# mkeeter/fidget

Measured on AMD Instinct MI355X. Metric: Mvoxel/s (interval+point eval) on prospero.vm 1024^3, higher is better.
Workload: dtype f32; 1 GPU; prospero.vm 3D heightmap+normals 1024^3, HipShape render hints (the library's tiles: 128/32/8, or 32/8 when the root level has few tiles), world_to_model=I

## Files before the change

fidget_amd/_abi.py:

```python
import ctypes as C
import os

import numpy as np

from ._build import LIB_PATH

UNARY = ["neg", "abs", "recip", "sqrt", "square", "floor", "ceil", "round", "sin", "cos", "tan",
         "asin", "acos", "atan", "exp", "ln", "not", "rand"]
BINARY = ["add", "sub", "mul", "div", "atan2", "min", "max", "compare", "mod", "and", "or", "mix"]

FH_OPS = (["Output", "Input", "CopyReg", "CopyImm"] + [u.capitalize() for u in UNARY]
          + [b.capitalize() + "RR" for b in ["add", "sub", "mul", "div", "atan2", "compare", "mix", "mod", "min", "max", "and", "or"]]
          + [b.capitalize() + "RI" for b in ["add", "sub", "mul", "div", "atan2", "compare", "mix", "mod", "min", "max", "and", "or"]]
          + [b.capitalize() + "IR" for b in ["sub", "div", "atan2", "compare", "mix", "mod"]])

STATUS = {1: "BadVarSlice", 2: "MismatchedSlices", 3: "BadChoiceSlice", 4: "MissingVar", 5: "BadTape",
          6: "Unsupported", 7: "HipError", 8: "Cancelled", 9: "ParseError", 10: "Overflow"}

GEOMETRY_PIXEL = np.dtype([("normal", np.float32, 3), ("depth", np.uint32)])
HIP_TILES_2D, HIP_TILES_3D = [128, 16], [128, 32, 8]
VM_TILES_2D, VM_TILES_3D = [128, 32, 8], [128, 64, 32, 16, 8]


class FidgetHipError(RuntimeError):
# ... 30 lines not shown
    "fhip_ctx_set_option": (i32, [vp, C.c_char_p, i32]),
    "fhip_ctx_get_option": (i32, [vp, C.c_char_p, C.POINTER(i32)]),
    "fhip_tape_from_bytecode": (i32, [vp, vp, C.c_size_t, C.POINTER(vp)]),
    "fhip_tape_free": (None, [vp]),
    "fhip_tape_len": (u32, [vp]),
    "fhip_tape_choice_count": (u32, [vp]),
    "fhip_tape_reg_count": (u32, [vp]),
    "fhip_tape_var_count": (u32, [vp]),
    "fhip_tape_output_count": (u32, [vp]),
    "fhip_tape_ops": (u32, [vp, vp, u32]),
    "fhip_tape_reg_tape": (i32, [vp, u32, vp, u32, vp, u32, vp]),
    "fhip_tape_group_count": (u32, [vp]),
    "fhip_tape_group_op": (i32, [vp]),
    "fhip_tape_group": (i32, [vp, vp, u32, vp]),
    "fhip_tape_term_plan": (u32, [vp, vp]),
    "fhip_tape_term_group": (i32, [vp, vp, u32, vp]),
    "fhip_tape_term_tree": (u32, [vp, vp, u32]),
    "fhip_tape_term_choice_src": (u32, [vp, vp, u32]),
    "fhip_simplify": (i32, [vp, vp, vp, u32, C.POINTER(vp)]),
    "fhip_interval_eval": (i32, [vp, vp, vp, u32, u32, vp, vp, vp]),
    "fhip_point_eval": (i32, [vp, vp, vp, u32, u32, vp, vp, vp]),
    "fhip_float_eval": (i32, [vp, vp, vp, vp, u32, vp]),
    "fhip_grad_eval": (i32, [vp, vp, vp, vp, u32, vp]),
    "fhip_solve": (i32, [vp, vp, u32, vp, vp, vp, u32, vp, u32, u32, vp, vp, vp, vp]),
    "fhip_render2d": (i32, [vp, vp, C.POINTER(_Cfg2D), vp, i32]),
    "fhip_render3d": (i32, [vp, vp, C.POINTER(_Cfg3D), vp, i32]),
    "fhip_render3d_shard": (i32, [vp, vp, C.POINTER(_Cfg3D), vp, i32, u32, u32]),
    "fhip_render3d_block": (i32, [vp, vp, C.POINTER(_Cfg3D), vp, i32, u32, vp]),
    "fhip_merge_depth": (i32, [vp, vp, vp, u64, u32]),
    "fhip_denoise_normals": (i32, [vp, vp, u32, u32, vp, i32]),
    "fhip_compute_ssao": (i32, [vp, vp, u32, u32, u32, vp, u32, vp, u32, vp, i32]),
    "fhip_blur_ssao": (i32, [vp, vp, u32, u32, vp, i32]),
    "fhip_apply_shading": (i32, [vp, vp, u32, u32, u32, vp, vp, i32]),
    "fhip_to_rgba": (i32, [vp, vp, u32, u32, i32, vp, i32]),
    "fhip_mesh_sample": (i32, [vp, vp, u32, vp, vp, vp, vp, u32, C.POINTER(vp)]),
    "fhip_mesh_build": (i32, [vp, vp, u32, vp, vp, vp, vp, u32, C.POINTER(vp)]),
    "fhip_mesh_vertices": (None, [vp, vp]),
    "fhip_mesh_triangles": (None, [vp, vp]),
    "fhip_mesh_vertices_ptr": (vp, [vp]),
    "fhip_mesh_triangles_ptr": (vp, [vp]),
    "fhip_mesh_free": (None, [vp]),
    "fhip_mesh_counts": (None, [vp, vp]),
    "fhip_mesh_leaves": (None, [vp, vp]),
    "fhip_mesh_sample_part": (i32, [vp, vp, u32, vp, vp, vp, vp, u32, u32, u32, C.POINTER(vp)]),
    "fhip_mesh_part_bytes": (C.c_uint64, [vp]),
    "fhip_mesh_part_export": (None, [vp, vp]),
    "fhip_mesh_merge": (i32, [vp, vp, vp, u32, vp, C.POINTER(vp)]),
    "fhip_mesh_vertices_dev": (vp, [vp]),
    "fhip_mesh_triangles_dev": (vp, [vp]),
    "fhip_mesh_stl_bytes": (u64, [vp]),
    "fhip_mesh_stl": (i32, [vp, vp, vp, i32]),
    "fhip_mesh_vertex_grads": (i32, [vp, vp, vp, vp, vp, vp, u32, vp, i32]),
    "fhip_shape_occupancy": (i32, [vp, vp, u32, vp, vp, vp, vp, u32, vp]),
    "fhip_voxels_words": (u64, [u32]),
    "fhip_shape_voxels": (i32, [vp, vp, u32, vp, vp, vp, vp, u32, vp, i32, vp]),
    "fhip_voxels_slices": (i32, [vp, vp, u32, u32, u32, vp, i32]),
    "fhip_voxels_layer_counts": (i32, [vp, vp, u32, vp, i32]),
    "fhip_contour2d": (i32, [vp, vp, vp, vp]),
    "fhip_contours_counts": (None, [vp, vp]),
    "fhip_contours_vertices": (i32, [vp, vp]),
    "fhip_contours_segments": (i32, [vp, vp]),
    "fhip_contours_next": (i32, [vp, vp]),
    "fhip_contours_vertices_dev": (vp, [vp]),
    "fhip_contours_segments_dev": (vp, [vp]),
    "fhip_contours_free": (None, [vp]),
    "fhip_contour_loops": (i32, [vp, u64, vp, vp, vp, vp]),
    "fhip_voxels_components": (i32, [vp, vp, u32, i32, u32, i32, vp]),
    "fhip_components_counts": (None, [vp, vp]),
    "fhip_components_table": (i32, [vp, vp, vp, vp, vp, vp]),
    "fhip_components_label_slices": (i32, [vp, vp, vp, i32, u32, u32, vp, i32]),
    "fhip_components_extract": (i32, [vp, vp, vp, i32, vp, u64, vp, i32]),
    "fhip_components_free": (None, [vp]),
    "fhip_voxels_distance": (i32, [vp, vp, u32, i32, i32, vp]),
    "fhip_distance_info": (None, [vp, vp]),
    "fhip_distance_slices": (i32, [vp, vp, u32, u32, vp, i32]),
    "fhip_distance_dev": (vp, [vp]),
    "fhip_distance_threshold": (i32, [vp, vp, u32, i32, vp, i32]),
    "fhip_distance_free": (None, [vp]),
    "fhip_distance_thickness": (i32, [vp, vp, vp]),
    "fhip_thickness_info": (None, [vp, vp]),
    "fhip_thickness_thin": (i32, [vp, vp, u32, vp, i32]),
    "fhip_thickness_histogram": (i32, [vp, vp, vp, u32, vp, i32]),
    "fhip_voxels_surface": (i32, [vp, vp, u32, i32, vp]),
    "fhip_voxels_mesh": (i32, [vp, vp, u32, i32, vp]),
    "fhip_voxels_flow": (i32, [vp, vp, vp, u32, i32, u32, u32, vp, i32]),
    "fhip_voxels_overhangs": (i32, [vp, vp, u32, i32, u32, u32, i32, vp, i32]),
    "fhip_voxels_heights": (i32, [vp, vp, u32, i32, u32, vp, i32]),
    "fhip_triangles_voxels": (i32, [vp, vp, u64, vp, u64, i32, vp, u32, vp, i32, vp]),
    "fhip_mesh_voxels": (i32, [vp, vp, vp, u32, vp, i32, vp]),
    "fhip_triangles_topology": (i32, [vp, vp, u64, vp, u64, i32, i32, u32, vp]),
    "fhip_mesh_topology": (i32, [vp, vp, i32, u32, vp]),
    "fhip_topology_counts": (None, [vp, vp]),
    "fhip_topology_vertex_rows": (u64, [vp]),
    "fhip_topology_vertices": (i32, [vp, vp]),
    "fhip_topology_triangles": (i32, [vp, vp]),
    "fhip_topology_triangle_shells": (i32, [vp, vp]),
    "fhip_topology_vertices_dev": (vp, [vp]),
    "fhip_topology_triangles_dev": (vp, [vp]),
    "fhip_topology_triangle_shells_dev": (vp, [vp]),
    "fhip_topology_shells": (i32, [vp, vp, vp, vp, vp, vp, vp, vp]),
    "fhip_topology_edges": (i32, [vp, vp, u32, vp, i32]),
    "fhip_topology_free": (None, [vp]),
    "fhip_voxels_outlines": (i32, [vp, vp, u32, i32, u32, u32, u32, vp]),
    "fhip_outlines_counts": (None, [vp, vp]),
    "fhip_outlines_layers": (i32, [vp, vp, vp, vp, vp]),
    "fhip_outlines_vertices": (i32, [vp, u64, u64, vp, vp, vp]),
    "fhip_outlines_loops": (i32, [vp, u64, u64, vp, vp, vp, vp, vp, vp]),
    "fhip_outlines_xy_dev": (vp, [vp]),
    "fhip_outlines_next_dev": (vp, [vp]),
    "fhip_outlines_loop_dev": (vp, [vp]),
    "fhip_outlines_free": (None, [vp]),
    "fhip_outlines_nesting": (i32, [vp, vp, vp, i32, vp]),
    "fhip_nesting_counts": (None, [vp, vp]),
    "fhip_nesting_layers": (i32, [vp, vp, vp, vp]),
    "fhip_nesting_loops": (i32, [vp, u64, u64, vp, vp, vp, vp, vp]),
    "fhip_nesting_parent_dev": (vp, [vp]),
    "fhip_nesting_depth_dev": (vp, [vp]),
    "fhip_nesting_children": (i32, [vp, u64, vp, vp]),
    "fhip_nesting_free": (None, [vp]),
    "fhip_topology_slices": (i32, [vp, vp, vp, u32, u32, vp]),
    "fhip_slices_counts": (None, [vp, vp]),
    "fhip_slices_planes": (i32, [vp, vp, vp, vp, vp]),
    "fhip_slices_loops": (i32, [vp, vp, vp, vp, vp, vp, vp, vp, vp]),
    "fhip_slices_vertices": (i32, [vp, vp, vp, vp, vp, vp, vp]),
    "fhip_slices_xy_dev": (vp, [vp]),
    "fhip_slices_next_dev": (vp, [vp]),
    "fhip_slices_loop_dev": (vp, [vp]),
    "fhip_slices_plane_dev": (vp, [vp]),
    "fhip_slices_free": (None, [vp]),
    "fhip_profile_enable": (None, [vp, i32]),
    "fhip_profile_read": (i32, [vp, vp, vp]),
    "fhip_profile_read_kernels": (i32, [vp, vp, vp]),
    "fhip_render_counters": (i32, [vp, vp]),
    "fhip_graph_new": (vp, []),
    "fhip_graph_free": (None, [vp]),
    "fhip_graph_len": (u32, [vp]),
    "fhip_graph_var": (u32, [vp, i32, u64]),
    "fhip_graph_constant": (u32, [vp, f32]),
    "fhip_graph_unary": (u32, [vp, i32, u32]),
    "fhip_graph_binary": (u32, [vp, i32, u32, u32]),
    "fhip_graph_from_text": (u32, [vp, C.c_char_p]),
    "fhip_tape_from_graph": (i32, [vp, vp, vp, u32, C.POINTER(vp)]),
    "fhip_tape_axis_slot": (i32, [vp, i32]),
    "fhip_tape_var_slot": (i32, [vp, u64]),
    "fhip_screen_to_world": (None, [vp, i32, vp]),
    "fhip_debug_stats": (i32, [vp, vp]),
    "fhip_debug_leaf_stats": (i32, [vp, vp]),
    "fhip_debug_tape_links": (u32, [vp, vp, u32]),
    "fhip_debug_tape_chain": (u32, [vp, vp, u32]),
    "fhip_debug_leaves": (u32, [vp, vp, u32]),
    "fhip_debug_probe": (i32, [vp, vp]),
    "fhip_debug_lane_frames": (u64, [vp]),
    "fhip_debug_rare_frames": (u64, [vp]),
    "fhip_debug_lane_tune": (i32, [vp, vp, vp]),
    "fhip_debug_trans_probe": (i32, [vp, u32, u32, u32, u64, vp]),
    "fhip_debug_arena": (u32, [vp, u32, u32, vp]),
    "fhip_debug_bound_tape": (i32, [vp, vp, vp, vp, vp, u32, C.POINTER(vp)]),
    "fhip_debug_bench": (i32, [vp, vp, u32, u32, i32, vp]),
    "fhip_debug_ubench": (i32, [vp, u32, u32, u32, vp]),
    "fhip_debug_math_sweep": (i32, [vp, i32, u32, u32, u64, vp, vp]),
    "fhip_debug_groups": (u32, [vp, i32, u32, vp, u32, vp]),
    "fhip_debug_walk_dual": (None, [vp, u64, vp, vp, u64, i32, vp, vp, vp]),
    "fhip_debug_stl_pack": (i32, [vp, vp, u64, vp, u64, vp]),
}
del vp, u32, i32, f32, u64
EXPORTS = list(SIGNATURES)

_lib = None


def lib():
    global _lib
    if _lib is None:
        if not os.path.exists(LIB_PATH):
            raise ImportError(f"{LIB_PATH} is missing: run `python -c 'import __graft_entry__ as g; g.build()'`")
        L = C.CDLL(LIB_PATH)
        for name, (res, args) in SIGNATURES.items():
            fn = getattr(L, name)
            fn.restype = res
            fn.argtypes = args
        _lib = L
    return _lib


def _p(a):
    return a.ctypes.data_as(C.c_void_p) if a is not None else None


def libm_probe():
    buf = C.create_string_buffer(200)
    n = lib().fhip_libm_probe(buf, 200)
    return int(n), buf.value.decode()


class _Handle:
    def __init__(self, h, free):
        self.h = h
        self._free = free

    def __del__(self):
        if self.h and self._free is not None:
            self._free(self.h)
            self.h = None


class _DeviceArray:
    def __init__(self, owner, ptr, shape, typestr):
        self._owner = owner
        self.ptr, self.shape = int(ptr), tuple(shape)
        self.__cuda_array_interface__ = {"shape": self.shape, "typestr": typestr, "data": (self.ptr, False), "version": 2, "strides": None}
```

fidget_amd/context.py:

```python
import ctypes as C
import os

import numpy as np

from ._abi import FidgetHipError, _p, lib


class HipContext:

    def __init__(self, device=0, stream=None):
        h = C.c_void_p()
        st = lib().fhip_ctx_create(device, C.c_void_p(stream or 0), C.byref(h))
        if st != 0:
            raise FidgetHipError(st, "no usable HIP device: fidget_amd has no CPU fallback")
        self._h = h

    def __del__(self):
        try:
            lib().fhip_ctx_destroy(self._h)
        except Exception:
            pass

    def check(self, st):
        if st != 0:
            raise FidgetHipError(st, (lib().fhip_last_error(self._h) or b"").decode())

    def sync(self):
        self.check(lib().fhip_ctx_sync(self._h))

    def trim(self):
        self.check(lib().fhip_ctx_trim(self._h))

    def reserve_arena(self, megabytes):
        self.check(lib().fhip_ctx_reserve_arena(self._h, int(megabytes)))

    def cancel(self):
        lib().fhip_cancel(self._h)

    def cancel_watch(self, flag):
        self._watched = flag
        lib().fhip_cancel_watch(self._h, None if flag is None else flag.ctypes.data_as(C.c_void_p))

    def cancel_reset(self):
        lib().fhip_cancel_reset(self._h)

    def lane_tune(self):
        ms, ln = (C.c_float * 3)(), C.c_int(0)
        ph = lib().fhip_debug_lane_tune(self._h, ms, C.byref(ln))
        return {"phase": int(ph), "stage_pipeline_ms": [float(ms[0]), float(ms[2])], "frame_lanes_ms": float(ms[1]), "kept": "frame lanes" if ln.value else "stage pipeline"}

    def lane_frames(self):
        return int(lib().fhip_debug_lane_frames(self._h))

    def rare_frames(self):
        return int(lib().fhip_debug_rare_frames(self._h))

    def set_option(self, name, value=1):
        self.check(lib().fhip_ctx_set_option(self._h, name.encode(), int(value)))

    def option(self, name):
        v = C.c_int(0)
        self.check(lib().fhip_ctx_get_option(self._h, name.encode(), C.byref(v)))
        return v.value

    def options(self, **kw):
        import contextlib

        @contextlib.contextmanager
        def scope():
            old = {k: self.option(k) for k in kw}
            try:
                for k, v in kw.items():
                    self.set_option(k, v)
                yield self
            finally:
                for k, v in old.items():
                    self.set_option(k, v)
        return scope()

    def profile(self, on):
        lib().fhip_profile_enable(self._h, int(on))

    def profile_read(self):
        ms = np.zeros(4, np.float64)
        n = np.zeros(4, np.uint32)
        self.check(lib().fhip_profile_read(self._h, _p(ms), _p(n)))
        names = ["tiles", "points", "normals", "other"]
        return {k: (float(ms[i]), int(n[i])) for i, k in enumerate(names)}

    def profile_read_kernels(self):
        ms = np.zeros(8, np.float64)
        n = np.zeros(8, np.uint32)
        self.check(lib().fhip_profile_read_kernels(self._h, _p(ms), _p(n)))
        names = ["fh_columns", "fh_float_eval_16x4", "fh_float_eval_32x2", "fh_tiles", "fh_prune1", "fh_tiles_v32", "fh_tiles_v64", "unused"]
        return {k: (float(ms[i]), int(n[i])) for i, k in enumerate(names)}

    def counters(self):
        c = np.zeros(8, np.uint64)
        self.check(lib().fhip_render_counters(self._h, _p(c)))
        return {"arena_ops": int(c[0]), "arena_overflow": int(c[1]), "leaves_last_slab": int(c[2]),
                "queue_overflow": int(c[3]), "groups_last_slab": [int(v) for v in c[4:6]], "hip_tile_stage_frames": int(c[6]), "substituted_tile_lists": int(c[7])}

    def last_leaves(self, cap=1 << 20):
        dt = np.dtype([("off", np.uint32), ("len", np.uint32), ("regs", np.uint16), ("choices", np.uint16),
                       ("x", np.uint32), ("y", np.uint32), ("z", np.uint32)])
        buf = np.zeros(cap, dt)
        n = lib().fhip_debug_leaves(self._h, _p(buf), cap)
        return buf[:n]

    def groups(self, kind, index, cap=1 << 20):
        dt = np.dtype([("off", np.uint32), ("len", np.uint32), ("regs", np.uint16), ("choices", np.uint16),
                       ("x", np.uint32), ("y", np.uint32), ("z", np.uint32), ("first", np.uint32), ("n", np.uint32), ("stride", np.uint32)])
        assert dt.itemsize == 36
        buf = np.zeros(cap, dt)
        cnt = np.zeros(2, np.uint32)
        n = lib().fhip_debug_groups(self._h, kind, index, _p(buf), cap, _p(cnt))
        return buf[:n], (int(cnt[0]), int(cnt[1]))

    def arena_ops(self, off, n):
        buf = np.zeros(n, np.uint64)
        got = lib().fhip_debug_arena(self._h, int(off), int(n), _p(buf))
        return buf[:got]

    def leaf_stats(self):
        c = np.zeros(8, np.uint64)
        self.check(lib().fhip_debug_leaf_stats(self._h, _p(c)))
        return {"leaves": int(c[0]), "tape_ops": int(c[1]), "tape_words_read": int(c[2]), "lane_ops": int(c[3]),
                "prune2_phase_clocks_max": [int(v) for v in c[4:8]]}

    def wave_stats(self):
        c = np.zeros(64, np.uint64)
        self.check(lib().fhip_debug_stats(self._h, _p(c)))
        names = ["tiles_l0", "tiles_l1", "tiles_l2", "tiles_l3", "tiles_l4", "columns_c0", "columns_c12", "tiles_2d"]
        self.tile_v = {f"l{l}": {"slots": int(c[8 + l]), "fwd_clocks": int(c[16 + l]), "prune_clocks": int(c[24 + l]), "max_slot_clocks": int(c[l])}
                       for l in range(8) if c[8 + l]}
        self.tile_phases = {f"l{l}": {"fwd_us": int(c[32 + l]) / 100.0, "prune_us": int(c[40 + l]) / 100.0,
                                      "ops": int(c[48 + l]), "ops_written": int(c[56 + l]), "fwd_shader_clocks": int(c[16 + l])} for l in range(8) if c[48 + l]}
        return {k: {"busy_us_sum": int(c[4 * i]) / 100.0, "busy_us_max": int(c[4 * i + 1]) / 100.0,
                    "waves": int(c[4 * i + 2]), "units": int(c[4 * i + 3])} for i, k in enumerate(names) if c[4 * i + 2]}


_default_ctx = None


def default_context():
    global _default_ctx
    if _default_ctx is None:
        _default_ctx = HipContext(int(os.environ.get("LOCAL_RANK", "0")) if os.environ.get("FHIP_USE_LOCAL_RANK") else 0)
    return _default_ctx
```

fidget_amd/csrc/capi_context.hpp:

```cpp
int fhip_libm_probe(char* msg, size_t cap) {
    using namespace fhlm;
    struct R1 { const char* name; float (*mine)(float); float (*host)(float); };
    const R1 r1[] = {{"sinf", [](float x) { return sincosf_<MemTables, false>(x); }, [](float x) { return ::sinf(x); }},
                     {"cosf", [](float x) { return sincosf_<MemTables, true>(x); }, [](float x) { return ::cosf(x); }},
                     {"tanf", [](float x) { return tanf_<MemTables>(x); }, [](float x) { return ::tanf(x); }},
                     {"asinf", [](float x) { return asinf_(x); }, [](float x) { return ::asinf(x); }},
                     {"acosf", [](float x) { return acosf_(x); }, [](float x) { return ::acosf(x); }},
                     {"atanf", [](float x) { return atanf_(x); }, [](float x) { return ::atanf(x); }},
                     {"expf", [](float x) { return expf_<MemTables>(x); }, [](float x) { return ::expf(x); }},
                     {"logf", [](float x) { return logf_<MemTables>(x); }, [](float x) { return ::logf(x); }}};
    static const float args[32] = {0.1f, -0.3f, 0.5f, 0.7853982f, 0.7853981f, 1.0f, -1.0f, 1.5707964f, 2.0f, 3.0f, 3.1415927f, -4.5f, 6.2831855f, 10.0f,
                                   -25.132742f, 100.0f, 119.99999f, 120.0f, 1000.5f, -31415.926f, 1.0e6f, 3.0e8f, 1.0e-3f, 2.4414062e-4f, -1.0e-5f,
                                   1.0e-20f, 0.9999999f, 0.99f, -0.6f, 0.25f, 87.0f, -80.0f};
    int bad = 0;
    if (msg && cap) msg[0] = 0;
    auto differ = [](float a, float b) { return !(a != a && b != b) && f2u(a) != f2u(b); };
    for (const R1& r : r1)
        for (float x : args) {
            volatile float xv = x;
            const float a = r.mine(xv), b = r.host(xv);
            if (differ(a, b) && bad++ == 0 && msg && cap)
                snprintf(msg, cap, "%s(%a): device family 0x%08x, host libm 0x%08x", r.name, (double)x, f2u(a), f2u(b));
        }
    for (int i = 0; i < 32; i++) {
        volatile float y = args[i], x = args[(i * 7 + 3) & 31];
        const float a = atan2f_(y, x), b = ::atan2f(y, x);
        if (differ(a, b) && bad++ == 0 && msg && cap)
            snprintf(msg, cap, "atan2f(%a, %a): device family 0x%08x, host libm 0x%08x", (double)y, (double)x, f2u(a), f2u(b));
    }
    return bad;
}
static void libm_probe_once() {
    static std::once_flag once;
    std::call_once(once, [] {
        char msg[160];
        const int bad = fhip_libm_probe(msg, sizeof msg);
        const char* q = getenv("FHIP_QUIET");
        if (bad && !(q && q[0] == '1'))
            fprintf(stderr, "fidget-hip: this host's libm is not the one the device restates (glibc 2.35 x86-64, FMA variants; trans_libm.hpp): %d of 288 "
                            "probe arguments differ, first %s.  Transcendental opcodes on the device will differ from this host's CPU evaluators "
                            "in the last bits for some arguments.\n", bad, msg);
    });
}

fhip_status fhip_ctx_create(int device, void* stream, fhip_ctx** out) {
    if (!out) return FHIP_ERR_BAD_TAPE;
    *out = nullptr;
    libm_probe_once();
    int count = 0;
    if (hipGetDeviceCount(&count) != hipSuccess || count <= 0 || device >= count) return FHIP_ERR_HIP;
    fhip_ctx* c = new fhip_ctx();
    c->device = device;
    c->stream = (hipStream_t)stream;
    if (hipSetDevice(device) != hipSuccess) { delete c; return FHIP_ERR_HIP; }
    hipDeviceProp_t prop;
    if (hipGetDeviceProperties(&prop, device) == hipSuccess) c->n_cu = prop.multiProcessorCount;
    options_from_env(c->opt);
    apply_options(c);
    const void* fns[] = {(const void*)k_eval_f32<false>, (const void*)k_eval_interval<false>, (const void*)k_eval_grad<false>,
                         (const void*)k_tiles<false, false, true, 16>, (const void*)k_tiles<false, true, true, 16>,
                         (const void*)k_tiles<true, false, true, 16>, (const void*)k_tiles<true, true, true, 16>,
                         (const void*)k_tiles<false, false, true, 64>, (const void*)k_tiles<false, true, true, 64>,
                         (const void*)k_tiles<true, false, true, 64>, (const void*)k_tiles<true, true, true, 64>,
                         (const void*)k_pixels2d<0, false>, (const void*)k_pixels2d<0, true>,
                         (const void*)k_leaves3d<2, 0, 1, false>, (const void*)k_leaves3d<2, 0, 1, true>,
                         (const void*)k_normals3d<false, true>, (const void*)k_normals3d<true, true>};
    for (const void* f : fns) (void)hipFuncSetAttribute(f, hipFuncAttributeMaxDynamicSharedMemorySize, FH_LDS_MAX);
    {
        std::vector<char> alt;
        if (const char* p = getenv("FHIP_INTERP_CO")) {
            if (FILE* f = fopen(p, "rb")) {
                fseek(f, 0, SEEK_END);
                long n = ftell(f);
                fseek(f, 0, SEEK_SET);
                alt.resize(n > 0 ? (size_t)n : 0);
                if (n <= 0 || fread(alt.data(), 1, (size_t)n, f) != (size_t)n) alt.clear();
                fclose(f);
            }
            if (alt.empty()) { fprintf(stderr, "fidget-hip: FHIP_INTERP_CO=%s cannot be read\n", p); delete c; return FHIP_ERR_HIP; }
            fprintf(stderr, "fidget-hip: assembly kernels from %s\n", p);
        }
        if (hipModuleLoadData(&c->asm_mod, alt.empty() ? (const void*)fh_interp_co : (const void*)alt.data()) != hipSuccess) { delete c; return FHIP_ERR_HIP; }
    }
    for (int i = 0; i < FH_ASM_COUNT; i++)
        if (hipModuleGetFunction(&c->asm_fn[i], c->asm_mod, FH_ASM_NAMES[i]) != hipSuccess) { delete c; return FHIP_ERR_HIP; }
    (void)hipFuncSetAttribute((const void*)c->asm_fn[FH_ASM_TILES], hipFuncAttributeMaxDynamicSharedMemorySize, FH_LDS_MAX);
    (void)hipFuncSetAttribute((const void*)c->asm_fn[FH_ASM_TILES_T], hipFuncAttributeMaxDynamicSharedMemorySize, FH_LDS_MAX);
    (void)hipGetLastError();
    {
        int lo = 0, hi = 0;
        (void)hipDeviceGetStreamPriorityRange(&lo, &hi);
        if (hipStreamCreateWithPriority(&c->stream2, hipStreamNonBlocking, hi) != hipSuccess) { delete c; return FHIP_ERR_HIP; }
    }
    (void)hipEventCreateWithFlags(&c->ev_fork, hipEventDisableTiming);
    (void)hipEventCreateWithFlags(&c->ev_pre, hipEventDisableTiming);
    (void)hipEventCreateWithFlags(&c->ev_l0, hipEventDisableTiming);
    (void)hipEventCreateWithFlags(&c->ev_l1, hipEventDisableTiming);
    (void)hipEventCreateWithFlags(&c->ev_rest_fork, hipEventDisableTiming);
    (void)hipEventCreateWithFlags(&c->ev_rest_join, hipEventDisableTiming);
    (void)hipEventCreateWithFlags(&c->ev_done, hipEventDisableTiming);
    for (auto& o : c->others) (void)hipEventCreateWithFlags(&o.ev_done, hipEventDisableTiming);
    if (!c->stream3 && hipStreamCreateWithFlags(&c->stream3, hipStreamNonBlocking) != hipSuccess) { delete c; return FHIP_ERR_HIP; }
    if (hipStreamCreateWithFlags(&c->stream_pre, hipStreamNonBlocking) != hipSuccess) { delete c; return FHIP_ERR_HIP; }
    if (c->sticky.ensure(256) != hipSuccess || hipMemset(c->sticky.p, 0, 256) != hipSuccess) { delete c; return FHIP_ERR_HIP; }
    {
        void* hf = nullptr;
        if (hipHostMalloc(&hf, 64, hipHostMallocDefault) != hipSuccess) { delete c; return FHIP_ERR_HIP; }
        memset(hf, 0, 64);
        ((uint32_t*)hf)[2] = 1;
        c->host_flags = (volatile uint32_t*)hf;
    }
    c->ev_tiles.resize(FH_MAX_SLABS); c->ev_leaves.resize(FH_MAX_SLABS); c->ev_aux.resize(FH_MAX_SLABS);
    for (int i = 0; i < FH_MAX_SLABS; i++) {
        (void)hipEventCreateWithFlags(&c->ev_tiles[i], hipEventDisableTiming);
        (void)hipEventCreateWithFlags(&c->ev_leaves[i], hipEventDisableTiming);
        (void)hipEventCreateWithFlags(&c->ev_aux[i], hipEventDisableTiming);
    }
    (void)hipFuncSetAttribute((const void*)k_prune2, hipFuncAttributeMaxDynamicSharedMemorySize, FH_LDS_MAX);
    {
        const void* fb[] = {(const void*)k_teval3d<false, true>, (const void*)k_teval3d<true, true>};
        for (const void* f : fb) (void)hipFuncSetAttribute(f, hipFuncAttributeMaxDynamicSharedMemorySize, FH_LDS_MAX);
    }
    *out = c;
    return FHIP_OK;
}
static void lanes_release(fhip_ctx* ctx, bool keep_measurements = false);
void fhip_ctx_destroy(fhip_ctx* c) {
    if (!c) return;
    (void)hipSetDevice(c->device);
    (void)hipStreamSynchronize(c->stream);
    lanes_release(c);
    if (c->ev_last) (void)hipEventDestroy(c->ev_last);
    if (c->stream_pre) (void)hipStreamSynchronize(c->stream_pre);
    if (c->stream2) (void)hipStreamSynchronize(c->stream2);
    (void)hipStreamSynchronize(c->stream);
    DevBuf* bufs[] = {&c->tmp_out, &c->io_a, &c->io_b, &c->io_c, &c->io_d, &c->io_e, &c->sticky};
    for (DevBuf* b : bufs) b->release();
    c->release_all();
    for (auto& o : c->others) o.release_all();
    if (c->stream_pre) (void)hipStreamDestroy(c->stream_pre);
    if (c->ev_rest_fork) (void)hipEventDestroy(c->ev_rest_fork);
    if (c->ev_rest_join) (void)hipEventDestroy(c->ev_rest_join);
    if (c->ev_pre) (void)hipEventDestroy(c->ev_pre);
    if (c->ev_l0) (void)hipEventDestroy(c->ev_l0);
    if (c->ev_l1) (void)hipEventDestroy(c->ev_l1);
    for (auto& sg : c->staging) { if (sg.p) (void)hipHostFree(sg.p); if (sg.ev) (void)hipEventDestroy(sg.ev); }
    c->mesh_leaves.release();
    if (c->host_flags) (void)hipHostFree((void*)c->host_flags);
    if (c->mesh_pinned) (void)hipHostFree(c->mesh_pinned);
    mesh_cache_release(c->mesh_octree_cache);
    free(c->mesh_first);
    if (c->asm_mod) (void)hipModuleUnload(c->asm_mod);
    if (c->stream2) { (void)hipStreamSynchronize(c->stream2); (void)hipStreamDestroy(c->stream2); }
    if (c->stream3) { (void)hipStreamSynchronize(c->stream3); (void)hipStreamDestroy(c->stream3); }
    for (hipEvent_t e : c->ev_aux) (void)hipEventDestroy(e);
    if (c->ev_fork) (void)hipEventDestroy(c->ev_fork);
    for (hipEvent_t e : c->ev_tiles) (void)hipEventDestroy(e);
    for (hipEvent_t e : c->ev_leaves) (void)hipEventDestroy(e);
    for (auto& e : c->prof_events) { (void)hipEventDestroy(e.second.first); (void)hipEventDestroy(e.second.second); }
    for (auto& e : c->asm_events) { (void)hipEventDestroy(e.second.first); (void)hipEventDestroy(e.second.second); }
    delete c;
}
const char* fhip_last_error(const fhip_ctx* c) { return c ? c->err.c_str() : "no context"; }
fhip_status fhip_ctx_sync(fhip_ctx* c) {
    (void)hipSetDevice(c->device);
    HIP_TRY(c, hipStreamSynchronize(c->stream));
    fhip_status st = FHIP_OK;
    for (auto& o : c->others)
        if (o.async_pending) {
            std::swap(static_cast<FrameBufs&>(*c), o);
            c->async_pending = false;
            const fhip_status s1 = finish_render(c);
            if (st == FHIP_OK) st = s1;
            std::swap(static_cast<FrameBufs&>(*c), o);
        }
    if (c->async_pending) {
        c->async_pending = false;
        const fhip_status s2 = finish_render(c);
        if (st == FHIP_OK) st = s2;
    }
    for (fhip_ctx* L : c->lanes) {
        const fhip_status s3 = fhip_ctx_sync(L);
        if (s3 && st == FHIP_OK) { st = s3; c->err = L->err; }
    }
    uint32_t sticky = 0;
    HIP_TRY(c, hipMemcpy(&sticky, c->sticky.p, 4, hipMemcpyDeviceToHost));
    if (sticky) {
        HIP_TRY(c, hipMemset(c->sticky.p, 0, 4));
        if (st == FHIP_OK) st = fail(c, FHIP_ERR_OVERFLOW, "device work queue overflow in an earlier asynchronous frame");
    }
    return st;
}
void fhip_cancel(fhip_ctx* c) { c->cancelled.store(1); }
void fhip_cancel_reset(fhip_ctx* c) { c->cancelled.store(0); }
void fhip_cancel_watch(fhip_ctx* c, const void* flag) { c->watch.store((const volatile unsigned char*)flag); }
fhip_status fhip_ctx_trim(fhip_ctx* c) {
    if (!c) return FHIP_ERR_UNSUPPORTED;
    (void)hipSetDevice(c->device);
    HIP_TRY(c, hipDeviceSynchronize());
    lanes_release(c);
    c->mesh_leaves.release();
    if (c->mesh_pinned) { (void)hipHostFree(c->mesh_pinned); c->mesh_pinned = nullptr; c->mesh_pinned_cap = 0; }
    return FHIP_OK;
}
static hipError_t sync_own_streams(fhip_ctx* ctx);
fhip_status fhip_ctx_reserve_arena(fhip_ctx* c, size_t megabytes) {
    if (!c) return FHIP_ERR_UNSUPPORTED;
    (void)hipSetDevice(c->device);
    const size_t want = std::min(c->arena_cap_bytes, megabytes << 20);
    if (want <= c->arena_bytes) return FHIP_OK;
    HIP_TRY(c, sync_own_streams(c));
    c->arena_bytes = want;
    return FHIP_OK;
}
fhip_status fhip_ctx_set_option(fhip_ctx* c, const char* name, int value) {
    if (!c || !name) return FHIP_ERR_UNSUPPORTED;
    if (!strcmp(name, "leaf_streams") || !strcmp(name, "pre_priority")) return fail(c, FHIP_ERR_UNSUPPORTED, std::string(name) + " is fixed when the context is created");
    for (const FhOptionEntry& e : FH_OPTION_TABLE)
        if (!strcmp(e.name, name)) {
            if (c->opt.*(e.field) == value) return FHIP_OK;
            const fhip_status st = fhip_ctx_sync(c);
            c->opt.*(e.field) = value;
            apply_options(c);
            lanes_release(c);
            return st;
        }
    return fail(c, FHIP_ERR_UNSUPPORTED, std::string("unknown option ") + name);
}
fhip_status fhip_ctx_get_option(const fhip_ctx* c, const char* name, int* value) {
    if (!c || !name || !value) return FHIP_ERR_UNSUPPORTED;
    for (const FhOptionEntry& e : FH_OPTION_TABLE)
        if (!strcmp(e.name, name)) { *value = c->opt.*(e.field); return FHIP_OK; }
    return FHIP_ERR_UNSUPPORTED;
}
```

fidget_amd/csrc/capi_core.hpp:

```cpp
struct DevBuf {
    void* p = nullptr;
    size_t cap = 0;
    hipError_t ensure(size_t bytes) {
        if (bytes <= cap) return hipSuccess;
        if (p) (void)hipFree(p);
        p = nullptr; cap = 0;
        hipError_t e = hipMalloc(&p, bytes);
        if (e == hipSuccess) cap = bytes;
        return e;
    }
    void release() { if (p) (void)hipFree(p); p = nullptr; cap = 0; }
};

static std::atomic<uint64_t> g_tape_serial{1};
struct BoundCache {
    struct Entry {
        uint64_t hash = 0, used = 0;
        std::vector<uint64_t> key;
        std::shared_ptr<const fhip_tape> tape;
    };
    std::mutex lock;
    std::vector<Entry> entries;
    uint64_t clock = 0;
};
struct fhip_tape {
    const uint64_t serial = g_tape_serial.fetch_add(1);
    fh::HostTape t;
    mutable uint64_t* d_ops = nullptr;
    std::vector<fh::HostTape> groups;
    int group_op = -1;
    fh::TermPlan plan;
    std::vector<fh::HostTape> tgroups;
    mutable FhTopOp* d_top = nullptr;
    mutable uint32_t* d_chsrc = nullptr;
    mutable uint64_t* d_links = nullptr;
    mutable uint64_t* d_ctab = nullptr;
    mutable std::atomic<uint32_t> input_slots{0x80000000u};
    mutable uint32_t n_chain = 0;
    mutable bool links_tried = false;
    mutable std::mutex upload_lock;
    mutable int device = -1;
    uint64_t parent_serial = 0;
    std::weak_ptr<const fhip_tape> self;
    mutable BoundCache bound;
};
struct fhip_graph {
    fh::Graph g;
};

#ifndef __HIP_DEVICE_COMPILE__
__asm__(".section .rodata\n.global fh_interp_co\n.p2align 6\nfh_interp_co:\n.incbin \"" FH_INTERP_CO "\"\n.previous\n");
#endif
extern "C" const char fh_interp_co[];
enum { FH_ASM_COLUMNS = 0, FH_ASM_FLOAT_16x4, FH_ASM_FLOAT_32x2, FH_ASM_TILES, FH_ASM_PRUNE1, FH_ASM_TILES_V32, FH_ASM_TILES_V64, FH_ASM_PROBE, FH_ASM_UBENCH, FH_ASM_COLUMNS_T, FH_ASM_NORMALS, FH_ASM_NORMALS_T, FH_ASM_TILES_T, FH_ASM_TILES_V32_T, FH_ASM_TILES_V64_T, FH_ASM_FLOAT_16x4_T, FH_ASM_FLOAT_32x2_T, FH_ASM_TRANS_PROBE, FH_ASM_COUNT };
static const char* const FH_ASM_NAMES[FH_ASM_COUNT] = {"fh_columns", "fh_float_eval_16x4", "fh_float_eval_32x2", "fh_tiles", "fh_prune1",
                                                       "fh_tiles_v32", "fh_tiles_v64", "fh_probe", "fh_ubench", "fh_columns_t", "fh_normals", "fh_normals_t", "fh_tiles_t", "fh_tiles_v32_t", "fh_tiles_v64_t", "fh_float_eval_16x4_t", "fh_float_eval_32x2_t", "fh_trans_probe"};

#define FH_OPTION_LIST(X)                                                                                                       \
     \
    X(no_asm, 0) X(no_split, 0) X(no_asm_tiles, 0) X(no_tiles_v, 0) X(no_asm_tiles_t, 0) X(no_columns_t, 0) X(no_asm_normals, 0)   \
    X(no_tape_groups, 0) X(prune2, 1)                                                                                           \
                      \
    X(no_column_inv, 0) X(no_zrep, 0) X(root32_max, 4096) X(column_walk, 1) X(column_group, 2)                                                    \
                                                                                                 \
    X(no_pipeline, 0) X(frame_lanes, 4) X(lanes_fail, 0) X(slab_layers, 4) X(arena_mb, 4096)  \
          \
    X(mesh_device_assembly, 1) X(mesh_device_walk, 1) X(mesh_simplify_min_ops, 256) X(mesh_keep_device, 0)                      \
                                                                                                              \
    X(probe, 0) X(stats, 0)
struct FhOptions {
#define X(name, dflt) int name = dflt;
    FH_OPTION_LIST(X)
#undef X
};
struct FhOptionEntry { const char* name; int FhOptions::*field; };
static const FhOptionEntry FH_OPTION_TABLE[] = {
#define X(name, dflt) {#name, &FhOptions::name},
    FH_OPTION_LIST(X)
#undef X
};
static void options_from_env(FhOptions& o) {
    for (const FhOptionEntry& e : FH_OPTION_TABLE) {
        std::string var = "FHIP_";
        for (const char* c = e.name; *c; c++) var += (char)toupper((unsigned char)*c);
        if (const char* v = getenv(var.c_str())) o.*(e.field) = *v ? atoi(v) : 1;
    }
}

struct FrameBufs {
    DevBuf state, arena, leaves, leaf_table, zbuf, normals, fp_lists, mind, squeue, slots[2], leaves_b, leaf_table_b, fp_lists_b, chw[2], tvals, topch, chwr, gscratch, rare_scratch;
    DevBuf queue[FH_MAX_LEVELS];
    uint32_t frame_stamp = 0;
    uint64_t resident_serial = 0;
    uint32_t resident_groups = 0;
    uint32_t forked = 0;
    bool async_pending = false;
    hipEvent_t ev_done = nullptr;
    bool ev_done_valid = false;
    std::shared_ptr<const fhip_tape> bound_hold;
    CleanSig clean;
    void release_all() {
        clean = CleanSig();
        DevBuf* bufs[] = {&state, &arena, &leaves, &leaf_table, &zbuf, &normals, &fp_lists, &mind, &squeue, &slots[0], &slots[1],
                          &leaves_b, &leaf_table_b, &fp_lists_b, &chw[0], &chw[1], &tvals, &topch, &chwr, &gscratch, &rare_scratch};
        for (DevBuf* b : bufs) b->release();
        for (auto& q : queue) q.release();
        if (ev_done) (void)hipEventDestroy(ev_done);
        ev_done = nullptr;
        bound_hold.reset();
    }
};
struct fhip_ctx : FrameBufs {
    FhOptions opt;
#define FH_EXTRA_SETS 4
    FrameBufs others[FH_EXTRA_SETS];
    uint32_t extra_sets = 3;
    bool frame_pipeline = true;
    hipStream_t stream_pre = nullptr;
    uint32_t pre_turn = 0;
    hipEvent_t ev_rest_fork = nullptr, ev_rest_join = nullptr;
    hipEvent_t ev_pre = nullptr, ev_l0 = nullptr, ev_l1 = nullptr;
    hipModule_t asm_mod = nullptr;
    hipFunction_t asm_fn[FH_ASM_COUNT] = {};
    bool use_asm = true;
    bool probe = false;
    bool use_split = true;
    bool use_pipeline = true;
    hipStream_t stream2 = nullptr, stream3 = nullptr;
    std::vector<hipEvent_t> ev_tiles, ev_leaves, ev_aux;
    hipEvent_t ev_fork = nullptr;
    FhRenderState last_state_b;
    uint32_t slab_contexts = 4;
    int device = 0;
    hipStream_t stream = nullptr;
    int n_cu = 256;
    std::string err;
    bool launch_failed = false;
    std::atomic<int> cancelled{0};
    const std::atomic<int>* cancel_src = nullptr;
    std::atomic<const volatile unsigned char*> watch{nullptr};
    bool is_cancelled() const {
        if ((cancel_src ? cancel_src : &cancelled)->load() != 0) return true;
        const volatile unsigned char* w = watch.load(std::memory_order_relaxed);
        return w && *w != 0;
    }
    DevBuf tmp_out, io_a, io_b, io_c, io_d, io_e;
    DevBuf sticky;
    struct Staging { void* p = nullptr; size_t cap = 0; hipEvent_t ev = nullptr; bool used = false; } staging[8];
    DevBuf mesh_leaves;
    void* mesh_pinned = nullptr;
    size_t mesh_pinned_cap = 0;
    void* mesh_octree_cache = nullptr;
    uint32_t* mesh_first = nullptr;
    size_t mesh_first_cap = 0;
    uint32_t staging_next = 0;
    size_t arena_bytes = (size_t)256 << 20, arena_cap_bytes = (size_t)4 << 30;
    uint64_t hip_tile_frames = 0;
    uint64_t substituted_tiles = 0;
    int last_hip_error = 0;
    volatile uint32_t* host_flags = nullptr;
    bool profiling = false;
    std::vector<std::pair<int, std::pair<hipEvent_t, hipEvent_t>>> prof_events;
    std::vector<std::pair<int, std::pair<hipEvent_t, hipEvent_t>>> asm_events;
    FhRenderState last_state;
    bool have_last_state = false;
    std::vector<fhip_ctx*> lanes;
    uint32_t lane_next = 0;
    uint64_t rare_frames = 0;
    uint64_t lane_frames = 0;
    uint64_t lane_frames_wanted = 0;
    hipEvent_t ev_last = nullptr;
    bool ev_last_valid = false;
    struct LaneTune {
        uint64_t key = 0, used = 0;
        int phase = 0;
        uint32_t n = 0;
        bool lanes = false;
        float ms[3] = {0.0f, 0.0f, 0.0f};
        hipEvent_t ev[6] = {nullptr, nullptr, nullptr, nullptr, nullptr, nullptr};
    };
    std::vector<LaneTune> lane_tune;
    uint64_t tune_last_key = 0, tune_clock = 0;
    int tune_cur = -1;
    bool is_lane = false, lane_stream_owned = false;
    DevBuf lane_img;
    hipEvent_t lane_done = nullptr, lane_copied = nullptr;
    bool lane_copied_valid = false;
};

#define FH_ARENA_START_MB 128
static void apply_options(fhip_ctx* c) {
    c->use_asm = c->opt.no_asm == 0;
    c->use_split = c->opt.no_split == 0;
    c->probe = c->opt.probe != 0;
    c->use_pipeline = c->opt.no_pipeline == 0;
    c->frame_pipeline = true;
    c->slab_contexts = 4;
    c->arena_cap_bytes = (size_t)std::max(1, c->opt.arena_mb) << 20;
    c->arena_bytes = std::min(c->arena_cap_bytes, std::max(c->arena_bytes, (size_t)FH_ARENA_START_MB << 20));
    c->extra_sets = 3;
}

static fhip_status finish_render(fhip_ctx* ctx);
static void mesh_cache_release(void* octree);
static fhip_status fail(fhip_ctx* ctx, fhip_status s, const std::string& msg) {
    if (ctx) ctx->err = msg;
    return s;
}
#define HIP_TRY(ctx, call)                                                                                       \
    do {                                                                                                         \
        hipError_t e_ = (call);                                                                                  \
        if (e_ != hipSuccess) {                                                                                  \
            if (ctx) (ctx)->last_hip_error = (int)e_;                                                            \
            return fail(ctx, FHIP_ERR_HIP, std::string(#call) + ": " + hipGetErrorString(e_));                   \
        }                                                                                                        \
    } while (0)

template <class F>
static void launch(fhip_ctx* ctx, hipStream_t st, int klass, F&& f) {
    if (ctx->profiling) {
        hipEvent_t a, b;
        (void)hipEventCreate(&a);
        (void)hipEventCreate(&b);
        (void)hipEventRecord(a, st);
        f();
        (void)hipEventRecord(b, st);
        ctx->prof_events.push_back({klass, {a, b}});
    } else {
        f();
    }
}

static bool simplify_host(const fh::HostTape& p, const uint8_t* choices, fh::HostTape& out) {
    std::vector<int> map(FH_MAX_REGS, -1);
    fh::RegPool pool;
    std::vector<uint64_t> rev;
    uint32_t ci = p.n_choices, kept = 0;
    auto use = [&](uint32_t r) { if (map[r] < 0) map[r] = pool.take(); return (uint32_t)map[r]; };
    for (size_t k = p.ops.size(); k-- > 0;) {
        const uint64_t w = p.ops[k];
        const uint32_t w0 = (uint32_t)w, w1 = (uint32_t)(w >> 32);
        const uint32_t op = FH_W_OP(w0), ro = FH_W_OUT(w0), ra = FH_W_A(w0), rb = w1;
        const bool is_choice = fh_is_choice(op);
        uint32_t c = FH_CHOICE_BOTH;
        if (is_choice) {
            c = choices[--ci];
            if (c == FH_CHOICE_UNKNOWN) return false;
        }
        if (op == FH_OUTPUT) { rev.push_back(fh_pack(op, 0, use(ra), 0, w1)); continue; }
        const int no = map[ro];
        if (no < 0) continue;
        map[ro] = -1;
        int alias = -1;
        bool copy_imm = false;
        if (op == FH_COPY_REG) alias = (int)ra;
        else if (is_choice && c == FH_CHOICE_LEFT) alias = (int)ra;
        else if (is_choice && c == FH_CHOICE_RIGHT) { if (fh_is_rr(op)) alias = (int)rb; else copy_imm = true; }
        if (alias >= 0) {
            if (map[alias] < 0) { map[alias] = no; continue; }
            pool.give(no);
            rev.push_back(fh_pack(FH_COPY_REG, no, map[alias], 0, 0));
            continue;
        }
        pool.give(no);
        if (copy_imm) { rev.push_back(fh_pack(FH_COPY_IMM, no, 0, 0, w1)); continue; }
        uint32_t na = 0, nb = 0;
        if (op != FH_INPUT && op != FH_COPY_IMM) na = use(ra);
        if (fh_is_rr(op)) nb = use(rb);
        if (is_choice) kept++;
        rev.push_back(fh_pack(op, no, na, nb, w1));
    }
    out.ops.assign(rev.rbegin(), rev.rend());
    out.n_regs = pool.high;
    out.n_choices = kept;
    out.n_outputs = p.n_outputs;
    out.n_vars = p.n_vars;
    out.vars = p.vars;
    return true;
}

template <class T> struct FhKArgs;
template <class... K> struct FhKArgs<void (*)(K...)> {
    template <class... A> static size_t pack(char* buf, A&&... a) {
        size_t off = 0;
        auto put = [&](auto v) {
            constexpr size_t al = alignof(decltype(v));
            off = (off + al - 1) & ~(al - 1);
            memcpy(buf + off, &v, sizeof(v));
            off += sizeof(v);
        };
        (put(static_cast<K>(std::forward<A>(a))), ...);
        return off;
    }
    static constexpr size_t bytes = (sizeof(K) + ... + 0) + 16 * sizeof...(K);
};
template <auto Kernel, class... A>
static inline void fh_launch(fhip_ctx* ctx, dim3 g, dim3 b, size_t lds, hipStream_t st, A&&... a) {
    constexpr int MAXDEV = 64;
    static std::atomic<hipFunction_t> fns[MAXDEV];
    static std::atomic<bool> no_handle[MAXDEV];
    const int device = ctx->device;
    hipFunction_t fn = nullptr;
    if (device >= 0 && device < MAXDEV) {
        fn = fns[device].load(std::memory_order_acquire);
        if (!fn && !no_handle[device].load(std::memory_order_relaxed)) {
            if (hipGetFuncBySymbol(&fn, (const void*)Kernel) != hipSuccess || !fn) { fn = nullptr; no_handle[device].store(true, std::memory_order_relaxed); (void)hipGetLastError(); }
            else fns[device].store(fn, std::memory_order_release);
        }
    }
    hipError_t e;
    if (!fn) {
        hipLaunchKernelGGL(Kernel, g, b, lds, st, std::forward<A>(a)...);
        e = hipGetLastError();
    } else {
        alignas(16) char buf[FhKArgs<decltype(Kernel)>::bytes];
        size_t bytes = FhKArgs<decltype(Kernel)>::pack(buf, std::forward<A>(a)...);
        void* extra[] = {HIP_LAUNCH_PARAM_BUFFER_POINTER, buf, HIP_LAUNCH_PARAM_BUFFER_SIZE, &bytes, HIP_LAUNCH_PARAM_END};
        e = hipModuleLaunchKernel(fn, g.x, g.y, g.z, b.x, b.y, b.z, (unsigned)lds, st, nullptr, extra);
    }
    if (e != hipSuccess) {
        ctx->launch_failed = true;
        ctx->last_hip_error = (int)e;
        if (ctx->err.empty()) ctx->err = std::string("kernel launch: ") + hipGetErrorString(e);
        (void)hipGetLastError();
    }
// ... 4 lines not shown
```

fidget_amd/csrc/capi_debug.hpp:

```cpp
void fhip_profile_enable(fhip_ctx* ctx, int on) { ctx->profiling = on != 0; }
fhip_status fhip_profile_read(fhip_ctx* ctx, double ms[4], uint32_t launches[4]) {
    HIP_TRY(ctx, hipStreamSynchronize(ctx->stream));
    for (int i = 0; i < 4; i++) { ms[i] = 0; launches[i] = 0; }
    for (auto& e : ctx->prof_events) {
        float t = 0;
        if (hipEventElapsedTime(&t, e.second.first, e.second.second) == hipSuccess) { ms[e.first] += t; launches[e.first]++; }
    }
    return FHIP_OK;
}
fhip_status fhip_profile_read_kernels(fhip_ctx* ctx, double ms[8], uint32_t launches[8]) {
    HIP_TRY(ctx, hipStreamSynchronize(ctx->stream));
    for (int i = 0; i < 8; i++) { ms[i] = 0; launches[i] = 0; }
    for (auto& e : ctx->asm_events) {
        float t = 0;
        if (e.first < 8 && hipEventElapsedTime(&t, e.second.first, e.second.second) == hipSuccess) { ms[e.first] += t; launches[e.first]++; }
    }
    return FHIP_OK;
}
fhip_status fhip_render_counters(fhip_ctx* ctx, uint64_t out[8]) {
    fhip_status st = finish_render(ctx);
    if (st != FHIP_OK && st != FHIP_ERR_OVERFLOW) return st;
    const FhRenderState& S = ctx->last_state;
    out[0] = S.arena_head; out[1] = S.arena_overflow; out[2] = S.n_leaves; out[3] = S.queue_overflow;
    for (int i = 0; i < 2; i++) out[4 + i] = S.count[i + 1];
    out[6] = ctx->hip_tile_frames;
    out[7] = ctx->substituted_tiles;
    return FHIP_OK;
}

fhip_status fhip_debug_stats(fhip_ctx* ctx, uint64_t out[64]) {
    fhip_status st = finish_render(ctx);
    if (st != FHIP_OK && st != FHIP_ERR_OVERFLOW) return st;
    for (int i = 0; i < 64; i++) out[i] = ctx->last_state.stat[i];
    return FHIP_OK;
}
uint32_t fhip_debug_tape_links(const fhip_tape* tape, uint64_t* out, uint32_t cap) {
    std::vector<uint64_t> lk;
    std::vector<uint64_t> cops;
    if (!fh::compute_links(tape->t, lk, cops)) return 0;
    for (size_t i = 0; i < lk.size() && i < cap; i++) out[i] = lk[i];
    return (uint32_t)lk.size();
}
uint32_t fhip_debug_tape_chain(const fhip_tape* tape, uint32_t* out, uint32_t cap) {
    std::vector<uint64_t> lk;
    std::vector<uint64_t> cops;
    if (!fh::compute_links(tape->t, lk, cops)) return 0;
    const std::vector<uint32_t> chain = chain_table(tape, cops);
    for (size_t i = 0; i < chain.size() && i < cap; i++) out[i] = chain[i];
    return (uint32_t)chain.size();
}
fhip_status fhip_debug_leaf_stats(fhip_ctx* ctx, uint64_t out[8]) {
    fhip_status st = finish_render(ctx);
    if (st != FHIP_OK && st != FHIP_ERR_OVERFLOW) return st;
    for (int i = 0; i < 8; i++) out[i] = ctx->last_state.leaf_stat[i];
    return FHIP_OK;
}

uint32_t fhip_debug_leaves(fhip_ctx* ctx, void* out, uint32_t cap) {
    if (finish_render(ctx) != FHIP_OK) return 0;
    const uint32_t n = std::min(std::min(ctx->last_state.n_leaves, ctx->last_state.leaf_cap), cap);
    if (hipMemcpy(out, ctx->last_state.leaves, (size_t)n * sizeof(FhLeaf), hipMemcpyDeviceToHost) != hipSuccess) return 0;
    return n;
}

uint32_t fhip_debug_groups(fhip_ctx* ctx, int kind, uint32_t index, void* out, uint32_t cap, uint32_t counts[2]) {
    counts[0] = counts[1] = 0;
    if (finish_render(ctx) != FHIP_OK) return 0;
    const FhRenderState& S = ctx->last_state;
    const FhGroup* base; uint32_t ns, nb, qcap;
    if (kind == 0) {
        if (index >= FH_MAX_LEVELS || !S.queue[index]) return 0;
        base = S.queue[index]; ns = S.count[index]; nb = S.count_big[index]; qcap = S.qcap[index];
    } else {
        if (index >= FH_MAX_SLABS || !S.squeue) return 0;
        base = S.squeue + (size_t)index * S.squeue_cap; ns = S.scount[index]; nb = S.scount_big[index]; qcap = S.squeue_cap;
    }
    ns = std::min(ns, qcap); nb = std::min(nb, qcap - ns);
    const uint32_t n0 = std::min(ns, cap), n1 = std::min(nb, cap - n0);
    if (n0 && hipMemcpy(out, base, (size_t)n0 * sizeof(FhGroup), hipMemcpyDeviceToHost) != hipSuccess) return 0;
    if (n1 && hipMemcpy((FhGroup*)out + n0, base + (qcap - nb), (size_t)n1 * sizeof(FhGroup), hipMemcpyDeviceToHost) != hipSuccess) return 0;
    counts[0] = n0; counts[1] = n1;
    return n0 + n1;
}

fhip_status fhip_debug_probe(fhip_ctx* ctx, float* out) {
    HIP_TRY(ctx, ctx->io_a.ensure(16 * 256));
    struct { void* p; } ka = {ctx->io_a.p};
    if (launch_asm(ctx, ctx->stream, FH_ASM_PROBE, 1, &ka, sizeof(ka)) != hipSuccess) return FHIP_ERR_HIP;
    HIP_TRY(ctx, hipStreamSynchronize(ctx->stream));
    HIP_TRY(ctx, hipMemcpy(out, ctx->io_a.p, 16 * 256, hipMemcpyDeviceToHost));
    return FHIP_OK;
}

fhip_status fhip_debug_ubench(fhip_ctx* ctx, uint32_t test, uint32_t iters, uint32_t n_waves, float* out) {
    HIP_TRY(ctx, ctx->io_a.ensure((size_t)n_waves * 4));
    HIP_TRY(ctx, hipMemsetAsync(ctx->io_a.p, 0, (size_t)n_waves * 4, ctx->stream));
    struct { void* p; uint32_t test, iters; } ka = {ctx->io_a.p, test, iters};
    if (launch_asm(ctx, ctx->stream, FH_ASM_UBENCH, n_waves, &ka, sizeof(ka), 64) != hipSuccess) return FHIP_ERR_HIP;
    HIP_TRY(ctx, hipStreamSynchronize(ctx->stream));
    HIP_TRY(ctx, hipMemcpy(out, ctx->io_a.p, (size_t)n_waves * 4, hipMemcpyDeviceToHost));
    return FHIP_OK;
}

fhip_status fhip_debug_math_sweep(fhip_ctx* ctx, int op, uint32_t first, uint32_t stride, uint64_t n, const float* ref, uint64_t out[4]) {
    (void)hipSetDevice(ctx->device);
    HIP_TRY(ctx, ctx->io_a.ensure(n * 4));
    HIP_TRY(ctx, ctx->io_b.ensure(64));
    HIP_TRY(ctx, hipMemcpyAsync(ctx->io_a.p, ref, n * 4, hipMemcpyHostToDevice, ctx->stream));
    HIP_TRY(ctx, hipMemsetAsync(ctx->io_b.p, 0, 64, ctx->stream));
    hipLaunchKernelGGL(k_math_sweep, dim3(ctx->n_cu * 16), dim3(256), 0, ctx->stream, op, first, stride, (size_t)n, (const float*)ctx->io_a.p,
                       (unsigned long long*)ctx->io_b.p);
    HIP_TRY(ctx, hipGetLastError());
    unsigned long long r[4];
    HIP_TRY(ctx, hipMemcpyAsync(r, ctx->io_b.p, 32, hipMemcpyDeviceToHost, ctx->stream));
    HIP_TRY(ctx, hipStreamSynchronize(ctx->stream));
    out[0] = r[0] >> 32; out[1] = r[1]; out[2] = r[2]; out[3] = r[0] & 0xFFFFFFFFull;
    return FHIP_OK;
}

fhip_status fhip_debug_trans_probe(fhip_ctx* ctx, uint32_t copy, uint32_t fn, uint32_t first, uint64_t n, uint64_t out[2]) {
    (void)hipSetDevice(ctx->device);
    if (!n || n % 256 || n > (1ull << 28)) return fail(ctx, FHIP_ERR_UNSUPPORTED, "trans probe: n must be a multiple of 256, at most 2^28");
    if (!ctx->asm_fn[FH_ASM_TRANS_PROBE]) return fail(ctx, FHIP_ERR_UNSUPPORTED, "trans probe: the assembly kernels are not loaded");
    HIP_TRY(ctx, ctx->io_a.ensure(n * 4));
    HIP_TRY(ctx, ctx->io_b.ensure(64));
    HIP_TRY(ctx, hipMemsetAsync(ctx->io_a.p, 0x5A, n * 4, ctx->stream));
    HIP_TRY(ctx, hipMemsetAsync(ctx->io_b.p, 0, 64, ctx->stream));
    struct { void* out; uint32_t first, copy, fn, pad; } ka = {ctx->io_a.p, first, copy, fn, 0};
    if (launch_asm(ctx, ctx->stream, FH_ASM_TRANS_PROBE, (uint32_t)(n / 256), &ka, sizeof(ka)) != hipSuccess) return FHIP_ERR_HIP;
    hipLaunchKernelGGL(k_trans_compare, dim3(ctx->n_cu * 16), dim3(256), 0, ctx->stream, (int)fn, first, (size_t)n, (const uint32_t*)ctx->io_a.p,
                       (unsigned long long*)ctx->io_b.p);
    HIP_TRY(ctx, hipGetLastError());
    unsigned long long r[2];
    HIP_TRY(ctx, hipMemcpyAsync(r, ctx->io_b.p, 16, hipMemcpyDeviceToHost, ctx->stream));
    HIP_TRY(ctx, hipStreamSynchronize(ctx->stream));
    out[0] = r[1]; out[1] = r[0] & 0xFFFFFFFFull;
    return FHIP_OK;
}

uint64_t fhip_debug_rare_frames(const fhip_ctx* ctx) {
    if (!ctx) return 0;
    uint64_t n = ctx->rare_frames;
    for (const fhip_ctx* l : ctx->lanes) n += l ? l->rare_frames : 0;
    return n;
}
uint64_t fhip_debug_lane_frames(const fhip_ctx* ctx) { return ctx ? ctx->lane_frames : 0; }
int fhip_debug_lane_tune(const fhip_ctx* ctx, float ms[3], int* lanes) {
    if (!ctx) return -1;
    for (const auto& t : ctx->lane_tune)
        if (t.key == ctx->tune_last_key) {
            if (ms) { ms[0] = t.ms[0]; ms[1] = t.ms[1]; ms[2] = t.ms[2]; }
            if (lanes) *lanes = t.lanes ? 1 : 0;
            return t.phase;
        }
    return -1;
}

uint32_t fhip_debug_arena(fhip_ctx* ctx, uint32_t off, uint32_t n, uint64_t* out) {
    if ((size_t)(off + (size_t)n) * 8 > ctx->arena_bytes) return 0;
    if (hipMemcpy(out, (const uint64_t*)ctx->arena.p + off, (size_t)n * 8, hipMemcpyDeviceToHost) != hipSuccess) return 0;
    return n;
}

fhip_status fhip_debug_bench(fhip_ctx* ctx, const fhip_tape* tape, uint32_t n_waves, uint32_t reps, int variant, double* ms) {
    fhip_status st = tape_to_device(ctx, tape);
    if (st) return st;
    HIP_TRY(ctx, ctx->state.ensure(2 * sizeof(FhRenderState)));
    FhRenderState S;
    memset(&S, 0, sizeof(S));
    for (int i = 0; i < FH_MAX_INPUTS; i++) S.P.in_kind[i] = i % 3;
    HIP_TRY(ctx, hipMemcpy(ctx->state.p, &S, sizeof(S), hipMemcpyHostToDevice));
    HIP_TRY(ctx, ctx->io_a.ensure((size_t)n_waves * WAVE * 4));
    hipEvent_t a, b;
    HIP_TRY(ctx, hipEventCreate(&a));
    HIP_TRY(ctx, hipEventCreate(&b));
    const uint32_t len = (uint32_t)tape->t.ops.size();
    FhRenderState* dS = (FhRenderState*)ctx->state.p;
    for (int it = 0; it < 2; it++) {
        HIP_TRY(ctx, hipEventRecord(a, ctx->stream));
        if (variant == 0) hipLaunchKernelGGL((k_bench_points<16, 4>), dim3(n_waves), dim3(WAVE), 0, ctx->stream, dS, tape->d_ops, len, reps, (float*)ctx->io_a.p);
        else if (variant == 1) hipLaunchKernelGGL((k_bench_points<32, 2>), dim3(n_waves), dim3(WAVE), 0, ctx->stream, dS, tape->d_ops, len, reps, (float*)ctx->io_a.p);
        else if (variant == 3) hipLaunchKernelGGL((k_bench_points<32, 1>), dim3(n_waves), dim3(WAVE), 0, ctx->stream, dS, tape->d_ops, len, reps, (float*)ctx->io_a.p);
        else hipLaunchKernelGGL((k_bench_points<0, 1>), dim3(n_waves), dim3(WAVE), (size_t)std::max<uint32_t>(tape->t.n_regs, 1) * WAVE * 4, ctx->stream, dS, tape->d_ops, len, reps, (float*)ctx->io_a.p);
        HIP_TRY(ctx, hipEventRecord(b, ctx->stream));
        HIP_TRY(ctx, hipEventSynchronize(b));
    }
    float t = 0;
    HIP_TRY(ctx, hipEventElapsedTime(&t, a, b));
    *ms = t;
    (void)hipEventDestroy(a); (void)hipEventDestroy(b);
    return FHIP_OK;
}

static const int UNARY_MAP[] = {FH_NEG, FH_ABS, FH_RECIP, FH_SQRT, FH_SQUARE, FH_FLOOR, FH_CEIL, FH_ROUND, FH_SIN,
                                FH_COS, FH_TAN, FH_ASIN, FH_ACOS, FH_ATAN, FH_EXP, FH_LN, FH_NOT, FH_RAND};
static const int BINARY_MAP[] = {FH_ADD_RR, FH_SUB_RR, FH_MUL_RR, FH_DIV_RR, FH_ATAN2_RR, FH_MIN_RR, FH_MAX_RR,
                                 FH_COMPARE_RR, FH_MOD_RR, FH_AND_RR, FH_OR_RR, FH_MIX_RR};
fhip_graph* fhip_graph_new(void) { return new fhip_graph(); }
void fhip_graph_free(fhip_graph* g) { delete g; }
uint32_t fhip_graph_len(const fhip_graph* g) { return (uint32_t)g->g.nodes.size(); }
uint32_t fhip_graph_var(fhip_graph* g, int kind, uint64_t index) { return g->g.var((uint8_t)kind, kind < 3 ? 0 : index); }
uint32_t fhip_graph_constant(fhip_graph* g, float v) { return g->g.constant(v); }
uint32_t fhip_graph_unary(fhip_graph* g, int opcode, uint32_t a) {
    if (opcode < 0 || opcode >= 18) return fh::NO_NODE;
    return g->g.unary(UNARY_MAP[opcode], a);
}
uint32_t fhip_graph_binary(fhip_graph* g, int opcode, uint32_t a, uint32_t b) {
    if (opcode < 0 || opcode >= 12) return fh::NO_NODE;
    return g->g.binary(BINARY_MAP[opcode], a, b);
}
uint32_t fhip_graph_from_text(fhip_graph* g, const char* text) {
    std::string err;
    return g->g.parse(text, err);
}
```

fidget_amd/csrc/capi_render.hpp:

```cpp
static fhip_status bind_inputs(fhip_ctx* ctx, const fhip_tape* tape, const int32_t* axis_slots, const uint64_t* keys,
                               const float* vals, uint32_t n, FhRender& P) {
    const fh::HostTape& t = tape->t;
    std::vector<char> bound(FH_MAX_INPUTS, 0);
    for (uint32_t s = 0; s < FH_MAX_INPUTS; s++) { P.in_kind[s] = 3; P.in_value[s] = 0.0f; }
    for (int a = 0; a < 3; a++) {
        const int s = axis_slots ? axis_slots[a] : t.vars.axis[a];
        if (s >= 0 && s < FH_MAX_INPUTS) { P.in_kind[s] = (uint32_t)a; bound[s] = 1; }
    }
    for (uint32_t i = 0; i < n; i++) {
        const int s = axis_slots ? (int)keys[i] : t.vars.slot_of(3, keys[i]);
        if (s >= 0 && s < FH_MAX_INPUTS) { P.in_value[s] = vals[i]; bound[s] = 1; }
    }
    for (uint32_t s = 0; s < t.n_vars; s++)
        if (!bound[s]) return fail(ctx, FHIP_ERR_MISSING_VAR, "a variable of the shape has no value");
    return FHIP_OK;
}

struct HostSpans {
    double t[8] = {0, 0, 0, 0, 0, 0, 0, 0};
    uint64_t n = 0;
    std::chrono::steady_clock::time_point last;
    void start() { last = std::chrono::steady_clock::now(); }
    void mark(int k) { const auto now = std::chrono::steady_clock::now(); t[k] += std::chrono::duration<double, std::micro>(now - last).count(); last = now; }
    void frame() {
// ... 19 lines not shown
    hipError_t e = hipSuccess;
    for (hipStream_t s : {ctx->stream, ctx->stream2, ctx->stream3, ctx->stream_pre}) {
        const hipError_t r = hipStreamSynchronize(s);
        if (r != hipSuccess && e == hipSuccess) e = r;
    }
    for (fhip_ctx* L : ctx->lanes)
        if (L) { const hipError_t r = sync_own_streams(L); if (r != hipSuccess && e == hipSuccess) e = r; }
    return e;
}
static fhip_status grow_arena_if_asked(fhip_ctx* ctx, size_t want) {
    if (want == ctx->arena_bytes) return FHIP_OK;
    HIP_TRY(ctx, sync_own_streams(ctx));
    if (ctx->host_flags) ctx->host_flags[0] = 0;
    ctx->arena_bytes = want;
    return FHIP_OK;
}

static fhip_status ensure_root_tables(fhip_ctx* ctx, const fhip_tape* tape) {
    const fh::HostTape& t = tape->t;
    std::lock_guard<std::mutex> guard(tape->upload_lock);
    if (tape->device >= 0 && tape->device != ctx->device) return fail(ctx, FHIP_ERR_UNSUPPORTED, "this tape's device copies belong to another device: build the tape per device");
    tape->device = ctx->device;
    if (!tape->d_top) {
        static_assert(sizeof(FhTopOp) == sizeof(fh::TopOp), "top op layout");
        HIP_TRY(ctx, hipMalloc((void**)&tape->d_top, tape->plan.top.size() * sizeof(FhTopOp)));
        HIP_TRY(ctx, hipMemcpy(tape->d_top, tape->plan.top.data(), tape->plan.top.size() * sizeof(FhTopOp), hipMemcpyHostToDevice));
        HIP_TRY(ctx, hipMalloc((void**)&tape->d_chsrc, std::max<size_t>(tape->plan.choice_src.size(), 1) * 4));
        HIP_TRY(ctx, hipMemcpy(tape->d_chsrc, tape->plan.choice_src.data(), tape->plan.choice_src.size() * 4, hipMemcpyHostToDevice));
    }
    if (ctx->opt.prune2 && !tape->links_tried) {
        tape->links_tried = true;
        std::vector<uint64_t> lk;
        std::vector<uint64_t> cops;
        if (fh::compute_links(t, lk, cops)) {
            uint64_t *dl = nullptr, *dc = nullptr;
            std::vector<uint32_t> chain = chain_table(tape, cops);
            const size_t n_cops = std::max<size_t>(cops.size(), 1);
            cops.resize(n_cops + (chain.size() + 1) / 2, 0);
            if (!chain.empty()) memcpy(cops.data() + n_cops, chain.data(), chain.size() * 4);
            hipError_t e = hipMalloc((void**)&dl, lk.size() * 8);
            if (e == hipSuccess) e = hipMemcpy(dl, lk.data(), lk.size() * 8, hipMemcpyHostToDevice);
            if (e == hipSuccess) e = hipMalloc((void**)&dc, std::max<size_t>(cops.size(), 1) * 8);
            if (e == hipSuccess) e = hipMemcpy(dc, cops.data(), cops.size() * 8, hipMemcpyHostToDevice);
            if (e != hipSuccess) {
                if (dl) (void)hipFree(dl);
                if (dc) (void)hipFree(dc);
                HIP_TRY(ctx, e);
            }
            tape->d_links = dl; tape->d_ctab = dc; tape->n_chain = (uint32_t)chain.size();
        }
    }
    return FHIP_OK;
}

static void bind_state(fhip_ctx* ctx, const fhip_tape* tape, bool is3d, RenderSetup& R) {
    FhRenderState& S = R.S;
    const FhRender& P = S.P;
    S.frame_stamp = ++ctx->frame_stamp;
    if (R.hip_tiles_unasked) ctx->hip_tile_frames++;
    S.gscratch = R.big_hbm ? (char*)ctx->gscratch.p : nullptr;
    if (is3d) {
        uint32_t* mp = (uint32_t*)ctx->mind.p;
        for (uint32_t l = 0; l < P.n_levels; l++) {
            S.mind[l] = mp;
            mp += (size_t)((P.width + P.tiles[l] - 1) / P.tiles[l]) * ((P.height + P.tiles[l] - 1) / P.tiles[l]);
        }
        for (int c = 0; c < 3; c++) S.fp_list[c] = (uint32_t*)ctx->fp_lists.p + (size_t)c * R.n_footprints;
        S.hit_list = (uint32_t*)ctx->fp_lists.p + (size_t)3 * R.n_footprints;
    }
    S.arena = (uint64_t*)ctx->arena.p;
    S.arena_overflow = 0;
    for (int l = 0; l < FH_MAX_LEVELS; l++) {
        S.queue[l] = (FhGroup*)ctx->queue[l].p;
        S.count[l] = S.cursor[l] = S.count_big[l] = S.cursor_big[l] = 0;
    }
    S.count_big[0] = (uint32_t)R.roots.size();
    if (R.groups) {
        S.ttop = tape->d_top; S.chsrc = tape->d_chsrc;
        R.d_ctab = tape->d_ctab; R.d_links = tape->d_links;
        S.tvals = (float*)ctx->tvals.p; S.topch = (uint8_t*)ctx->topch.p; S.chwr = (uint32_t*)ctx->chwr.p;
    }
    if (R.prune1) for (int k = 0; k < 2; k++) S.chw[k] = (uint32_t*)ctx->chw[k].p;
    if (R.split) for (int k = 0; k < 2; k++) S.slots[k] = (FhSlot*)ctx->slots[k].p;
    S.squeue = (FhGroup*)ctx->squeue.p;
    for (int k = 0; k < FH_MAX_SLABS; k++) S.scount[k] = S.scount_big[k] = 0;
    S.queue_overflow = 0;
    S.leaves = (FhLeaf*)ctx->leaves.p;
    S.n_leaves = S.leaf_cursor = S.leaf_cursor_big = S.normal_cursor = S.normal_cursor_big = 0;
    S.leaf_table = (FhLeafRef*)ctx->leaf_table.p;
    for (int c = 0; c < 3; c++) S.fp_count[c] = S.fp_cursor[c] = 0;
    S.zbuf = (uint64_t*)ctx->zbuf.p;
    S.normals = (float*)ctx->normals.p;
    S.image2d = nullptr;
    memset(S.stat, 0, sizeof(S.stat));
    memset(S.leaf_stat, 0, sizeof(S.leaf_stat));
    S.want_stats = (ctx->profiling || ctx->probe || (ctx->opt.stats & 1)) ? 1 : 0;
}

static fhip_status prepare(fhip_ctx* ctx, const fhip_tape* tape, const TapeFacts& facts, bool is3d, const std::vector<uint32_t>& ts,
                           const PartSpec& part, RenderSetup& R) {
    static_assert(PLAN_BAD_TAPE == FHIP_ERR_BAD_TAPE && PLAN_UNSUPPORTED == FHIP_ERR_UNSUPPORTED, "the plan's refusals are fhip_status values");
    const FhRender& P = R.S.P;
    PlanInputs in = plan_inputs(ctx);
    in.arena_bytes = arena_bytes_for(ctx->arena_bytes, ctx->arena_cap_bytes, (size_t)FH_ARENA_START_MB << 20, ctx->host_flags && ctx->host_flags[0] != 0, facts.n_ops,
                                     is3d && !R.root_invariant ? (uint64_t)P.width * P.height * P.depth : 0);
    const PlanStatus ps = plan_frame(facts, in, is3d, ts, part, R);
    if (ps.status) return fail(ctx, (fhip_status)ps.status, ps.msg);
    { const fhip_status gs = grow_arena_if_asked(ctx, in.arena_bytes); if (gs) return gs; }
    const FrameBytes& B = R.bytes;
    HIP_TRY(ctx, ctx->gscratch.ensure(B.gscratch));
    HIP_TRY(ctx, ctx->state.ensure(4 * sizeof(FhRenderState)));
    { void* const before = ctx->arena.p; HIP_TRY(ctx, ctx->arena.ensure(ctx->arena_bytes)); if (ctx->arena.p != before) ctx->resident_serial = 0; }
    for (size_t l = 0; l < ts.size(); l++) HIP_TRY(ctx, ctx->queue[l].ensure(B.queue[l]));
    const std::pair<DevBuf*, size_t> list[] = {{&ctx->squeue, B.squeue}, {&ctx->leaves, B.leaves}, {&ctx->leaves_b, B.leaves_b}, {&ctx->leaf_table, B.leaf_table},
                                               {&ctx->leaf_table_b, B.leaf_table_b}, {&ctx->zbuf, B.zbuf}, {&ctx->normals, B.normals}, {&ctx->fp_lists, B.fp_lists},
                                               {&ctx->fp_lists_b, B.fp_lists_b}, {&ctx->mind, B.mind}, {&ctx->tvals, B.tvals}, {&ctx->topch, B.topch}, {&ctx->chwr, B.chwr},
                                               {&ctx->chw[0], B.chw[0]}, {&ctx->chw[1], B.chw[1]}, {&ctx->slots[0], B.slots}, {&ctx->slots[1], B.slots}};
    for (const auto& b : list) HIP_TRY(ctx, b.first->ensure(b.second));
    if (R.groups) {
        const fhip_status us = ensure_root_tables(ctx, tape);
        if (us) return us;
        plan_linked_prune(facts, in, tape->d_links && tape->d_ctab, tape->n_chain, R);
    }
    bind_state(ctx, tape, is3d, R);
    return FHIP_OK;
}

static int blocks_for(const fhip_ctx* ctx, size_t lds, int max_per_cu);
static int blocks_big(const fhip_ctx* ctx, const RenderSetup& R, size_t lds, int max_per_cu) {
    return R.big_hbm ? (int)R.hbm_waves : blocks_for(ctx, lds, max_per_cu);
}
static int blocks_for(const fhip_ctx* ctx, size_t lds, int max_per_cu) {
    int per_cu = lds ? (int)std::min<size_t>((size_t)max_per_cu, FH_LDS_MAX / std::max<size_t>(lds, 1)) : max_per_cu;
    per_cu = std::max(per_cu, 1);
    return ctx->n_cu * per_cu;
}

static fhip_status finish_render(fhip_ctx* ctx) {
    HIP_TRY(ctx, hipMemcpyAsync(&ctx->last_state, ctx->state.p, sizeof(FhRenderState), hipMemcpyDeviceToHost, ctx->stream));
    HIP_TRY(ctx, hipStreamSynchronize(ctx->stream));
    for (uint32_t k = 1; k < ctx->forked; k++) {
        HIP_TRY(ctx, hipMemcpy(&ctx->last_state_b, (char*)ctx->state.p + k * sizeof(FhRenderState), sizeof(FhRenderState), hipMemcpyDeviceToHost));
        ctx->last_state.queue_overflow += ctx->last_state_b.queue_overflow;
        ctx->last_state.arena_overflow += ctx->last_state_b.arena_overflow;
        for (int i = 0; i < 64; i++) ctx->last_state.stat[i] += ctx->last_state_b.stat[i];
        for (int i = 0; i < 8; i++) ctx->last_state.leaf_stat[i] += ctx->last_state_b.leaf_stat[i];
    }
    ctx->have_last_state = true;
    if (ctx->last_state.queue_overflow) return fail(ctx, FHIP_ERR_OVERFLOW, "device work queue overflow");
    return FHIP_OK;
}

struct FrameClear { void* p = nullptr; size_t bytes = 0; uint32_t fill = 0; };
static fhip_status upload_frame(fhip_ctx* ctx, hipStream_t st, const fhip_tape* tape, RenderSetup& R, const FrameClear (&clear)[3]) {
    const size_t roots_bytes = R.roots.size() * sizeof(FhGroup);
    fhip_ctx::Staging& sg = ctx->staging[ctx->staging_next++ % 8];
    if (sg.ev && sg.used) HIP_TRY(ctx, hipEventSynchronize(sg.ev));
    if (!sg.ev) HIP_TRY(ctx, hipEventCreateWithFlags(&sg.ev, hipEventDisableTiming));
    if (sg.cap < sizeof(FhRenderState) + roots_bytes) {
        if (sg.p) (void)hipHostFree(sg.p);
        sg.p = nullptr; sg.cap = 0;
        HIP_TRY(ctx, hipHostMalloc(&sg.p, sizeof(FhRenderState) + roots_bytes + 4096, hipHostMallocDefault));
        sg.cap = sizeof(FhRenderState) + roots_bytes + 4096;
    }
    memcpy(sg.p, &R.S, sizeof(FhRenderState));
    if (roots_bytes) memcpy((char*)sg.p + sizeof(FhRenderState), R.roots.data(), roots_bytes);
    { const fhip_status hs = hold_bound(ctx, tape); if (hs) return hs; }
    if (ctx->resident_serial != tape->serial || ctx->resident_groups != R.S.n_tgroups) {
        ctx->resident_serial = 0;
        HIP_TRY(ctx, hipMemcpyAsync(ctx->arena.p, tape->t.ops.data(), tape->t.ops.size() * 8, hipMemcpyHostToDevice, st));
        for (uint32_t g = 0; g < R.S.n_tgroups; g++)
            HIP_TRY(ctx, hipMemcpyAsync((uint64_t*)ctx->arena.p + R.S.tgroup[g].off, tape->tgroups[g].ops.data(),
                                        tape->tgroups[g].ops.size() * 8, hipMemcpyHostToDevice, st));
        ctx->resident_serial = tape->serial;
        ctx->resident_groups = R.S.n_tgroups;
    }
    static_assert(sizeof(FhRenderState) % 4 == 0 && sizeof(FhGroup) % 4 == 0, "copied as 32-bit words");
    FhFrameBegin fb;
    memset(&fb, 0, sizeof(fb));
    fb.state_dst = (uint32_t*)ctx->state.p; fb.state_src = (const uint32_t*)sg.p; fb.state_words = (uint32_t)(sizeof(FhRenderState) / 4);
    if (!R.roots.empty()) {
        fb.roots_dst = (uint32_t*)((FhGroup*)ctx->queue[0].p + (R.S.qcap[0] - R.roots.size()));
        fb.roots_src = (const uint32_t*)((const char*)sg.p + sizeof(FhRenderState));
        fb.roots_words = (uint32_t)(roots_bytes / 4);
    }
    size_t most = 0;
    for (int k = 0; k < 3; k++) {
        fb.clear[k] = (uint32_t*)clear[k].p; fb.clear_words[k] = clear[k].bytes / 4; fb.fill[k] = clear[k].fill;
        if (clear[k].p) most = std::max(most, clear[k].bytes);
    }
    const unsigned blocks = (unsigned)std::max<size_t>(8, std::min<size_t>((size_t)ctx->n_cu * 32, (most + 64 * 64 - 1) / (64 * 64)));
    FH_KLAUNCH(k_frame_begin, dim3(blocks), dim3(WAVE), 0, st, fb);
    HIP_TRY(ctx, hipGetLastError());
    HIP_TRY(ctx, hipEventRecord(sg.ev, st));
    sg.used = true;
    for (auto& e : ctx->prof_events) { (void)hipEventDestroy(e.second.first); (void)hipEventDestroy(e.second.second); }
    ctx->prof_events.clear();
    for (auto& e : ctx->asm_events) { (void)hipEventDestroy(e.second.first); (void)hipEventDestroy(e.second.second); }
    ctx->asm_events.clear();
    return FHIP_OK;
}

#define FH_LAUNCH_TILES(IS3D, FULL, BIG, grid, lds)                                                                  \
    do {                                                                                                            \
        if (R.tl == 64) FH_KLAUNCH((k_tiles<IS3D, FULL, BIG, 64>), dim3(grid), dim3(WAVE), lds, st, dS, level); \
        else FH_KLAUNCH((k_tiles<IS3D, FULL, BIG, 16>), dim3(grid), dim3(WAVE), lds, st, dS, level);            \
    } while (0)
struct KaTiles { FhRenderState* S; uint32_t level, big, max_regs, max_choices, n_waves, flags, skip_regs, skip_choices; };
struct KaPrune1 { FhRenderState* S; uint32_t level, big, max_choices, mode; };
struct KaColumns { FhRenderState* S; uint32_t n_waves, slots, depmask, flags, pad[2]; const void* table; uint32_t nfpl, layers; };
struct KaNormals { FhRenderState* S; uint32_t n_waves, slots, z_lo, z_hi, bucket_cap, mode; };

struct FrameStreams { hipStream_t s[N_ROLES]; Role cur; hipStream_t on() const { return s[cur]; } };
static FrameStreams frame_streams(const fhip_ctx* ctx, Role at = CALLER) { return FrameStreams{{ctx->stream, ctx->stream_pre, ctx->stream2, ctx->stream3}, at}; }
static hipError_t hop(FrameStreams& fs, Role to, hipEvent_t ev) {
    if (to == fs.cur) return hipSuccess;
    const hipError_t e = hipEventRecord(ev, fs.on());
    fs.cur = to;
    return e != hipSuccess ? e : hipStreamWaitEvent(fs.on(), ev, 0);
}
static ScheduleInputs schedule_inputs(const fhip_ctx* ctx, int out_is_device) {
    ScheduleInputs in;
    in.no_tiles_v = ctx->opt.no_tiles_v; in.no_zrep = ctx->opt.no_zrep; in.column_walk = ctx->opt.column_walk; in.column_group = ctx->opt.column_group;
    in.frame_pipeline = ctx->frame_pipeline; in.use_pipeline = ctx->use_pipeline; in.profiling = ctx->profiling; in.slab_contexts = ctx->slab_contexts;
    in.has_side = ctx->stream2 != nullptr; in.has_tail = ctx->stream3 != nullptr; in.has_flags = ctx->host_flags != nullptr; in.out_is_device = out_is_device != 0;
    return in;
}
static char* rare_file(const fhip_ctx* ctx, const FhRenderState* dS, uint32_t rare_stride) {
    if (!rare_stride) return nullptr;
    return (char*)ctx->rare_scratch.p + (size_t)(dS - (const FhRenderState*)ctx->state.p) * FH_RARE_BLOCKS * rare_stride;
}
static void tiles_by_groups(fhip_ctx* ctx, const RenderSetup& R, FhRenderState* dS, hipStream_t st) {
    const int gg = blocks_for(ctx, R.lds_tiles_group, 8);
    KaTiles ka = {dS, 0, 1, R.group_regs, R.group_choices, (uint32_t)gg, (ctx->probe ? 1u : 0u) | 2u | 4u | 8u, 0, 0};
    (void)launch_asm(ctx, st, FH_ASM_TILES, (uint32_t)gg, &ka, sizeof(ka), R.lds_tiles_group);
    const uint32_t blocks = R.S.qcap[0], root_words = (R.S.troot_choices + 15) / 16, group_words = (R.group_choices + 15) / 16;
    if (R.S.top_chain && R.S.n_top > 64u * FH_CHAIN_SEG) FH_KLAUNCH(k_tchain3d_chunks, dim3(WAVE, blocks), dim3(WAVE), 0, st, dS);
    else if (R.S.top_chain) FH_KLAUNCH(k_tchain3d, dim3(WAVE, blocks), dim3(WAVE), 0, st, dS);
    else FH_KLAUNCH(k_ttop3d, dim3(blocks), dim3(WAVE), 0, st, dS);
    if (R.classify_only || !root_words) FH_KLAUNCH(k_tmark3d, dim3(blocks), dim3(WAVE), 0, st, dS);
    if (R.classify_only) return;
    if (root_words) FH_KLAUNCH(k_tscatter3d, dim3(root_words + 1, blocks), dim3(WAVE), 0, st, dS, group_words, root_words);
    KaPrune1 kp = {dS, 0, 1, R.S.troot_choices, 2};
    if (!R.prune2) { (void)launch_asm(ctx, st, FH_ASM_PRUNE1, blocks * 64, &kp, sizeof(kp)); return; }
    hipEvent_t ea = nullptr, eb = nullptr;
    if (ctx->profiling) { (void)hipEventCreate(&ea); (void)hipEventCreate(&eb); (void)hipEventRecord(ea, st); }
    FH_KLAUNCH(k_prune2, dim3(blocks * FH_P2_PER_SLOT), dim3(FH_P2_WPB * FH_P2_WPC * 64), R.lds_prune2, st, dS, 0u, 1u, root_words,
                       (const uint2*)R.d_links, (const uint2*)R.d_ctab, 2u, R.S.troot_len, R.S.troot_choices, R.p2_cap_kept,
                       (const uint32_t*)(R.d_ctab + std::max<uint32_t>(R.S.troot_choices, 1)), R.n_chain);
    size_t kp_bytes = sizeof(kp);
    void* extra[] = {HIP_LAUNCH_PARAM_BUFFER_POINTER, &kp, HIP_LAUNCH_PARAM_BUFFER_SIZE, &kp_bytes, HIP_LAUNCH_PARAM_END};
    (void)hipModuleLaunchKernel(ctx->asm_fn[FH_ASM_PRUNE1], blocks * 64, 1, 1, WAVE, 1, 1, 0, st, nullptr, extra);
    if (ctx->profiling) { (void)hipEventRecord(eb, st); ctx->asm_events.push_back({FH_ASM_PRUNE1, {ea, eb}}); }
}
static void tiles_asm(fhip_ctx* ctx, const RenderSetup& R, const LevelPlan& L, FhRenderState* dS, int level, FrameStreams& fs) {
    const int gs = blocks_for(ctx, R.lds_tiles_small, 8), gb = blocks_big(ctx, R, R.lds_tiles_big, 8);
    const int K_TILES = R.asm_tiles_t ? FH_ASM_TILES_T : FH_ASM_TILES;
    auto big_stream = [&] { return L.fork_big ? fs.s[SIDE] : fs.on(); };
    KaTiles ka = {dS, (uint32_t)level, 0, SMALL_REGS, SMALL_CHOICES, (uint32_t)gs, (ctx->probe ? 1u : 0u) | (L.exp ? 2u : 0u), 0, 0};
    if (L.fork_big) { (void)hipEventRecord(ctx->ev_rest_fork, fs.on()); (void)hipStreamWaitEvent(fs.s[SIDE], ctx->ev_rest_fork, 0); }
    if (L.v32) {
        ka.n_waves = (uint32_t)(ctx->n_cu * 32);
        (void)launch_asm(ctx, fs.on(), R.asm_tiles_t ? FH_ASM_TILES_V32_T : FH_ASM_TILES_V32, ka.n_waves, &ka, sizeof(ka));
    } else if (L.small_lds)
        (void)launch_asm(ctx, fs.on(), K_TILES, (uint32_t)gs, &ka, sizeof(ka), R.lds_tiles_small);
    ka.big = 1;
    if (L.exp) ka.flags |= ((R.S.P.max_choices + 15) / 16) << 16;
    if (L.rare) return;
    if (L.v64) {
        ka.max_regs = V64_REGS; ka.max_choices = V64_CHOICES;
        ka.n_waves = L.per_slab ? 128u : (uint32_t)(ctx->n_cu * 8);
        if (L.both_lists) ka.flags |= 16u;
        (void)launch_asm(ctx, big_stream(), R.asm_tiles_t ? FH_ASM_TILES_V64_T : FH_ASM_TILES_V64, ka.n_waves, &ka, sizeof(ka));
        (void)hop(fs, L.rest_on, ctx->ev_l1);
        ka.flags &= ~16u;
        ka.skip_regs = V64_REGS; ka.skip_choices = V64_CHOICES;
    }
    if (L.mid) {
        const int gm = blocks_for(ctx, R.lds_tiles_mid, 8);
        ka.max_regs = MID_REGS; ka.max_choices = MID_CHOICES; ka.n_waves = (uint32_t)gm;
        (void)launch_asm(ctx, big_stream(), K_TILES, (uint32_t)gm, &ka, sizeof(ka), R.lds_tiles_mid);
        ka.skip_regs = MID_REGS; ka.skip_choices = MID_CHOICES;
    }
    ka.max_regs = R.S.P.max_regs; ka.max_choices = R.S.P.max_choices; ka.n_waves = (uint32_t)gb;
    if (L.rest) (void)launch_asm(ctx, big_stream(), K_TILES, (uint32_t)gb, &ka, sizeof(ka), R.lds_tiles_big);
    if (L.fork_big) { (void)hipEventRecord(ctx->ev_rest_join, fs.s[SIDE]); (void)hipStreamWaitEvent(fs.on(), ctx->ev_rest_join, 0); }
    if (L.exp) {
        KaPrune1 kp = {dS, (uint32_t)level, 0, SMALL_CHOICES, 0};
        const uint32_t bound = R.S.qcap[level] * 64;
        if (level > 0) (void)launch_asm(ctx, fs.on(), FH_ASM_PRUNE1, bound, &kp, sizeof(kp));
        kp.big = 1; kp.max_choices = R.S.P.max_choices;
        (void)launch_asm(ctx, fs.on(), FH_ASM_PRUNE1, bound, &kp, sizeof(kp));
    }
}
static void tiles_hip(fhip_ctx* ctx, const RenderSetup& R, FhRenderState* dS, int level, hipStream_t st) {
    const int gs = blocks_for(ctx, R.lds_tiles_small, 8), gb = blocks_big(ctx, R, R.lds_tiles_big, 8);
    if (level > 0 && R.full) FH_KLAUNCH((k_teval3d<true, false>), dim3(gs), dim3(WAVE), R.lds_tiles_small, st, dS, level);
    else if (level > 0) FH_KLAUNCH((k_teval3d<false, false>), dim3(gs), dim3(WAVE), R.lds_tiles_small, st, dS, level);
    if (R.full) FH_KLAUNCH((k_teval3d<true, true>), dim3(gb), dim3(WAVE), R.lds_tiles_big, st, dS, level);
    else FH_KLAUNCH((k_teval3d<false, true>), dim3(gb), dim3(WAVE), R.lds_tiles_big, st, dS, level);
}
static void launch_tiles_mono(fhip_ctx* ctx, const RenderSetup& R, FhRenderState* dS, int level, bool is3d, hipStream_t st) {
    const int gs = blocks_for(ctx, R.lds_tiles_small, 8), gb = blocks_big(ctx, R, R.lds_tiles_big, 8);
    launch(ctx, st, FHIP_K_TILES, [&] {
        if (is3d) { if (R.full) FH_LAUNCH_TILES(true, true, true, gb, R.lds_tiles_big); else FH_LAUNCH_TILES(true, false, true, gb, R.lds_tiles_big); }
        else { if (R.full) FH_LAUNCH_TILES(false, true, true, gb, R.lds_tiles_big); else FH_LAUNCH_TILES(false, false, true, gb, R.lds_tiles_big); }
    });
    if (level > 0)
        launch(ctx, st, FHIP_K_TILES, [&] {
            if (is3d) { if (R.full) FH_LAUNCH_TILES(true, true, false, gs, R.lds_tiles_small); else FH_LAUNCH_TILES(true, false, false, gs, R.lds_tiles_small); }
            else { if (R.full) FH_LAUNCH_TILES(false, true, false, gs, R.lds_tiles_small); else FH_LAUNCH_TILES(false, false, false, gs, R.lds_tiles_small); }
        });
}
static void launch_tiles(fhip_ctx* ctx, const RenderSetup& R, const LevelPlan& L, FhRenderState* dS, int level, bool is3d, FrameStreams& fs, const FhHead* head = nullptr) {
    if (L.path == LevelPlan::MONO) return launch_tiles_mono(ctx, R, dS, level, is3d, fs.on());
    const int gp = ctx->n_cu * 8;
    launch(ctx, fs.on(), FHIP_K_TILES, [&] {
        if (is3d) FH_KLAUNCH(k_tsetup3d, dim3(gp), dim3(WAVE), 0, fs.on(), dS, level, head ? *head : FhHead{});
        else FH_KLAUNCH(k_tsetup2d, dim3(gp), dim3(WAVE), 0, fs.on(), dS, level);
    });
    launch(ctx, fs.on(), FHIP_K_TILES, [&] {
        if (L.path == LevelPlan::GROUPS) tiles_by_groups(ctx, R, dS, fs.on());
        else if (L.path == LevelPlan::ASM) tiles_asm(ctx, R, L, dS, level, fs);
        else tiles_hip(ctx, R, dS, level, fs.on());
    });
    const bool last = level + 1 == (int)R.S.P.n_levels;
    const int gpush = last ? ctx->n_cu * L.push_mul : gp;
    launch(ctx, fs.on(), FHIP_K_TILES, [&] {
        const uint32_t rb = L.rare ? FH_RARE_BLOCKS : 0u;
        if (is3d) FH_KLAUNCH(k_tpush3d, dim3(gpush + rb, last ? 1 : 17), dim3(WAVE), 0, fs.on(), dS, level, rb, rare_file(ctx, dS, L.rare_stride), L.rare_stride);
        else {
            if (!R.classify_only) FH_KLAUNCH(k_tpush2d, dim3(gpush), dim3(WAVE), 0, fs.on(), dS, level);
            const uint32_t slots_max = R.S.qcap[level] * ((level == 0 && R.groups) ? R.S.n_tgroups : 1u);
            FH_KLAUNCH(k_tfill2d, dim3(64, slots_max), dim3(256), 0, fs.on(), dS, level);
        }
    });
}

static fhip_status render2d_frame(fhip_ctx* ctx, const fhip_tape* tape, const fhip_render2d_config* cfg, float* out,
                                  int out_is_device) {
    if (ctx->is_cancelled()) return fail(ctx, FHIP_ERR_CANCELLED, "cancelled");
    RenderSetup R;
    memset(&R.S, 0, sizeof(R.S));
    FhRender& P = R.S.P;
    P.width = cfg->width; P.height = cfg->height; P.depth = 0; P.z = cfg->z; P.pixel_perfect = cfg->pixel_perfect ? 1 : 0;
    fhip_status st = bind_inputs(ctx, tape, cfg->axis_slots, cfg->var_keys, cfg->var_values, cfg->n_vars, P);
    if (st) return st;
    const uint32_t size[2] = {cfg->width, cfg->height};
    float s2w[9], m3[9];
    const float ident[9] = {1, 0, 0, 0, 1, 0, 0, 0, 1};
    fhip_screen_to_world(size, 2, s2w);
    mat_product(cfg->world_to_model ? cfg->world_to_model : ident, s2w, 3, m3);
    const float m4[16] = {m3[0], m3[1], 0, m3[2], m3[3], m3[4], 0, m3[5], 0, 0, 1, 0, m3[6], m3[7], 0, m3[8]};
    memcpy(P.mat, m4, sizeof(m4));
    std::vector<uint32_t> ts = cfg->tile_sizes ? trim_tiles(cfg->tile_sizes, cfg->n_tile_sizes, std::max(cfg->width, cfg->height))
                                               : trim_tiles(HIP_TILES_2D, 2, std::max(cfg->width, cfg->height));
    std::vector<uint32_t> tags;
    {
        std::vector<uint32_t> out;
        for (size_t i = 0; i < ts.size(); i++) {
            if (i) {
                uint32_t a = ts[i - 1];
                const uint32_t b = ts[i];
                if (a <= b || a % b) return fail(ctx, FHIP_ERR_UNSUPPORTED, "bad tile size list");
                while (a / b > 8) {
                    uint32_t c = 0;
                    for (uint32_t k = 8; k >= 2 && !c; k--) if (a % k == 0 && (a / k) % b == 0 && a / k > b) c = a / k;
                    if (!c) break;
                    out.push_back(c); tags.push_back((uint32_t)i);
                    a = c;
                }
            }
            out.push_back(ts[i]); tags.push_back((uint32_t)i);
        }
        if (out.size() > FH_MAX_LEVELS) return fail(ctx, FHIP_ERR_UNSUPPORTED, "1..8 tile levels supported");
        ts = out;
    }
    const size_t npix = (size_t)cfg->width * cfg->height;
    float* d_out = out;
    if (!out_is_device) { HIP_TRY(ctx, ctx->tmp_out.ensure(npix * 4)); d_out = (float*)ctx->tmp_out.p; }
    const TapeFacts facts = tape_facts(tape);
    auto pass = [&](RenderSetup& Q, const std::vector<uint32_t>& tiles, const std::vector<uint32_t>& tg) -> fhip_status {
        for (size_t i = 0; i < FH_MAX_LEVELS; i++) Q.S.P.tag[i] = i < tg.size() ? tg[i] : (uint32_t)i;
        fhip_status ps = prepare(ctx, tape, facts, false, tiles, PartSpec{}, Q);
        if (ps) return ps;
        Q.S.image2d = d_out;
        FhRenderState* dS = (FhRenderState*)ctx->state.p;
        const FrameClear no_clear[3] = {};
        FrameStreams fs = frame_streams(ctx);
        hipStream_t const st = fs.on();
        ps = upload_frame(ctx, st, tape, Q, no_clear);
        if (ps) return ps;
        for (uint32_t l = 0; l < Q.S.P.n_levels; l++) {
            if (ctx->is_cancelled()) return fail(ctx, FHIP_ERR_CANCELLED, "cancelled");
            launch_tiles(ctx, Q, plan_level(Q, schedule_inputs(ctx, out_is_device), (int)l, false, 0u, CALLER, CALLER), dS, (int)l, false, fs);
        }
        if (Q.classify_only) return FHIP_OK;
        launch(ctx, st, FHIP_K_POINTS, [&] {
            if (Q.full) FH_KLAUNCH((k_pixels2d<32, true>), dim3(ctx->n_cu * 8), dim3(WAVE), 0, st, dS);
            else FH_KLAUNCH((k_pixels2d<32, false>), dim3(ctx->n_cu * 16), dim3(WAVE), 0, st, dS);
        });
        if (Q.S.P.max_regs > 32)
            launch(ctx, st, FHIP_K_POINTS, [&] {
                const int g = blocks_big(ctx, Q, Q.lds_points_big, 16);
                if (Q.full) FH_KLAUNCH((k_pixels2d<0, true>), dim3(g), dim3(WAVE), Q.lds_points_big, st, dS);
                else FH_KLAUNCH((k_pixels2d<0, false>), dim3(g), dim3(WAVE), Q.lds_points_big, st, dS);
            });
        if (ctx->host_flags) FH_KLAUNCH(k_latch_arena, dim3(1), dim3(1), 0, st, dS, 1u, ctx->host_flags);
        return FHIP_OK;
    };
    const bool small_ok = ts.size() == 2 && tags.size() == 2 && ts[1] >= 8 && ts[0] / ts[1] <= 8 && ctx->opt.root32_max > 0 && linked_root_tape(facts, plan_inputs(ctx)) &&
                          (uint64_t)((P.width + ts[1] - 1) / ts[1]) * ((P.height + ts[1] - 1) / ts[1]) <= 2048u &&
                          (uint64_t)((P.width + ts[0] - 1) / ts[0]) * ((P.height + ts[0] - 1) / ts[0]) <= 64u;
    if (small_ok) {
        RenderSetup A = R;
        A.one_level_64 = true;
        st = pass(A, std::vector<uint32_t>{ts[1]}, std::vector<uint32_t>{1u});
        if (st) return st;
        if (!P.pixel_perfect) {
            RenderSetup B = R;
            B.one_level_64 = true; B.classify_only = true;
            st = pass(B, std::vector<uint32_t>{ts[0]}, std::vector<uint32_t>{0u});
            if (st) return st;
        }
    } else {
        st = pass(R, ts, tags);
        if (st) return st;
    }
    HIP_TRY(ctx, hipGetLastError());
    HIP_TRY(ctx, hipEventRecord(ctx->ev_done, ctx->stream));
    ctx->ev_done_valid = true;
    if (!out_is_device) {
        HIP_TRY(ctx, hipMemcpyAsync(out, d_out, npix * 4, hipMemcpyDeviceToHost, ctx->stream));
        return finish_render(ctx);
    }
    return FHIP_OK;
}

static void slab_begin(fhip_ctx* ctx, const RenderSetup& R, const FrameSchedule& F, FhRenderState* dS, int k, hipStream_t st) {
    const FhRender& P = R.S.P;
    const uint32_t pre = R.S.pre_levels, n_groups = R.groups_per_slab, n32 = ((P.width + 31) / 32) * ((P.height + 31) / 32);
    launch(ctx, st, FHIP_K_OTHER, [&] {
        const bool pyr3 = P.n_levels == 3 && P.tiles[2] == 8 && P.tiles[1] == 32 && P.tiles[0] == 128 && n32 <= 1024;
        const bool rebuild = k != F.slab_first;
        const bool pyr2 = P.n_levels == 2 && P.tiles[1] == 8 && P.tiles[0] == 32 && pre == 1;
        if (rebuild && pyr2) { FH_KLAUNCH(k_slab_begin2, dim3(n32 + F.reset_blocks), dim3(256), 0, st, dS, n32, F.table_words, (uint32_t)k, n_groups); return; }
        if (rebuild && pyr3 && pre == 2) { FH_KLAUNCH(k_slab_begin3, dim3(n32 + F.reset_blocks), dim3(256), 0, st, dS, n32, F.table_words, (uint32_t)k, n_groups); return; }
        FH_KLAUNCH(k_reset_slab, dim3(F.reset_blocks * 4), dim3(WAVE), 0, st, dS, F.table_words, (uint32_t)k, n_groups, (pyr3 && rebuild) ? 1u : 0u);
        if (rebuild && pyr3) FH_KLAUNCH(k_minpyramid3, dim3(n32), dim3(256), 0, st, dS);
        else if (rebuild) FH_KLAUNCH(k_minpyramid, dim3(P.roots_x * P.roots_y), dim3(256), 0, st, dS);
    });
}
static fhip_status tile_step(fhip_ctx* ctx, const RenderSetup& R, const FrameSchedule& F, FrameStreams& fs, FhRenderState* dS, int k, int idx, const FhHead* head) {
    fs.cur = F.tiles;
    if (F.pipe && idx >= (int)F.NC) HIP_TRY(ctx, hipStreamWaitEvent(fs.on(), ctx->ev_leaves[idx - (int)F.NC], 0));
    const FhHead* const mine = head && idx == 0 ? head : nullptr;
    if (!mine) slab_begin(ctx, R, F, dS, k, fs.on());
    for (uint32_t l = R.S.pre_levels; l < R.S.P.n_levels; l++) launch_tiles(ctx, R, F.level[l], dS, (int)l, true, fs, l == R.S.pre_levels ? mine : nullptr);
    if (F.pipe) HIP_TRY(ctx, hipEventRecord(ctx->ev_tiles[idx], fs.on()));
    fs.cur = CALLER;
    return FHIP_OK;
}
static void classify_work(fhip_ctx* ctx, const RenderSetup& R, const FrameSchedule& F, FhRenderState* dS, hipStream_t st) {
    const uint32_t class_blocks = (R.n_footprints + FH_CLASSIFY_FP - 1) / FH_CLASSIFY_FP;
    if (F.by_list && F.rare && R.S.P.max_regs > R.S.leaf_asm_regs)
        launch(ctx, st, FHIP_K_OTHER, [&] { FH_KLAUNCH(k_classify3d, dim3(FH_RARE_BLOCKS), dim3(WAVE), 0, st, dS, 1, 0u, rare_file(ctx, dS, F.rare_stride), F.rare_stride); });
    else if (!F.by_list) launch(ctx, st, FHIP_K_OTHER, [&] {
        FH_KLAUNCH(k_classify3d, dim3(class_blocks + (F.rare ? FH_RARE_BLOCKS : 0u)), dim3(R.S.P.slab / 8 > 16 ? 256 : WAVE), 0, st, dS, R.asm_points ? 1 : 0, class_blocks,
                   rare_file(ctx, dS, F.rare_stride), F.rare_stride);
    });
    if (R.S.P.max_regs > R.S.leaf_asm_regs && !F.rare)
        launch(ctx, st, FHIP_K_POINTS, [&] {
            const int g = blocks_big(ctx, R, R.lds_points_big, 16);
            if (R.full) FH_KLAUNCH((k_leaves3d<2, 0, 1, true>), dim3(g), dim3(WAVE), R.lds_points_big, st, dS);
            else FH_KLAUNCH((k_leaves3d<2, 0, 1, false>), dim3(g), dim3(WAVE), R.lds_points_big, st, dS);
        });
}
static void leaf_work(fhip_ctx* ctx, const RenderSetup& R, const FrameSchedule& F, FhRenderState* dS, uint32_t sk, hipStream_t st) {
    launch(ctx, st, FHIP_K_POINTS, [&] {
        if (F.leaf_walk == FrameSchedule::HIP_LEAVES) {
            const int per_cu = R.full ? 8 : 16;
            if (R.full) { FH_KLAUNCH((k_leaves3d<0, 16, 4, true>), dim3(ctx->n_cu * per_cu), dim3(WAVE), 0, st, dS); FH_KLAUNCH((k_leaves3d<1, 32, 2, true>), dim3(ctx->n_cu * per_cu), dim3(WAVE), 0, st, dS); }
            else { FH_KLAUNCH((k_leaves3d<0, 16, 4, false>), dim3(ctx->n_cu * per_cu), dim3(WAVE), 0, st, dS); FH_KLAUNCH((k_leaves3d<1, 32, 2, false>), dim3(ctx->n_cu * per_cu), dim3(WAVE), 0, st, dS); }
            return;
        }
        const int which = R.asm_points_t ? FH_ASM_COLUMNS_T : FH_ASM_COLUMNS;
        const uint32_t layers = R.S.P.slab / 8;
        const void* const slab_table = sk == 0 ? (const void*)R.S.leaf_table : (const void*)((const FhLeafRef*)ctx->leaf_table_b.p + (size_t)(sk - 1) * R.S.leaf_cap);
        const void* const slab_leaves = sk == 0 ? (const void*)R.S.leaves : (const void*)((const FhLeaf*)ctx->leaves_b.p + (size_t)(sk - 1) * R.S.leaf_cap);
        KaColumns ka = {dS, 0u, R.col_slots, R.col_depmask, R.col_flags, {0, 0}, slab_table, R.n_footprints, layers};
        if (F.leaf_walk == FrameSchedule::BY_LIST) {
            ka.flags |= (3u << 20) | (6u << 24); ka.pad[0] = F.list_waves; ka.table = slab_leaves; ka.nfpl = R.S.leaf_cap;
            (void)launch_asm(ctx, st, which, F.list_waves, &ka, sizeof(ka));
        } else if (F.leaf_walk == FrameSchedule::BY_COLUMNS) {
            ka.flags |= (1u << 20) | (F.g << 24);
            (void)launch_asm(ctx, st, which, (R.n_footprints + 63) / 64 * 64, &ka, sizeof(ka), 0, (layers + (1u << F.g) - 1) >> F.g);
        } else {
            const uint32_t n_blocks = (R.n_footprints + 3) / 4;
            ka.pad[0] = n_blocks > 1 ? (uint32_t)(((uint64_t)1 << 32) / n_blocks) : 0u;
            (void)launch_asm(ctx, st, which, n_blocks, &ka, sizeof(ka), 0, layers);
        }
    });
}
static void normals_work(fhip_ctx* ctx, const RenderSetup& R, const FrameSchedule& F, FhRenderState* dS, int k, hipStream_t st) {
    const uint32_t z_lo = (uint32_t)k * R.S.P.slab, z_hi = z_lo + R.S.P.slab;
    launch(ctx, st, FHIP_K_NORMALS, [&] {
        const int gs = blocks_for(ctx, R.lds_normals_small, 8), gb = blocks_big(ctx, R, R.lds_normals_big, 8);
        const int which = R.asm_points_t ? FH_ASM_NORMALS_T : FH_ASM_NORMALS;
        if (F.by_list) {
            if (F.rare && R.S.P.max_regs > R.S.norm_asm_regs)
                FH_KLAUNCH(k_hits3d, dim3(FH_RARE_BLOCKS), dim3(WAVE), 0, st, dS, z_lo, z_hi, R.hit_bucket_cap, 0u, rare_file(ctx, dS, F.rare_stride), F.rare_stride);
            KaNormals kn = {dS, F.list_waves, R.col_slots, z_lo, z_hi, R.hit_bucket_cap, 1u};
            (void)launch_asm(ctx, st, which, kn.n_waves, &kn, sizeof(kn));
        }
        else if (R.asm_normals) {
            const uint32_t hb = std::min<uint32_t>(R.n_footprints, (uint32_t)ctx->n_cu * 64);
            FH_KLAUNCH(k_hits3d, dim3(hb + (F.rare ? FH_RARE_BLOCKS : 0u)), dim3(WAVE), 0, st, dS, z_lo, z_hi, R.hit_bucket_cap, hb, rare_file(ctx, dS, F.rare_stride), F.rare_stride);
            KaNormals kn = {dS, std::max<uint32_t>((uint32_t)(ctx->n_cu * 8) / FH_HIT_BUCKETS, 1u) * FH_HIT_BUCKETS, R.col_slots, z_lo, z_hi, R.hit_bucket_cap, 0};
            (void)launch_asm(ctx, st, which, kn.n_waves, &kn, sizeof(kn));
        }
        else if (R.full) FH_KLAUNCH((k_normals3d<true, false>), dim3(gs), dim3(WAVE), R.lds_normals_small, st, dS, z_lo, z_hi);
        else FH_KLAUNCH((k_normals3d<false, false>), dim3(gs), dim3(WAVE), R.lds_normals_small, st, dS, z_lo, z_hi);
        if (R.S.P.max_regs > R.S.norm_asm_regs && !(F.rare && R.asm_normals)) {
            if (R.full) FH_KLAUNCH((k_normals3d<true, true>), dim3(gb), dim3(WAVE), R.lds_normals_big, st, dS, z_lo, z_hi);
            else FH_KLAUNCH((k_normals3d<false, true>), dim3(gb), dim3(WAVE), R.lds_normals_big, st, dS, z_lo, z_hi);
        }
    });
}
static FhHead tile_head(const fhip_ctx* ctx, const RenderSetup& R, const FrameSchedule& F) {
    FhHead h{};
    FhFork& fork = h.fork;
    fork.n = F.NC; fork.mark = F.coarse ? 1u : 0u;
    fork.leaves = (FhLeaf*)ctx->leaves_b.p; fork.leaf_table = (FhLeafRef*)ctx->leaf_table_b.p; fork.fp_lists = (uint32_t*)ctx->fp_lists_b.p;
    fork.leaf_cap = (size_t)R.S.leaf_cap; fork.n_footprints = (size_t)R.n_footprints; fork.hit_words = R.hit_words;
    h.on = F.coarse && R.zrep && R.S.pre_levels == 1 && F.by_list && F.n_rendered > 0 && F.level[1].path != LevelPlan::MONO ? 1u : 0u;
    h.slab = (uint32_t)F.slab_first; h.n_root_groups = R.groups_per_slab; h.depmask = R.col_depmask;
    return h;
}
static fhip_status coarse_levels(fhip_ctx* ctx, const RenderSetup& R, const FrameSchedule& F, FrameStreams& fs, FhRenderState* dS, const FhHead& head) {
    const uint32_t pre = R.S.pre_levels;
    const FhFork& fork = head.fork;
    const bool forked_here = F.coarse && R.zrep;
    if (F.coarse) {
        launch_tiles(ctx, R, F.level[0], dS, 0, true, fs);
        if (pre > 1) {
            HIP_TRY(ctx, hop(fs, F.l1_flags, ctx->ev_l0));
            if (R.zrep) launch(ctx, fs.on(), FHIP_K_OTHER, [&] { FH_KLAUNCH(k_tape_flags, dim3(ctx->n_cu * 4), dim3(WAVE), 0, fs.on(), dS, 1, R.col_depmask, 0, FhFork{}); });
            HIP_TRY(ctx, hop(fs, F.l1, ctx->ev_l0));
            launch_tiles(ctx, R, F.level[1], dS, 1, true, fs);
        }
        HIP_TRY(ctx, hop(fs, F.fork_on, pre > 1 ? ctx->ev_l1 : ctx->ev_l0));
        if (R.zrep && !head.on) launch(ctx, fs.on(), FHIP_K_OTHER, [&] { FH_KLAUNCH(k_tape_flags, dim3(ctx->n_cu * 8 + 1), dim3(WAVE), 0, fs.on(), dS, (int)pre, R.col_depmask, 1, fork); });
        if (!F.pipe && !forked_here) launch(ctx, fs.on(), FHIP_K_OTHER, [&] { FH_KLAUNCH(k_mark_frame, dim3(1), dim3(1), 0, fs.on(), dS); });
    }
    if (F.pipe) {
        if (!forked_here) FH_KLAUNCH(k_fork_state, dim3(1), dim3(1), 0, fs.on(), dS, fork);
        HIP_TRY(ctx, hipEventRecord(ctx->ev_fork, fs.on()));
        if (F.fork_to_side) HIP_TRY(ctx, hipStreamWaitEvent(fs.s[SIDE], ctx->ev_fork, 0));
    }
    if (F.ev_pre) HIP_TRY(ctx, hop(fs, CALLER, ctx->ev_pre));
    fs.cur = CALLER;
    if (F.fork_to_tail) HIP_TRY(ctx, hipStreamWaitEvent(fs.s[TAIL], ctx->ev_fork, 0));
    return FHIP_OK;
}
static fhip_status render_slabs(fhip_ctx* ctx, const RenderSetup& R, const FrameSchedule& F, FrameStreams& fs, FhRenderState* dS0, const FhHead& head) {
    const FhHead* const hd = head.on ? &head : nullptr;
    auto slab_state = [&](int idx) { return dS0 + (F.pipe ? (uint32_t)idx % F.NC : 0u); };
    for (int idx = 0; F.tiles_first && idx < F.n_rendered; idx++) { const fhip_status st = tile_step(ctx, R, F, fs, slab_state(idx), F.slab_first - idx, idx, hd); if (st) return st; }
    for (int idx = 0; idx < F.n_rendered; idx++) {
        if (ctx->is_cancelled()) {
            if (hd && idx == 0 && !F.tiles_first) ctx->forked = 0;
            return fail(ctx, FHIP_ERR_CANCELLED, "cancelled");
        }
        const int k = F.slab_first - idx;
        FhRenderState* const dS = slab_state(idx);
        if (!F.tiles_first) { const fhip_status st = tile_step(ctx, R, F, fs, dS, k, idx, hd); if (st) return st; }
        if (F.pipe) HIP_TRY(ctx, hipStreamWaitEvent(fs.s[F.leaf], ctx->ev_tiles[idx], 0));
        if (F.aux_edge) HIP_TRY(ctx, hipStreamWaitEvent(fs.s[F.lists], ctx->ev_tiles[idx], 0));
        classify_work(ctx, R, F, dS, fs.s[F.lists]);
        leaf_work(ctx, R, F, dS, (uint32_t)(dS - dS0), fs.s[F.leaf]);
        if (F.aux_edge) { HIP_TRY(ctx, hipEventRecord(ctx->ev_aux[idx], fs.s[F.leaf])); HIP_TRY(ctx, hipStreamWaitEvent(fs.s[F.normals], ctx->ev_aux[idx], 0)); }
        if (F.normals_on) normals_work(ctx, R, F, dS, k, fs.s[F.normals]);
        if (F.pipe) HIP_TRY(ctx, hipEventRecord(ctx->ev_leaves[idx], fs.s[F.normals]));
    }
    if (F.aux_edge && F.n_rendered > 0) HIP_TRY(ctx, hipStreamWaitEvent(fs.s[CALLER], ctx->ev_leaves[F.n_rendered - 1], 0));
    return FHIP_OK;
}

static fhip_status render3d_frame(fhip_ctx* ctx, const fhip_tape* tape, const fhip_render3d_config* cfg, void* out,
                                  int out_is_device, const PartSpec& part) {
    if (ctx->is_cancelled()) return fail(ctx, FHIP_ERR_CANCELLED, "cancelled");
    if (ctx->opt.stats & 2) g_spans.start();
    (void)hipSetDevice(ctx->device);
    RenderSetup R;
    memset(&R.S, 0, sizeof(R.S));
    FhRender& P = R.S.P;
    P.width = cfg->width; P.height = cfg->height; P.depth = cfg->depth; P.z = 0; P.pixel_perfect = 0;
    fhip_status st = bind_inputs(ctx, tape, cfg->axis_slots, cfg->var_keys, cfg->var_values, cfg->n_vars, P);
    if (st) return st;
    const uint32_t size[3] = {cfg->width, cfg->height, cfg->depth};
    float s2w[16];
    const float ident[16] = {1, 0, 0, 0, 0, 1, 0, 0, 0, 0, 1, 0, 0, 0, 0, 1};
    fhip_screen_to_world(size, 3, s2w);
    mat_product(cfg->world_to_model ? cfg->world_to_model : ident, s2w, 4, P.mat);
    const TapeFacts facts = tape_facts(tape);
    const PlanInputs pin = plan_inputs(ctx);
    column_facts(P, facts, pin, R);
    const TileChoice tiles = choose_tiles_3d(cfg->tile_sizes, cfg->n_tile_sizes, size, part.n_shards * part.nx * part.ny, part.nz, R.column_inv, pin.root32_max, pin.no_zrep,
                                             linked_root_tape(facts, pin));
    if (!tiles.valid) return fail(ctx, FHIP_ERR_UNSUPPORTED, "bad tile size list");
    if (tiles.substituted) ctx->substituted_tiles++;
    ScheduleInputs in = schedule_inputs(ctx, out_is_device);
    in.huge = (size_t)std::max<uint32_t>(tape->t.n_regs, 1) * WAVE * 16 > FH_LDS_MAX || tiles_lds(std::max<uint32_t>(tape->t.n_regs, 1), tape->t.n_choices, 64) > FH_LDS_MAX;
    in.whole = part.n_shards == 1 && part.nx * part.ny * part.nz == 1;
    if (frame_pipelined(in)) {
        for (uint32_t i = 0; i < ctx->extra_sets; i++) std::swap(static_cast<FrameBufs&>(*ctx), ctx->others[i]);
        in.frames_queued = ctx->extra_sets > 0 && ctx->others[0].ev_done_valid && hipEventQuery(ctx->others[0].ev_done) == hipErrorNotReady;
        (void)hipGetLastError();
    }
    const CleanSig left_clean = ctx->clean;
    ctx->clean = CleanSig();
    FH_SPAN(0);
    st = prepare(ctx, tape, facts, true, tiles.ts, part, R);
    if (st) return st;
    FH_SPAN(1);
    in.pre_turn = ctx->pre_turn;
    if (ctx->host_flags) { in.rare_seen = ctx->host_flags[2]; in.last_leaves = ctx->host_flags[3]; }
    const FrameSchedule F = schedule_frame(R, in);
    if (F.takes_turn) ctx->pre_turn++;
    if (F.rare) { HIP_TRY(ctx, ctx->rare_scratch.ensure((size_t)F.rare_stride * FH_RARE_BLOCKS * 4)); ctx->rare_frames++; }
    R.S.leaf_list = F.by_list ? 1u : 0u; ctx->forked = F.pipe ? F.NC : 0;
    FrameStreams fs = frame_streams(ctx, F.root);
    if (F.fpipe && ctx->ev_done_valid) HIP_TRY(ctx, hipStreamWaitEvent(fs.on(), ctx->ev_done, 0));
    const size_t npix = (size_t)cfg->width * cfg->height;
    FhGeometryPixel* d_out = (FhGeometryPixel*)out;
    if (!out_is_device) { HIP_TRY(ctx, ctx->tmp_out.ensure(npix * sizeof(FhGeometryPixel))); d_out = (FhGeometryPixel*)ctx->tmp_out.p; }
    FhRenderState* const dS0 = (FhRenderState*)ctx->state.p;
    const CleanFrame kind = {out_is_device != 0, ctx->profiling};
    CleanSig want_clean;
    want_clean.valid = true; want_clean.pixels = npix; want_clean.mind_words = R.mind_words;
    const bool is_clean = set_is_clean(left_clean, want_clean);
    const FrameClear clear3[3] = {{ctx->zbuf.p, npix * 8, 0u}, {ctx->normals.p, npix * 12, 0u}, {ctx->mind.p, R.mind_words * 4, 0u}}, no_clear[3] = {};
    st = upload_frame(ctx, fs.on(), tape, R, is_clean ? no_clear : clear3);
    if (st) return st;
    FH_SPAN(2);
    const FhHead head = tile_head(ctx, R, F);
    st = coarse_levels(ctx, R, F, fs, dS0, head);
    if (st) return st;
    FH_SPAN(3);
    st = render_slabs(ctx, R, F, fs, dS0, head);
    if (st) return st;
    FH_SPAN(4);
    launch(ctx, ctx->stream, FHIP_K_OTHER, [&] { FH_KLAUNCH(k_finish3d, dim3(ctx->n_cu * 16), dim3(WAVE), 0, ctx->stream, dS0, d_out, std::max<uint32_t>(ctx->forked, 1u), (uint32_t*)ctx->sticky.p, ctx->host_flags,
                                                            leaves_set_clean(kind) ? 1u : 0u, (uint32_t)R.mind_words); });
    HIP_TRY(ctx, hipGetLastError());
    if (ctx->launch_failed) { ctx->launch_failed = false; return FHIP_ERR_HIP; }
    ctx->async_pending = out_is_device != 0;
    HIP_TRY(ctx, hipEventRecord(ctx->ev_done, ctx->stream));
    ctx->ev_done_valid = true;
    ctx->clean = set_left_by(kind, want_clean, true);
    if (ctx->opt.stats & 2) { g_spans.mark(5); g_spans.frame(); }
    if (!out_is_device) {
        HIP_TRY(ctx, hipMemcpyAsync(out, d_out, npix * sizeof(FhGeometryPixel), hipMemcpyDeviceToHost, ctx->stream));
        return finish_render(ctx);
    }
    return FHIP_OK;
}
static bool lanes_possible(fhip_ctx* ctx, int out_is_device) {
    if (ctx->opt.frame_lanes < 2 || ctx->is_lane || !out_is_device || ctx->profiling || ctx->probe || (ctx->opt.stats & 1)) return false;
    if (!ctx->ev_last_valid) return false;
    const hipError_t q = hipEventQuery(ctx->ev_last);
    (void)hipGetLastError();
    return q == hipErrorNotReady;
}
static void lane_tune_release(fhip_ctx* ctx);
static void lanes_release(fhip_ctx* ctx, bool keep_measurements) {
    if (!keep_measurements) lane_tune_release(ctx);
    for (fhip_ctx* L : ctx->lanes) {
        hipStream_t const s = L->lane_stream_owned ? L->stream : nullptr;
        if (L->lane_done) (void)hipEventDestroy(L->lane_done);
        if (L->lane_copied) (void)hipEventDestroy(L->lane_copied);
        L->lane_img.release();
        fhip_ctx_destroy(L);
        if (s) (void)hipStreamDestroy(s);
    }
    ctx->lanes.clear();
}
static fhip_status run_on_lane_(fhip_ctx* ctx, uint32_t max_lanes, size_t bytes, void* out, const std::function<fhip_status(fhip_ctx*, void*)>& render) {
    const uint32_t K = std::min((uint32_t)std::min(ctx->opt.frame_lanes, 8), max_lanes);
    if (ctx->opt.lanes_fail) return fail(ctx, FHIP_ERR_HIP, "frame lanes: failure provoked (option lanes_fail)");
    while (ctx->lanes.size() < K) {
        hipStream_t const mine[3] = {ctx->stream_pre, ctx->stream3, ctx->stream2};
        const size_t k = ctx->lanes.size();
        hipStream_t s = k < 3 ? mine[k] : nullptr;
        const bool owned = !s;
        if (owned) HIP_TRY(ctx, hipStreamCreateWithFlags(&s, hipStreamNonBlocking));
        fhip_ctx* L = nullptr;
        const fhip_status st = fhip_ctx_create(ctx->device, (void*)s, &L);
        if (st) { if (owned) (void)hipStreamDestroy(s); return fail(ctx, st, "frame lanes: no child context"); }
        L->lane_stream_owned = owned;
        L->opt = ctx->opt;
        L->opt.no_pipeline = 1;
        L->opt.frame_lanes = 0;
        apply_options(L);
        L->is_lane = true;
        (void)hipEventCreateWithFlags(&L->lane_done, hipEventDisableTiming);
        (void)hipEventCreateWithFlags(&L->lane_copied, hipEventDisableTiming);
        ctx->lanes.push_back(L);
    }
    fhip_ctx* const L = ctx->lanes[ctx->lane_next++ % K];
    L->cancel_src = &ctx->cancelled;
    L->watch.store(ctx->watch.load(std::memory_order_relaxed), std::memory_order_relaxed);
    HIP_TRY(ctx, L->lane_img.ensure(bytes));
    if (L->lane_copied_valid) HIP_TRY(ctx, hipStreamWaitEvent(L->stream, L->lane_copied, 0));
    const fhip_status st = render(L, L->lane_img.p);
    if (st) { ctx->err = L->err; return st; }
    HIP_TRY(ctx, hipEventRecord(L->lane_done, L->stream));
    HIP_TRY(ctx, hipStreamWaitEvent(ctx->stream, L->lane_done, 0));
    HIP_TRY(ctx, hipMemcpyAsync(out, L->lane_img.p, bytes, hipMemcpyDeviceToDevice, ctx->stream));
    HIP_TRY(ctx, hipEventRecord(L->lane_copied, ctx->stream));
    L->lane_copied_valid = true;
    ctx->lane_frames++;
    if (ctx->tune_cur < 0) ctx->lane_frames_wanted++;
    return FHIP_OK;
}
static const fhip_status FHIP_LANE_FALLBACK = (fhip_status)1000;
static fhip_status run_on_lane(fhip_ctx* ctx, uint32_t max_lanes, size_t bytes, void* out, const std::function<fhip_status(fhip_ctx*, void*)>& render) {
    ctx->last_hip_error = 0;
    for (fhip_ctx* L : ctx->lanes) if (L) L->last_hip_error = 0;
    const fhip_status st = run_on_lane_(ctx, max_lanes, bytes, out, render);
    if (st != FHIP_ERR_HIP) return st;
    bool resources = ctx->opt.lanes_fail != 0 || ctx->last_hip_error == (int)hipErrorOutOfMemory || ctx->err.rfind("frame lanes:", 0) == 0;
    for (fhip_ctx* L : ctx->lanes) if (L && L->last_hip_error == (int)hipErrorOutOfMemory) resources = true;
    if (!resources) return st;
    if (ctx->mesh_leaves.cap) {
        (void)hipDeviceSynchronize();
        ctx->mesh_leaves.release();
    }
    fprintf(stderr, "fidget-hip: frame lanes given up for this context (%s); frames keep to the stage pipeline\n", ctx->err.c_str());
    (void)hipGetLastError();
    (void)hipStreamSynchronize(ctx->stream);
    ctx->opt.frame_lanes = 0;
    lanes_release(ctx);
    ctx->err.clear();
    return FHIP_LANE_FALLBACK;
}
static constexpr uint32_t TUNE_SKIP = 4, TUNE_WIN = 8;
static uint32_t tune_lanes(const fhip_ctx* ctx) { return (uint32_t)std::min(std::max(ctx->opt.frame_lanes, 2), 8); }
static void lane_tune_release(fhip_ctx* ctx) {
    for (auto& t : ctx->lane_tune)
        for (hipEvent_t& e : t.ev) if (e) { (void)hipEventDestroy(e); e = nullptr; }
    ctx->lane_tune.clear();
    ctx->tune_last_key = 0;
    ctx->tune_cur = -1;
}
static bool lane_mode(fhip_ctx* ctx, const fhip_tape* tape, const fhip_render3d_config* cfg, int out_is_device, const PartSpec& part) {
    ctx->tune_cur = -1;
    const bool whole = part.n_shards == 1 && part.nx * part.ny * part.nz == 1;
    const bool possible = lanes_possible(ctx, out_is_device) && ctx->use_pipeline && ctx->frame_pipeline;
    const bool prior = ctx->use_asm && !ctx->opt.no_columns_t && !tape_asm_ok(tape->t);
    if (!possible) { ctx->tune_last_key = 0; return false; }
    uint64_t key = (tape->parent_serial ? tape->parent_serial : tape->serial) * 0x9E3779B97F4A7C15ull;
    key ^= ((uint64_t)cfg->width << 42) ^ ((uint64_t)cfg->height << 21) ^ (uint64_t)cfg->depth;
    key ^= (((uint64_t)part.shard * 64 + part.n_shards) * 0xD6E8FEB86659FD93ull) ^ ((((uint64_t)part.ix * 16 + part.iy) * 16 + part.iz) * 4096 + (part.nx * 16 + part.ny) * 16 + part.nz) * 0xA24BAED4963EE407ull;
    key |= 1;
    int at = -1;
    for (size_t i = 0; i < ctx->lane_tune.size(); i++) if (ctx->lane_tune[i].key == key) at = (int)i;
    if (at < 0) {
        if (ctx->lane_tune.size() < 32) { ctx->lane_tune.emplace_back(); at = (int)ctx->lane_tune.size() - 1; }
        else {
            at = 0;
            for (size_t i = 1; i < ctx->lane_tune.size(); i++) if (ctx->lane_tune[i].used < ctx->lane_tune[at].used) at = (int)i;
            for (hipEvent_t& e : ctx->lane_tune[at].ev) if (e) { (void)hipEventDestroy(e); e = nullptr; }
            ctx->lane_tune[at] = fhip_ctx::LaneTune();
        }
        ctx->lane_tune[at].key = key;
    }
    fhip_ctx::LaneTune& T = ctx->lane_tune[at];
    T.used = ++ctx->tune_clock;
    if (T.phase == 4) { ctx->tune_last_key = key; return T.lanes; }
    if (ctx->tune_last_key != key) {
        ctx->tune_last_key = key;
        if (T.phase < 3) { T.n = 0; return prior; }
    }
    if (T.phase == 3) {
        const hipError_t q = hipEventQuery(T.ev[5]);
        (void)hipGetLastError();
        if (q != hipSuccess) return false;
        bool ok = true;
        for (int w = 0; w < 3; w++) {
            float t = 0.0f;
            ok = ok && hipEventElapsedTime(&t, T.ev[2 * w], T.ev[2 * w + 1]) == hipSuccess && t > 0.0f;
            T.ms[w] = t / (w == 1 ? 2 * tune_lanes(ctx) : TUNE_WIN);
        }
        (void)hipGetLastError();
        T.lanes = ok ? T.ms[1] < 0.97f * std::min(T.ms[0], T.ms[2]) : prior;
        T.phase = 4;
        if (!T.lanes && ctx->lane_frames_wanted == 0) {
            bool others = false;
            for (const fhip_ctx::LaneTune& o : ctx->lane_tune) others = others || (&o != &T && (o.phase != 4 || o.lanes));
            if (!others) lanes_release(ctx, true);
        }
        return T.lanes;
    }
    ctx->tune_cur = at;
    return T.phase == 1;
}
static fhip_status frame_queued(fhip_ctx* ctx, int out_is_device) {
    if (!out_is_device || ctx->is_lane || ctx->opt.frame_lanes < 2) return FHIP_OK;
    if (!ctx->ev_last) HIP_TRY(ctx, hipEventCreateWithFlags(&ctx->ev_last, hipEventDisableTiming));
    HIP_TRY(ctx, hipEventRecord(ctx->ev_last, ctx->stream));
    ctx->ev_last_valid = true;
    if (ctx->tune_cur >= 0) {
        fhip_ctx::LaneTune& T = ctx->lane_tune[(size_t)ctx->tune_cur];
        ctx->tune_cur = -1;
        T.n++;
        const uint32_t K = tune_lanes(ctx);
        const uint32_t skip = T.phase == 1 ? K : TUNE_SKIP, win = T.phase == 1 ? 2 * K : TUNE_WIN, tail = T.phase == 1 ? K : 0u;
        if (T.n == skip || T.n == skip + win) {
            hipEvent_t& e = T.ev[2 * T.phase + (T.n == skip ? 0 : 1)];
            if (!e) HIP_TRY(ctx, hipEventCreate(&e));
            HIP_TRY(ctx, hipEventRecord(e, ctx->stream));
        }
        if (T.n == skip + win + tail) { T.phase++; T.n = 0; }
    }
    return FHIP_OK;
}
static fhip_status render3d_part(fhip_ctx* ctx, const fhip_tape* tape, const fhip_render3d_config* cfg, void* out,
                                 int out_is_device, const PartSpec& part) {
    (void)hipSetDevice(ctx->device);
    std::shared_ptr<const fhip_tape> bound;
    fhip_render3d_config bcfg;
    if (tape->t.n_vars > FH_MAX_INPUTS) {
        const fhip_status bs = bound_tape(ctx, tape, cfg->axis_slots, cfg->var_keys, cfg->var_values, cfg->n_vars, bound);
        if (bs) return bs;
        tape = bound.get();
        bcfg = *cfg; bcfg.axis_slots = BOUND_AXES; bcfg.var_keys = nullptr; bcfg.var_values = nullptr; bcfg.n_vars = 0;
        cfg = &bcfg;
    }
    fhip_status st = lane_mode(ctx, tape, cfg, out_is_device, part)
        ? run_on_lane(ctx, 8, (size_t)cfg->width * cfg->height * sizeof(FhGeometryPixel), out,
                      [&](fhip_ctx* L, void* img) { return render3d_frame(L, tape, cfg, img, 1, part); })
        : render3d_frame(ctx, tape, cfg, out, out_is_device, part);
    if (st == FHIP_LANE_FALLBACK) st = render3d_frame(ctx, tape, cfg, out, out_is_device, part);
    if (st) ctx->tune_cur = -1;
    return st ? st : frame_queued(ctx, out_is_device);
}
fhip_status fhip_render2d(fhip_ctx* ctx, const fhip_tape* tape, const fhip_render2d_config* cfg, float* out, int out_is_device) {
    (void)hipSetDevice(ctx->device);
    std::shared_ptr<const fhip_tape> bound;
    fhip_render2d_config bcfg;
    if (tape->t.n_vars > FH_MAX_INPUTS) {
        const fhip_status bs = bound_tape(ctx, tape, cfg->axis_slots, cfg->var_keys, cfg->var_values, cfg->n_vars, bound);
        if (bs) return bs;
        tape = bound.get();
        bcfg = *cfg; bcfg.axis_slots = BOUND_AXES; bcfg.var_keys = nullptr; bcfg.var_values = nullptr; bcfg.n_vars = 0;
        cfg = &bcfg;
    }
    ctx->tune_cur = -1;
    ctx->tune_last_key = 0;
    fhip_status st = lanes_possible(ctx, out_is_device)
        ? run_on_lane(ctx, 3, (size_t)cfg->width * cfg->height * 4, out, [&](fhip_ctx* L, void* img) { return render2d_frame(L, tape, cfg, (float*)img, 1); })
        : render2d_frame(ctx, tape, cfg, out, out_is_device);
    if (st == FHIP_LANE_FALLBACK) st = render2d_frame(ctx, tape, cfg, out, out_is_device);
    return st ? st : frame_queued(ctx, out_is_device);
}
fhip_status fhip_render3d(fhip_ctx* ctx, const fhip_tape* tape, const fhip_render3d_config* cfg, void* out,
                          int out_is_device) {
    return render3d_part(ctx, tape, cfg, out, out_is_device, PartSpec{});
}
fhip_status fhip_render3d_shard(fhip_ctx* ctx, const fhip_tape* tape, const fhip_render3d_config* cfg, void* out,
                                int out_is_device, uint32_t shard, uint32_t n_shards) {
    if (n_shards == 0 || shard >= n_shards) return fail(ctx, FHIP_ERR_UNSUPPORTED, "bad shard");
    PartSpec p;
    p.shard = shard; p.n_shards = n_shards;
    return render3d_part(ctx, tape, cfg, out, out_is_device, p);
}
fhip_status fhip_render3d_block(fhip_ctx* ctx, const fhip_tape* tape, const fhip_render3d_config* cfg, void* out,
                                int out_is_device, uint32_t index, const uint32_t split[3]) {
    if (!split || !split[0] || !split[1] || !split[2] || index >= split[0] * split[1] * split[2]) return fail(ctx, FHIP_ERR_UNSUPPORTED, "bad block");
    PartSpec p;
    p.nx = split[0]; p.ny = split[1]; p.nz = split[2];
    p.ix = index % p.nx; p.iy = (index / p.nx) % p.ny; p.iz = index / (p.nx * p.ny);
    return render3d_part(ctx, tape, cfg, out, out_is_device, p);
}
fhip_status fhip_merge_depth(fhip_ctx* ctx, void* front, const void* back, uint64_t n_pixels, uint32_t image_depth) {
    if (!n_pixels) return FHIP_OK;
    (void)hipSetDevice(ctx->device);
    FH_KLAUNCH(k_merge_depth, dim3((unsigned)std::min<uint64_t>((n_pixels + 255) / 256, 65535)), dim3(256), 0, ctx->stream,
                       (FhGeometryPixel*)front, (const FhGeometryPixel*)back, (size_t)n_pixels, image_depth);
    HIP_TRY(ctx, hipGetLastError());
    return FHIP_OK;
}
```

fidget_amd/csrc/frame_schedule.hpp:

```cpp
#pragma once
#include <stddef.h>
#include <stdint.h>

#include <algorithm>
#include <vector>

#include "frame_plan.hpp"
#include "render_state.h"

static const uint32_t V32_REGS = 32, V32_CHOICES = 256, V64_REGS = 64, V64_CHOICES = 512;
static const uint32_t FH_RARE_BLOCKS = 8;

enum Role : uint8_t { CALLER = 0, PRE, SIDE, TAIL, N_ROLES };

struct ScheduleInputs {
    int no_tiles_v = 0, no_zrep = 0, column_walk = 1, column_group = 2;
    bool frame_pipeline = true, use_pipeline = true, profiling = false, has_side = true, has_tail = true, has_flags = true;
    uint32_t slab_contexts = 4;
    bool out_is_device = true, huge = false, whole = true;
    bool frames_queued = false;
    uint32_t pre_turn = 0;
    uint32_t rare_seen = 1, last_leaves = 0;
};

struct LevelPlan {
    enum Path : uint8_t { MONO, GROUPS, ASM, HIP } path = MONO;
    Role rest_on = CALLER;
    bool per_slab = false, exp = false;
    bool v32 = false, small_lds = false, v64 = false, both_lists = false;
    bool mid = false, rest = false;
    bool rare = false;
    bool fork_big = false;
    uint32_t rare_stride = 0; int push_mul = 2;
};

struct FrameSchedule {
    bool fpipe = false, lone = false, alt_pre = false, takes_turn = false;
    Role root = CALLER, l1_flags = CALLER, l1 = CALLER, fork_on = CALLER, tiles = CALLER, lists = CALLER, leaf = CALLER, normals = CALLER;
    bool fork_to_side = false, fork_to_tail = false, ev_pre = false, pre_implied = false, aux_edge = false;
    bool coarse = false, pipe = false, tiles_first = false; uint32_t NC = 1;
    int slab_first = 0, slab_stop = 0, n_rendered = 0;
    bool rare = false; uint32_t rare_stride = 0;
    enum LeafWalk : uint8_t { HIP_LEAVES, BY_LIST, BY_COLUMNS, BY_BLOCKS } leaf_walk = HIP_LEAVES;
    bool by_list = false, by_columns = false; uint32_t g = 0;
    uint32_t list_waves = 0, table_words = 0; int reset_blocks = 1;
    bool normals_on = true;
    LevelPlan level[FH_MAX_LEVELS];
};

static bool frame_pipelined(const ScheduleInputs& in) { return in.frame_pipeline && in.use_pipeline && !in.profiling && in.out_is_device && !in.huge; }

static LevelPlan plan_level(const RenderSetup& R, const ScheduleInputs& in, int level, bool is3d, uint32_t rare_stride, Role on, Role rest_on) {
    LevelPlan L;
#ifdef FH_PUSH_MUL
    L.push_mul = FH_PUSH_MUL;
#endif
    L.rare_stride = rare_stride; L.rest_on = rest_on;
    const uint32_t pre = R.S.pre_levels, l = (uint32_t)level;
    const FhRender& P = R.S.P;
    if (!R.split) return L;
    L.per_slab = pre > 0 && l >= pre;
    L.exp = R.prune1 && l < R.exp_levels;
    L.rare = rare_stride && is3d && R.asm_tiles && !in.no_tiles_v && level > 0 && L.per_slab && !L.exp;
    if (R.groups && level == 0) { L.path = LevelPlan::GROUPS; return L; }
    if (!R.asm_tiles) { L.path = LevelPlan::HIP; return L; }
    L.path = LevelPlan::ASM;
    L.fork_big = level > 0 && l < pre && in.use_pipeline && !in.profiling && in.has_side && on == CALLER && is3d;
    const bool vk = !in.no_tiles_v && !L.exp;
    L.both_lists = level > 0 && vk && l < pre && !L.fork_big;
    L.v32 = level > 0 && vk && !L.both_lists; L.small_lds = level > 0 && !vk;
    if (L.rare) return L;
    const bool root_v64 = vk && level == 0 && is3d && P.max_regs <= V64_REGS && P.max_choices <= V64_CHOICES;
    L.v64 = vk && (level > 0 || root_v64);
    L.rest = !L.v64 || P.max_regs > V64_REGS || P.max_choices > V64_CHOICES;
    L.mid = !vk && level > 0 && l < pre && R.lds_tiles_mid * 2 <= R.lds_tiles_big;
    return L;
}

static FrameSchedule schedule_frame(const RenderSetup& R, const ScheduleInputs& in) {
    FrameSchedule F;
    const FhRender& P = R.S.P;
    const uint32_t pre = R.S.pre_levels, n_groups = R.groups_per_slab, slabs = R.slab_hi - R.slab_lo;
    F.fpipe = frame_pipelined(in);
    F.alt_pre = F.fpipe && P.n_levels == 2 && R.column_inv && in.no_zrep == 0 && in.has_tail && in.whole;
    F.lone = F.fpipe && !in.frames_queued;
#ifdef FH_EXP_NO_LONE
    F.lone = false;
#endif
    F.takes_turn = F.fpipe && !F.lone && F.alt_pre;
    F.root = !F.fpipe || F.lone ? CALLER : (F.takes_turn && (in.pre_turn & 1u) ? TAIL : PRE);
    F.coarse = pre && n_groups;
    F.pipe = in.use_pipeline && !in.profiling && slabs > 1 && n_groups > 0 && !R.big_hbm;
    F.NC = F.pipe ? std::min<uint32_t>(in.slab_contexts, slabs) : 1;
    F.slab_first = (int)R.slab_hi - 1; F.slab_stop = (int)R.slab_stop;
    F.n_rendered = n_groups ? std::max(0, F.slab_first - F.slab_stop + 1) : 0;
    const bool l1_side = F.fpipe && !F.lone && pre > 1 && in.has_side && slabs > 1 && n_groups > 0;
    F.tiles_first = F.pipe && l1_side && R.root_invariant && in.has_tail && R.asm_points && slabs <= F.NC;
    F.l1 = l1_side ? SIDE : F.root;
    F.l1_flags = F.tiles_first ? F.root : F.l1;
    const bool tail_to_side = F.fpipe && !F.lone && F.pipe && pre == 1 && in.has_side;
    F.fork_on = F.tiles_first ? TAIL : tail_to_side ? SIDE : F.l1;
    F.tiles = !F.pipe ? CALLER : F.tiles_first ? TAIL : SIDE;
    F.fork_to_side = F.pipe && F.fork_on != SIDE;
    F.fork_to_tail = F.tiles_first;
    F.pre_implied = F.fpipe && F.pipe && pre == 1 && in.has_side && F.fork_on == SIDE;
    F.ev_pre = F.fpipe && F.fork_on != CALLER && !F.pre_implied;
    const bool on_main = F.tiles_first && in.frames_queued;
    F.aux_edge = F.pipe && in.has_tail && R.asm_points && !on_main && !F.alt_pre;
    F.lists = F.normals = F.aux_edge ? TAIL : CALLER;
    const size_t stride = (std::max(std::max(R.lds_tiles_big, R.lds_points_big), R.lds_normals_big) + 255) / 256 * 256;
    F.rare = R.split && R.asm_tiles && R.asm_points && R.asm_normals && !R.big_hbm && in.has_flags && in.rare_seen == 0 &&
             stride * FH_RARE_BLOCKS * 4 <= ((size_t)256 << 20);
    F.rare_stride = F.rare ? (uint32_t)stride : 0u;
    const uint32_t layers = P.slab / 8;
    F.by_list = in.column_walk == 1 && R.column_inv && R.split && R.zrep && R.asm_points && R.asm_normals && layers <= 64 && in.has_flags;
    F.table_words = F.by_list ? 0u : R.table_words;
    F.list_waves = (R.n_footprints + 63) / 64 * 64;
    if (F.by_list && in.last_leaves) F.list_waves = std::min(F.list_waves, (in.last_leaves + in.last_leaves / 8 + 63) / 64 * 64);
    F.reset_blocks = (int)std::max<uint32_t>(1, std::min<uint32_t>(1024, (std::max(F.table_words, n_groups) + 255) / 256));
    F.by_columns = in.column_walk == 2 || ((in.column_walk == 1 || in.column_walk == 3) && R.column_inv);
    const uint32_t g_opt = (uint32_t)std::min(std::max(in.column_group, 0), 6);
    F.g = F.by_columns ? 6u : (R.smooth_tape && g_opt > 1 ? g_opt - 1 : g_opt);
    F.leaf_walk = !R.asm_points ? FrameSchedule::HIP_LEAVES : F.by_list ? FrameSchedule::BY_LIST
                : ((F.by_columns && layers <= 64) || (!F.by_columns && F.g > 0)) ? FrameSchedule::BY_COLUMNS : FrameSchedule::BY_BLOCKS;
#ifdef FH_EXP_SKIP_NORMALS
    F.normals_on = false;
#endif
    for (uint32_t l = 0; l < P.n_levels && l < FH_MAX_LEVELS; l++) {
        const Role on = l >= pre ? F.tiles : l == 0 ? F.root : F.l1;
        F.level[l] = plan_level(R, in, (int)l, true, F.rare_stride, on, l == 1 && l < pre ? F.fork_on : on);
    }
    return F;
}
```

fidget_amd/csrc/kernels.hip:

```cpp
#include <hip/hip_runtime.h>

#include "dev_ops.hpp"
#include "render_state.h"

using namespace fhd;

#define AS4 __attribute__((address_space(4)))
typedef const AS4 uint64_t* ctape_t;

typedef unsigned long long Q4 __attribute__((ext_vector_type(4), aligned(8)));
FH_DEV uint64_t q4_pick(Q4 q, int u) { return u == 0 ? q.x : (u == 1 ? q.y : (u == 2 ? q.z : q.w)); }

FH_DEV uint32_t uni(uint32_t v) { return __builtin_amdgcn_readfirstlane(v); }
FH_DEV uint32_t arena_reserve(FhRenderState* S, uint32_t n) {
    const uint32_t base = atomicAdd(&S->arena_head, n);
    if (base + n < base || base + n > S->arena_cap) { atomicMin(&S->arena_head, S->arena_cap); return 0xFFFFFFFFu; }
    return base;
}
FH_DEV uint64_t ballot(bool p) { return __ballot(p); }

FH_DEV bool op_is_heavy(uint32_t op) {
    return (op >= FH_SIN && op <= FH_LN) || op == FH_ATAN2_RR || op == FH_ATAN2_RI || op == FH_ATAN2_IR ||
           op == FH_MOD_RR || op == FH_MOD_RI || op == FH_MOD_IR;
}
// ... 1033 lines not shown
            const uint32_t w0 = (uint32_t)w, w1 = (uint32_t)(w >> 32);
            const uint32_t op = FH_W_OP(w0), ro = FH_W_OUT(w0), ra = FH_W_A(w0);
            float a[ZB], b[ZB], c[ZB];
            if (op >= FH_ADD_RR) {
                int base;
                if (op < FH_ADD_RI) { base = op - FH_ADD_RR; RGET(ra, a); RGET(w1, b); }
                else if (op < FH_SUB_IR) { base = op - FH_ADD_RI; RGET(ra, a); FOR_Z b[j] = u2f(w1); }
                else { const int irb = op - FH_SUB_IR; base = irb == 0 ? 1 : irb + 2; FOR_Z a[j] = u2f(w1); RGET(ra, b); }
                int ch;
                switch (base) {
                    case 0: FOR_Z c[j] = a[j] + b[j]; break;
                    case 1: FOR_Z c[j] = a[j] - b[j]; break;
                    case 2: FOR_Z c[j] = a[j] * b[j]; break;
                    case 3: FOR_Z c[j] = a[j] / b[j]; break;
                    case 4: if (FULL) { FOR_Z c[j] = t_atan2(a[j], b[j]); } break;
                    case 5: FOR_Z c[j] = f_compare(a[j], b[j]); break;
                    case 6: FOR_Z c[j] = f_mix(a[j], b[j]); break;
                    case 7: if (FULL) { FOR_Z c[j] = rem_euclid(a[j], b[j]); } break;
                    case 8: FOR_Z c[j] = f_min(a[j], b[j], ch); break;
                    case 9: FOR_Z c[j] = f_max(a[j], b[j], ch); break;
                    case 10: FOR_Z c[j] = f_and(a[j], b[j], ch); break;
                    default: FOR_Z c[j] = f_or(a[j], b[j], ch); break;
                }
                RSET(ro, c);
            } else if (op >= FH_NEG) {
                RGET(ra, a);
                switch (op) {
                    case FH_NEG: FOR_Z c[j] = -a[j]; break;
                    case FH_ABS: FOR_Z c[j] = fabsf(a[j]); break;
                    case FH_RECIP: FOR_Z c[j] = 1.0f / a[j]; break;
                    case FH_SQRT: FOR_Z c[j] = sqrtf(a[j]); break;
                    case FH_SQUARE: FOR_Z c[j] = a[j] * a[j]; break;
                    case FH_FLOOR: FOR_Z c[j] = floorf(a[j]); break;
                    case FH_CEIL: FOR_Z c[j] = ceilf(a[j]); break;
                    case FH_ROUND: FOR_Z c[j] = roundf(a[j]); break;
                    case FH_NOT: FOR_Z c[j] = a[j] == 0.0f ? 1.0f : 0.0f; break;
                    case FH_RAND: FOR_Z c[j] = f_rand(a[j]); break;
                    default:
                        if (FULL) { FOR_Z c[j] = F32::unary<true>((int)op, a[j]); }
                        break;
                }
                RSET(ro, c);
            } else if (op == FH_INPUT) {
                const uint32_t kd = P.in_kind[w1];
                if (kd == 0) { FOR_Z c[j] = x[j]; } else if (kd == 1) { FOR_Z c[j] = y[j]; }
                else if (kd == 2) { FOR_Z c[j] = z[j]; } else { const float v = P.in_value[w1]; FOR_Z c[j] = v; }
                RSET(ro, c);
            } else if (op == FH_COPY_REG) {
                RGET(ra, a);
                RSET(ro, a);
            } else if (op == FH_COPY_IMM) {
                FOR_Z c[j] = u2f(w1);
                RSET(ro, c);
            } else {
                RGET(ra, a);
                FOR_Z res[j] = a[j];
            }
        }
        cur = nxt;
    }
}
#undef RGET
#undef RSET

template <bool FULL>
FH_DEV float run_points_lds(ctape_t tape, uint32_t len, const AS4 FhRender& P, float* lds, int lane, float x, float y, float z) {
    Regs<float, WAVE> R{lds, lane};
    float res = 0.0f;
    for (uint32_t k = 0; k < len; k++) {
        const uint64_t w = tape[k];
        step<F32, WAVE, FULL>(
            w, R,
            [&](uint32_t slot) {
                const uint32_t kd = P.in_kind[slot];
                return kd == 0 ? x : (kd == 1 ? y : (kd == 2 ? z : (float)P.in_value[slot]));
            },
            [&](uint32_t, float v) { res = v; }, [&](int) {});
    }
    return res;
}

template <int NR, bool FULL>
__global__ void __launch_bounds__(WAVE) k_pixels2d(FhRenderState* S) {
    extern __shared__ __attribute__((aligned(16))) char smem[];
    const AS4 FhRender& P = *(const AS4 FhRender*)&S->P;
    const int lane = threadIdx.x;
    const uint32_t T = P.tiles[P.n_levels - 1];
    Mat4 mat;
#pragma unroll
    for (int i = 0; i < 16; i++) mat.m[i] = P.mat[i];
    const uint32_t n_leaves = min(S->n_leaves, S->leaf_cap);
    for (uint32_t li = blockIdx.x; li < n_leaves; li += gridDim.x) {
        const AS4 FhLeaf& lf = *(const AS4 FhLeaf*)&S->leaves[li];
        const bool fits = lf.tape.n_regs <= 32;
        if (NR ? !fits : fits) continue;
        const ctape_t tape = (ctape_t)(S->arena + lf.tape.off);
        for (uint32_t p0 = 0; p0 < T * T; p0 += WAVE) {
            const uint32_t p = p0 + lane;
            const uint32_t px = lf.x + (p % T), py = lf.y + (p / T);
            float x[1], y[1], z[1], res[1] = {0.0f};
            xf_point(mat, (float)px, (float)py, P.z, x[0], y[0], z[0]);
            if (NR) run_points<(NR ? NR : 1), 1, FULL>(tape, lf.tape.len, P, x, y, z, res);
            else res[0] = run_points_lds<FULL>(tape, lf.tape.len, P, (float*)big_file(S, smem), lane, x[0], y[0], z[0]);
            if (p < T * T && px < P.width && py < P.height)
                S->image2d[(size_t)py * P.width + px] = isnan_(res[0]) ? u2f(0x7FC00000u) : res[0];
        }
    }
}

#define FH_CLASSIFY_FP 32
template <int CLS, int NR, int ZB, bool FULL>
FH_DEV void leaves3d_body(FhRenderState* S, char* file, uint32_t first, uint32_t stride);
__global__ void __launch_bounds__(256) k_classify3d(FhRenderState* S, int merge01, uint32_t class_blocks, char* rare_file, uint32_t rare_stride) {
    if (blockIdx.x >= class_blocks) {
        if (threadIdx.x < WAVE) leaves3d_body<2, 0, 1, true>(S, rare_file + (size_t)(blockIdx.x - class_blocks) * rare_stride, blockIdx.x - class_blocks, gridDim.x - class_blocks);
        return;
    }
    __shared__ uint32_t mx_s[FH_CLASSIFY_FP], any_s[FH_CLASSIFY_FP];
    const AS4 FhRender& P = *(const AS4 FhRender*)&S->P;
    const uint32_t T = P.tiles[P.n_levels - 1];
    const uint32_t fw = (P.width + T - 1) / T, fh = (P.height + T - 1) / T;
    const uint32_t layers = P.slab / T;
    const uint32_t fl = threadIdx.x % FH_CLASSIFY_FP, lg = threadIdx.x / FH_CLASSIFY_FP, n_lg = blockDim.x / FH_CLASSIFY_FP;
    const uint32_t fi = blockIdx.x * FH_CLASSIFY_FP + fl;
    if (threadIdx.x < FH_CLASSIFY_FP) { mx_s[threadIdx.x] = 0; any_s[threadIdx.x] = 0; }
    __syncthreads();
    const FhLeafRef* col = S->leaf_table + fi;
    uint32_t mx = 0;
    bool any = false;
    if (fi < fw * fh) {
#pragma unroll 8
        for (uint32_t l = lg; l < layers; l += n_lg) {
            const FhLeafRef e = col[(size_t)l * fw * fh];
            if (e.id) { any = true; mx = max(mx, e.len_regs >> 24); }
        }
    }
    if (any) { atomicMax(&mx_s[fl], mx); any_s[fl] = 1; }
    __syncthreads();
    if (threadIdx.x >= FH_CLASSIFY_FP) return;
    mx = mx_s[fl];
    any = any_s[fl] != 0;
    const int cls = !any ? -1 : (mx <= 16 ? 0 : (mx <= (merge01 ? S->norm_asm_regs : 32u) ? (merge01 ? 0 : 1) : 2));
    const int lane = threadIdx.x & (WAVE - 1);
    for (int c = 0; c < 3; c++) {
        const uint64_t m = ballot(cls == c);
        if (m == 0) continue;
        uint32_t base = 0;
        if (lane == (int)__builtin_ctzll(m)) base = atomicAdd(&S->fp_count[c], (uint32_t)__popcll(m));
        base = __shfl(base, __builtin_ctzll(m), WAVE);
        if (cls == c) S->fp_list[c][base + (uint32_t)__popcll(m & ((1ull << lane) - 1))] = ((fi / fw) << 16) | (fi % fw);
    }
}

template <int CLS, int NR, int ZB, bool FULL>
FH_DEV void leaves3d_body(FhRenderState* S, char* file, uint32_t first, uint32_t stride) {
    const AS4 FhRender& P = *(const AS4 FhRender*)&S->P;
    const int lane = threadIdx.x & (WAVE - 1);
    const uint32_t T = P.tiles[P.n_levels - 1];
    Mat4 mat;
#pragma unroll
    for (int i = 0; i < 16; i++) mat.m[i] = P.mat[i];
    const uint32_t n_leaves = min(S->n_leaves, S->leaf_cap);
    if (CLS == 2 && S->n_leaves_lds == 0) return;
    for (uint32_t li = first; li < n_leaves; li += stride) {
        const AS4 FhLeaf& lf = *(const AS4 FhLeaf*)&S->leaves[li];
        const uint32_t regs = lf.tape.n_regs;
        if (CLS == 0 ? regs > 16 : (CLS == 1 ? (regs <= 16 || regs > 32) : regs <= S->leaf_asm_regs)) continue;
        const uint32_t px = lf.x + (lane % T), py = lf.y + (lane / T), lz = lf.z;
        const bool inimg = px < P.width && py < P.height;
        const size_t pix = (size_t)py * P.width + px;
        uint32_t depth = inimg ? (uint32_t)(S->zbuf[pix] >> 32) : 0xFFFFFFFFu;
        bool pending = depth < lz + T;
        if (ballot(pending) == 0) continue;
        const ctape_t tape = (ctape_t)(S->arena + lf.tape.off);
        const uint32_t len = lf.tape.len;
        bool hit = false;
        for (int k = (int)T - 1; k >= 0; k -= ZB) {
            float x[ZB], y[ZB], z[ZB], res[ZB];
            FOR_Z { xf_point(mat, (float)px, (float)py, (float)(lz + k - j), x[j], y[j], z[j]); res[j] = 0.0f; }
            if (NR) run_points<(NR ? NR : 1), ZB, FULL>(tape, len, P, x, y, z, res);
            else res[0] = run_points_lds<FULL>(tape, len, P, (float*)file, lane, x[0], y[0], z[0]);
            FOR_Z {
                if (pending && res[j] < 0.0f) {
                    depth = lz + (uint32_t)(k - j) + 1;
                    hit = true;
                    pending = false;
                }
            }
            if (ballot(pending) == 0) break;
        }
        if (hit) atomicMax((unsigned long long*)&S->zbuf[pix], ((unsigned long long)depth << 32) | (li + 1));
    }
}
template <int CLS, int NR, int ZB, bool FULL>
__global__ void __launch_bounds__(WAVE) k_leaves3d(FhRenderState* S) {
    extern __shared__ __attribute__((aligned(16))) char smem[];
    leaves3d_body<CLS, NR, ZB, FULL>(S, CLS == 2 ? big_file(S, smem) : smem, blockIdx.x, gridDim.x);
}

template <bool FULL, bool BIG>
FH_DEV void normals3d_body(FhRenderState* S, uint32_t z_lo, uint32_t z_hi, char* file, uint32_t first, uint32_t stride) {
    const AS4 FhRender& P = *(const AS4 FhRender*)&S->P;
    const int lane = threadIdx.x & (WAVE - 1);
    const uint32_t T = P.tiles[P.n_levels - 1];
    const uint32_t fw = (P.width + T - 1) / T;
    Regs<GR, WAVE> R{(GR*)file, lane};
    Mat4 mat;
#pragma unroll
    for (int i = 0; i < 16; i++) mat.m[i] = P.mat[i];
    const uint32_t n_all = BIG ? S->fp_count[2] : S->fp_count[0] + S->fp_count[1];
    for (uint32_t wi = first; wi < n_all; wi += stride) {
        uint32_t fi;
        if (BIG) fi = S->fp_list[2][wi];
        else if (wi < S->fp_count[0]) fi = S->fp_list[0][wi];
        else fi = S->fp_list[1][wi - S->fp_count[0]];
        fi = uni(fi);
        const uint32_t px = (fi & 0xFFFFu) * T + (lane % T), py = (fi >> 16) * T + (lane / T);
        const bool inimg = px < P.width && py < P.height;
        const size_t pix = (size_t)py * P.width + px;
        const uint64_t zb = inimg ? S->zbuf[pix] : 0;
        uint32_t id = (uint32_t)zb;
        const uint32_t depth = (uint32_t)(zb >> 32);
        if (depth <= z_lo || depth > z_hi) id = 0;
        uint64_t todo = ballot(id != 0);
        while (todo) {
            const uint32_t cur = uni(__shfl(id, __builtin_ctzll(todo), WAVE));
            const bool mine = (id == cur);
            const AS4 FhLeaf& lf = *(const AS4 FhLeaf*)&S->leaves[cur - 1];
            const ctape_t tape = (ctape_t)(S->arena + lf.tape.off);
            const uint32_t len = lf.tape.len;
            GR gx, gy, gz, res = gr1(0.0f);
            xf_grad(mat, gr((float)px, 1, 0, 0), gr((float)py, 0, 1, 0), gr((float)(depth - 1), 0, 0, 1), gx, gy, gz);
            for (uint32_t q = 0; q < len; q++) {
                const uint64_t w = tape[q];
                step<GRAD, WAVE, FULL>(
                    w, R,
                    [&](uint32_t slot) {
                        const uint32_t kd = P.in_kind[slot];
                        return kd == 0 ? gx : (kd == 1 ? gy : (kd == 2 ? gz : gr1(P.in_value[slot])));
                    },
                    [&](uint32_t, GR v) { res = v; }, [&](int) {});
            }
            if (mine) {
                S->normals[pix * 3 + 0] = res.dx; S->normals[pix * 3 + 1] = res.dy; S->normals[pix * 3 + 2] = res.dz;
                S->zbuf[pix] = zb & 0xFFFFFFFF00000000ull;
                id = 0;
            }
            todo &= ~ballot(mine);
        }
    }
}
template <bool FULL, bool BIG>
__global__ void __launch_bounds__(WAVE) k_normals3d(FhRenderState* S, uint32_t z_lo, uint32_t z_hi) {
    extern __shared__ __attribute__((aligned(16))) char smem[];
    normals3d_body<FULL, BIG>(S, z_lo, z_hi, BIG ? big_file(S, smem) : smem, blockIdx.x, gridDim.x);
}

__global__ void __launch_bounds__(WAVE) k_hits3d(FhRenderState* S, uint32_t z_lo, uint32_t z_hi, uint32_t bucket_cap, uint32_t hit_blocks, char* rare_file, uint32_t rare_stride) {
    if (blockIdx.x >= hit_blocks) {
        normals3d_body<true, true>(S, z_lo, z_hi, rare_file + (size_t)(blockIdx.x - hit_blocks) * rare_stride, blockIdx.x - hit_blocks, gridDim.x - hit_blocks);
        return;
    }
    const AS4 FhRender& P = *(const AS4 FhRender*)&S->P;
    const uint32_t T = P.tiles[P.n_levels - 1];
    const int lane = threadIdx.x & (WAVE - 1);
    const uint32_t n0 = S->fp_count[0], n_all = n0 + S->fp_count[1];
    for (uint32_t wi = blockIdx.x; wi < n_all; wi += hit_blocks) {
        const uint32_t fi = uni(wi < n0 ? S->fp_list[0][wi] : S->fp_list[1][wi - n0]);
        const uint32_t px = (fi & 0xFFFFu) * T + (lane % T), py = (fi >> 16) * T + (lane / T);
        const uint64_t zb = (px < P.width && py < P.height) ? S->zbuf[(size_t)py * P.width + px] : 0;
        uint32_t id = (uint32_t)zb;
        const uint32_t depth = (uint32_t)(zb >> 32);
        if (depth <= z_lo || depth > z_hi) id = 0;
        uint64_t todo = ballot(id != 0);
        uint32_t k = 0, mine = 0;
        while (todo) {
            const uint32_t cur = uni(__shfl(id, __builtin_ctzll(todo), WAVE));
            if (lane == (int)k) mine = cur;
            k++;
            todo &= ~ballot(id == cur);
        }
        if (k == 0) continue;
        const uint32_t b = wi % FH_HIT_BUCKETS;
        uint32_t base = 0;
        if (lane == 0) base = atomicAdd(&S->hit_list[b * FH_HIT_STRIDE], k);
        base = uni(__shfl(base, 0, WAVE));
        if ((uint32_t)lane < k && base + lane < bucket_cap) S->hit_list[FH_HIT_BUCKETS * FH_HIT_STRIDE + (size_t)b * bucket_cap + base + lane] = mine;
    }
}

FH_DEV void reset_slab_body(FhRenderState* S, uint32_t i, uint32_t stride, uint32_t table_words, uint32_t slab, uint32_t n_root_groups, uint32_t reset_root_mind) {
    for (uint32_t k = i; k < table_words; k += stride) S->leaf_table[k] = FhLeafRef{0, 0, 0, 0};
    const uint32_t P0 = S->pre_levels;
    if (i == 0) {
        S->slab_z = slab * S->P.slab;
        for (uint32_t l = P0; l < FH_MAX_LEVELS; l++) {
            S->count[l] = 0; S->cursor[l] = 0; S->count_big[l] = 0; S->cursor_big[l] = 0;
            S->setup_cur[l] = 0; S->push_cur[l] = 0;
            S->n_slots[0][l] = 0; S->n_slots[1][l] = 0; S->eval_cur[0][l] = 0; S->eval_cur[1][l] = 0;
        }
        if (P0 == 0) {
            S->count_big[0] = n_root_groups;
            S->arena_head = S->arena_root_end;
        } else {
            S->queue[P0] = S->squeue + (size_t)slab * S->squeue_cap;
            S->count[P0] = S->scount[slab];
            S->count_big[P0] = S->scount_big[slab];
            S->arena_head = S->arena_frame_end;
        }
        S->n_leaves = 0; S->n_leaves_lds = 0; S->leaf_cursor = 0; S->leaf_cursor_big = 0; S->normal_cursor = 0; S->normal_cursor_big = 0;
        for (int c = 0; c < 3; c++) { S->fp_count[c] = 0; S->fp_cursor[c] = 0; }
    }
    if (S->hit_list)
        for (uint32_t k = i; k < FH_HIT_BUCKETS; k += stride) S->hit_list[k * FH_HIT_STRIDE] = 0;
    if (P0 == 0 && i < n_root_groups) S->queue[0][S->qcap[0] - 1 - i].z = slab * S->P.slab;
    if (reset_root_mind) {
        const uint32_t T = S->P.tiles[0], n = ((S->P.width + T - 1) / T) * ((S->P.height + T - 1) / T);
        for (uint32_t k = i; k < n; k += stride) S->mind[0][k] = 0xFFFFFFFFu;
    }
}
__global__ void k_reset_slab(FhRenderState* S, uint32_t table_words, uint32_t slab, uint32_t n_root_groups, uint32_t reset_root_mind) {
    reset_slab_body(S, blockIdx.x * blockDim.x + threadIdx.x, gridDim.x * blockDim.x, table_words, slab, n_root_groups, reset_root_mind);
}
struct FhFrameBegin {
    uint32_t* state_dst; const uint32_t* state_src; uint32_t state_words;
    uint32_t* roots_dst; const uint32_t* roots_src; uint32_t roots_words;
    uint32_t* clear[3]; unsigned long long clear_words[3]; uint32_t fill[3];
};
__global__ void __launch_bounds__(WAVE) k_frame_begin(FhFrameBegin a) {
    if (blockIdx.x < 4) {
        for (uint32_t i = blockIdx.x * WAVE + threadIdx.x; i < a.state_words; i += 4 * WAVE) a.state_dst[i] = a.state_src[i];
    } else if (blockIdx.x < 8) {
        for (uint32_t i = (blockIdx.x - 4) * WAVE + threadIdx.x; i < a.roots_words; i += 4 * WAVE) a.roots_dst[i] = a.roots_src[i];
    }
    const size_t tid = (size_t)blockIdx.x * blockDim.x + threadIdx.x, nth = (size_t)gridDim.x * blockDim.x;
    for (int k = 0; k < 3; k++) {
        if (!a.clear[k]) continue;
        const uint4 f = make_uint4(a.fill[k], a.fill[k], a.fill[k], a.fill[k]);
        uint4* p4 = (uint4*)a.clear[k];
        const size_t n4 = a.clear_words[k] / 4;
        for (size_t i = tid; i < n4; i += nth) p4[i] = f;
        for (size_t i = n4 * 4 + tid; i < a.clear_words[k]; i += nth) a.clear[k][i] = a.fill[k];
    }
}
__global__ void k_mark_frame(FhRenderState* S) { S->arena_frame_end = min(S->arena_head, S->arena_cap); }

__global__ void __launch_bounds__(256) k_minpyramid(FhRenderState* S) {
    const AS4 FhRender& P = *(const AS4 FhRender*)&S->P;
    const uint32_t T0 = P.tiles[0];
    const uint32_t x0 = (blockIdx.x / P.roots_y) * T0, y0 = (blockIdx.x % P.roots_y) * T0;
    for (int l = (int)P.n_levels - 1; l >= 0; l--) {
        const uint32_t T = P.tiles[l], n = T0 / T, ntx = (P.width + T - 1) / T;
        for (uint32_t t = threadIdx.x; t < n * n; t += blockDim.x) {
            const uint32_t tx = x0 / T + t % n, ty = y0 / T + t / n;
            if (tx * T >= P.width || ty * T >= P.height) continue;
            uint32_t mn = 0xFFFFFFFFu;
            if (l == (int)P.n_levels - 1) {
                for (uint32_t p = 0; p < T * T; p++) {
                    const uint32_t x = tx * T + p % T, y = ty * T + p / T;
                    if (x < P.width && y < P.height) mn = min(mn, (uint32_t)(S->zbuf[(size_t)y * P.width + x] >> 32));
                }
            } else {
                const uint32_t Tc = P.tiles[l + 1], c = T / Tc, ncx = (P.width + Tc - 1) / Tc;
                for (uint32_t q = 0; q < c * c; q++) {
                    const uint32_t sx = tx * c + q % c, sy = ty * c + q / c;
                    if (sx * Tc < P.width && sy * Tc < P.height) mn = min(mn, S->mind[l + 1][sy * ncx + sx]);
                }
            }
            S->mind[l][ty * ntx + tx] = mn;
        }
        __threadfence_block();
        __syncthreads();
    }
}

template <bool ROOT>
FH_DEV void minpyramid3_body(FhRenderState* S, uint32_t block) {
    __shared__ uint32_t part[4];
    const AS4 FhRender& P = *(const AS4 FhRender*)&S->P;
    const int lane = threadIdx.x & 63, w = threadIdx.x >> 6;
    const uint32_t T2 = P.tiles[2], T1 = P.tiles[1], T0 = P.tiles[0];
    const uint32_t n1x = (P.width + T1 - 1) / T1, n2x = (P.width + T2 - 1) / T2, n0x = (P.width + T0 - 1) / T0;
    const uint32_t bx = block % n1x, by = block / n1x;
    const uint32_t ty = by * 4 + w, y = ty * T2 + (lane >> 3);
    uint32_t v[4];
#pragma unroll
    for (int i = 0; i < 4; i++) {
        const uint32_t x = (bx * 4 + i) * T2 + (lane & 7);
        v[i] = (x < P.width && y < P.height) ? (uint32_t)(S->zbuf[(size_t)y * P.width + x] >> 32) : 0xFFFFFFFFu;
    }
    uint32_t row = 0xFFFFFFFFu;
#pragma unroll
    for (int i = 0; i < 4; i++) {
        uint32_t mn = v[i];
#pragma unroll
        for (int d = 32; d >= 1; d >>= 1) mn = min(mn, (uint32_t)__shfl_xor((int)mn, d, WAVE));
        const uint32_t tx = bx * 4 + i;
        if (lane == 0 && tx * T2 < P.width && ty * T2 < P.height) S->mind[2][ty * n2x + tx] = mn;
        row = min(row, mn);
    }
    if (lane == 0) part[w] = row;
    __syncthreads();
    if (threadIdx.x == 0) {
        const uint32_t m = min(min(part[0], part[1]), min(part[2], part[3]));
        S->mind[1][by * n1x + bx] = m;
        if (ROOT) atomicMin(&S->mind[0][(by * T1 / T0) * n0x + bx * T1 / T0], m);
    }
}
// ... 154 lines not shown
```

include/fidget_hip_debug.h:

```cpp
#ifndef FIDGET_HIP_DEBUG_H
#define FIDGET_HIP_DEBUG_H
#include "fidget_hip.h"
#ifdef __cplusplus
extern "C" {
#endif

fhip_status fhip_debug_stats(fhip_ctx* ctx, uint64_t out[64]);
fhip_status fhip_debug_leaf_stats(fhip_ctx* ctx, uint64_t out[8]);
uint32_t fhip_debug_tape_links(const fhip_tape* tape, uint64_t* out, uint32_t cap);
uint32_t fhip_debug_tape_chain(const fhip_tape* tape, uint32_t* out, uint32_t cap);
uint32_t fhip_debug_leaves(fhip_ctx* ctx, void* out, uint32_t cap);
fhip_status fhip_debug_probe(fhip_ctx* ctx, float* out);
uint64_t fhip_debug_lane_frames(const fhip_ctx* ctx);
uint64_t fhip_debug_rare_frames(const fhip_ctx* ctx);
int fhip_debug_lane_tune(const fhip_ctx* ctx, float ms[3], int* lanes);
fhip_status fhip_debug_trans_probe(fhip_ctx* ctx, uint32_t copy, uint32_t fn, uint32_t first, uint64_t n, uint64_t out[2]);
uint32_t fhip_debug_arena(fhip_ctx* ctx, uint32_t off, uint32_t n, uint64_t* out);
fhip_status fhip_debug_bound_tape(fhip_ctx* ctx, const fhip_tape* tape, const int32_t* axis_slots, const uint64_t* keys, const float* vals,
                                  uint32_t n, fhip_tape** out);
fhip_status fhip_debug_bench(fhip_ctx* ctx, const fhip_tape* tape, uint32_t n_waves, uint32_t reps, int variant,
                             double* ms);

fhip_status fhip_debug_ubench(fhip_ctx* ctx, uint32_t test, uint32_t iters, uint32_t n_waves, float* out);
fhip_status fhip_debug_math_sweep(fhip_ctx* ctx, int op, uint32_t first, uint32_t stride, uint64_t n, const float* ref, uint64_t out[4]);
uint32_t fhip_debug_groups(fhip_ctx* ctx, int kind, uint32_t index, void* out, uint32_t cap, uint32_t counts[2]);

void fhip_debug_walk_dual(const uint32_t* cells, uint64_t n_cells, const uint32_t* root, const float* verts, uint64_t n_verts, int parallel,
                          uint64_t counts[2], uint64_t* tris, float* verts_out);
fhip_status fhip_debug_stl_pack(fhip_ctx* ctx, const float* verts, uint64_t n_verts, const uint64_t* tris, uint64_t n_tris, void* out);

#ifdef __cplusplus
}
#endif
#endif
```

Measured before the change: 9.936 million Mvoxel/s.

## Fuse rare-leaf point and normal eval into one kernel; trim frame events

Adds a k_rare_leaves3d kernel that evaluates point depth and, for the winning lane, the gradient normal for high-register leaves in one pass. When the schedule selects rare_leaves, it replaces the separate rare classify and rare hits launches. It also defers the staging-slot event record until the coarse levels hand off to another stream, and skips recording leaf and fork events that no later stage waits on. The frame-in-flight check now reuses the last end event instead of recording an extra ev_last, which removes per-frame event overhead but makes the bookkeeping subtler.

Result: faster. 10.37 million Mvoxel/s, median of 6 (+4.4%).

```diff
diff --git a/fidget_amd/_abi.py b/fidget_amd/_abi.py
--- a/fidget_amd/_abi.py
+++ b/fidget_amd/_abi.py
@@ -206,6 +206,7 @@
     "fhip_debug_probe": (i32, [vp, vp]),
     "fhip_debug_lane_frames": (u64, [vp]),
     "fhip_debug_rare_frames": (u64, [vp]),
+    "fhip_debug_rare_launches": (u64, [vp]),
     "fhip_debug_lane_tune": (i32, [vp, vp, vp]),
     "fhip_debug_trans_probe": (i32, [vp, u32, u32, u32, u64, vp]),
     "fhip_debug_arena": (u32, [vp, u32, u32, vp]),
diff --git a/fidget_amd/context.py b/fidget_amd/context.py
--- a/fidget_amd/context.py
+++ b/fidget_amd/context.py
@@ -54,6 +54,9 @@
 
     def rare_frames(self):
         return int(lib().fhip_debug_rare_frames(self._h))
+
+    def rare_launches(self):
+        return int(lib().fhip_debug_rare_launches(self._h))
 
     def set_option(self, name, value=1):
         self.check(lib().fhip_ctx_set_option(self._h, name.encode(), int(value)))
diff --git a/fidget_amd/csrc/capi_context.hpp b/fidget_amd/csrc/capi_context.hpp
--- a/fidget_amd/csrc/capi_context.hpp
+++ b/fidget_amd/csrc/capi_context.hpp
@@ -130,7 +130,6 @@
     (void)hipSetDevice(c->device);
     (void)hipStreamSynchronize(c->stream);
     lanes_release(c);
-    if (c->ev_last) (void)hipEventDestroy(c->ev_last);
     if (c->stream_pre) (void)hipStreamSynchronize(c->stream_pre);
     if (c->stream2) (void)hipStreamSynchronize(c->stream2);
     (void)hipStreamSynchronize(c->stream);
diff --git a/fidget_amd/csrc/capi_core.hpp b/fidget_amd/csrc/capi_core.hpp
--- a/fidget_amd/csrc/capi_core.hpp
+++ b/fidget_amd/csrc/capi_core.hpp
@@ -146,14 +146,14 @@
     }
     DevBuf tmp_out, io_a, io_b, io_c, io_d, io_e;
     DevBuf sticky;
-    struct Staging { void* p = nullptr; size_t cap = 0; hipEvent_t ev = nullptr; bool used = false; } staging[8];
+    struct Staging { void* p = nullptr; size_t cap = 0; hipEvent_t ev = nullptr; } staging[FH_STAGING_SLOTS];
     DevBuf mesh_leaves;
     void* mesh_pinned = nullptr;
     size_t mesh_pinned_cap = 0;
     void* mesh_octree_cache = nullptr;
     uint32_t* mesh_first = nullptr;
     size_t mesh_first_cap = 0;
-    uint32_t staging_next = 0;
+    StagingRing ring;
     size_t arena_bytes = (size_t)256 << 20, arena_cap_bytes = (size_t)4 << 30;
     uint64_t hip_tile_frames = 0;
     uint64_t substituted_tiles = 0;
@@ -167,10 +167,11 @@
     std::vector<fhip_ctx*> lanes;
     uint32_t lane_next = 0;
     uint64_t rare_frames = 0;
+    uint64_t rare_launches = 0;
     uint64_t lane_frames = 0;
     uint64_t lane_frames_wanted = 0;
-    hipEvent_t ev_last = nullptr;
-    bool ev_last_valid = false;
+    hipEvent_t last_end = nullptr;
+    bool before_asked = false, before_busy = false;
     struct LaneTune {
         uint64_t key = 0, used = 0;
         int phase = 0;
diff --git a/fidget_amd/csrc/capi_debug.hpp b/fidget_amd/csrc/capi_debug.hpp
--- a/fidget_amd/csrc/capi_debug.hpp
+++ b/fidget_amd/csrc/capi_debug.hpp
@@ -142,6 +142,12 @@
     if (!ctx) return 0;
     uint64_t n = ctx->rare_frames;
     for (const fhip_ctx* l : ctx->lanes) n += l ? l->rare_frames : 0;
+    return n;
+}
+uint64_t fhip_debug_rare_launches(const fhip_ctx* ctx) {
+    if (!ctx) return 0;
+    uint64_t n = ctx->rare_launches;
+    for (const fhip_ctx* l : ctx->lanes) n += l ? l->rare_launches : 0;
     return n;
 }
 uint64_t fhip_debug_lane_frames(const fhip_ctx* ctx) { return ctx ? ctx->lane_frames : 0; }
diff --git a/fidget_amd/csrc/capi_render.hpp b/fidget_amd/csrc/capi_render.hpp
--- a/fidget_amd/csrc/capi_render.hpp
+++ b/fidget_amd/csrc/capi_render.hpp
@@ -195,10 +195,16 @@
 }
 
 struct FrameClear { void* p = nullptr; size_t bytes = 0; uint32_t fill = 0; };
-static fhip_status upload_frame(fhip_ctx* ctx, hipStream_t st, const fhip_tape* tape, RenderSetup& R, const FrameClear (&clear)[3]) {
+struct RecordSlot {
+    fhip_ctx* ctx = nullptr; uint32_t slot = 0; hipStream_t st = nullptr;
+    void operator()() const { if (hipEventRecord(ctx->staging[slot].ev, st) == hipSuccess) ctx->ring.used[slot] = true; else (void)hipGetLastError(); }
+};
+typedef SlotGuard<RecordSlot> StagingGuard;
+static fhip_status upload_frame(fhip_ctx* ctx, hipStream_t st, const fhip_tape* tape, RenderSetup& R, const FrameClear (&clear)[3], StagingGuard* later = nullptr) {
     const size_t roots_bytes = R.roots.size() * sizeof(FhGroup);
-    fhip_ctx::Staging& sg = ctx->staging[ctx->staging_next++ % 8];
-    if (sg.ev && sg.used) HIP_TRY(ctx, hipEventSynchronize(sg.ev));
+    const uint32_t slot = ctx->ring.take();
+    fhip_ctx::Staging& sg = ctx->staging[slot];
+    if (sg.ev && ctx->ring.used[slot]) HIP_TRY(ctx, hipEventSynchronize(sg.ev));
     if (!sg.ev) HIP_TRY(ctx, hipEventCreateWithFlags(&sg.ev, hipEventDisableTiming));
     if (sg.cap < sizeof(FhRenderState) + roots_bytes) {
         if (sg.p) (void)hipHostFree(sg.p);
@@ -234,9 +240,9 @@
     }
     const unsigned blocks = (unsigned)std::max<size_t>(8, std::min<size_t>((size_t)ctx->n_cu * 32, (most + 64 * 64 - 1) / (64 * 64)));
     FH_KLAUNCH(k_frame_begin, dim3(blocks), dim3(WAVE), 0, st, fb);
+    if (later) { later->record_now = RecordSlot{ctx, slot, st}; later->arm(); }
+    else RecordSlot{ctx, slot, st}();
     HIP_TRY(ctx, hipGetLastError());
-    HIP_TRY(ctx, hipEventRecord(sg.ev, st));
-    sg.used = true;
     for (auto& e : ctx->prof_events) { (void)hipEventDestroy(e.second.first); (void)hipEventDestroy(e.second.second); }
     ctx->prof_events.clear();
     for (auto& e : ctx->asm_events) { (void)hipEventDestroy(e.second.first); (void)hipEventDestroy(e.second.second); }
@@ -472,7 +478,7 @@
     }
     HIP_TRY(ctx, hipGetLastError());
     HIP_TRY(ctx, hipEventRecord(ctx->ev_done, ctx->stream));
-    ctx->ev_done_valid = true;
+    ctx->ev_done_valid = true; ctx->last_end = ctx->ev_done;
     if (!out_is_device) {
         HIP_TRY(ctx, hipMemcpyAsync(out, d_out, npix * 4, hipMemcpyDeviceToHost, ctx->stream));
         return finish_render(ctx);
@@ -496,7 +502,7 @@
 }
 static fhip_status tile_step(fhip_ctx* ctx, const RenderSetup& R, const FrameSchedule& F, FrameStreams& fs, FhRenderState* dS, int k, int idx, const FhHead* head) {
     fs.cur = F.tiles;
-    if (F.pipe && idx >= (int)F.NC) HIP_TRY(ctx, hipStreamWaitEvent(fs.on(), ctx->ev_leaves[idx - (int)F.NC], 0));
+    if (waits_leaves(F, idx)) HIP_TRY(ctx, hipStreamWaitEvent(fs.on(), ctx->ev_leaves[idx - (int)F.NC], 0));
     const FhHead* const mine = head && idx == 0 ? head : nullptr;
     if (!mine) slab_begin(ctx, R, F, dS, k, fs.on());
     for (uint32_t l = R.S.pre_levels; l < R.S.P.n_levels; l++) launch_tiles(ctx, R, F.level[l], dS, (int)l, true, fs, l == R.S.pre_levels ? mine : nullptr);
@@ -506,8 +512,9 @@
 }
 static void classify_work(fhip_ctx* ctx, const RenderSetup& R, const FrameSchedule& F, FhRenderState* dS, hipStream_t st) {
     const uint32_t class_blocks = (R.n_footprints + FH_CLASSIFY_FP - 1) / FH_CLASSIFY_FP;
-    if (F.by_list && F.rare && R.S.P.max_regs > R.S.leaf_asm_regs)
-        launch(ctx, st, FHIP_K_OTHER, [&] { FH_KLAUNCH(k_classify3d, dim3(FH_RARE_BLOCKS), dim3(WAVE), 0, st, dS, 1, 0u, rare_file(ctx, dS, F.rare_stride), F.rare_stride); });
+    if (F.rare_leaves) {}
+    else if (F.by_list && F.rare && R.S.P.max_regs > R.S.leaf_asm_regs)
+        launch(ctx, st, FHIP_K_OTHER, [&] { ctx->rare_launches++; FH_KLAUNCH(k_classify3d, dim3(FH_RARE_BLOCKS), dim3(WAVE), 0, st, dS, 1, 0u, rare_file(ctx, dS, F.rare_stride), F.rare_stride); });
     else if (!F.by_list) launch(ctx, st, FHIP_K_OTHER, [&] {
         FH_KLAUNCH(k_classify3d, dim3(class_blocks + (F.rare ? FH_RARE_BLOCKS : 0u)), dim3(R.S.P.slab / 8 > 16 ? 256 : WAVE), 0, st, dS, R.asm_points ? 1 : 0, class_blocks,
                    rare_file(ctx, dS, F.rare_stride), F.rare_stride);
@@ -551,8 +558,11 @@
         const int gs = blocks_for(ctx, R.lds_normals_small, 8), gb = blocks_big(ctx, R, R.lds_normals_big, 8);
         const int which = R.asm_points_t ? FH_ASM_NORMALS_T : FH_ASM_NORMALS;
         if (F.by_list) {
-            if (F.rare && R.S.P.max_regs > R.S.norm_asm_regs)
+            if (F.rare_leaves) { ctx->rare_launches++; FH_KLAUNCH(k_rare_leaves3d, dim3(FH_RARE_BLOCKS), dim3(WAVE), 0, st, dS, z_lo, z_hi, rare_file(ctx, dS, F.rare_stride), F.rare_stride); }
+            else if (F.rare && R.S.P.max_regs > R.S.norm_asm_regs) {
+                ctx->rare_launches++;
                 FH_KLAUNCH(k_hits3d, dim3(FH_RARE_BLOCKS), dim3(WAVE), 0, st, dS, z_lo, z_hi, R.hit_bucket_cap, 0u, rare_file(ctx, dS, F.rare_stride), F.rare_stride);
+            }
             KaNormals kn = {dS, F.list_waves, R.col_slots, z_lo, z_hi, R.hit_bucket_cap, 1u};
             (void)launch_asm(ctx, st, which, kn.n_waves, &kn, sizeof(kn));
         }
@@ -580,28 +590,29 @@
     h.slab = (uint32_t)F.slab_first; h.n_root_groups = R.groups_per_slab; h.depmask = R.col_depmask;
     return h;
 }
-static fhip_status coarse_levels(fhip_ctx* ctx, const RenderSetup& R, const FrameSchedule& F, FrameStreams& fs, FhRenderState* dS, const FhHead& head) {
+static fhip_status coarse_levels(fhip_ctx* ctx, const RenderSetup& R, const FrameSchedule& F, FrameStreams& fs, FhRenderState* dS, const FhHead& head, StagingGuard& slot) {
     const uint32_t pre = R.S.pre_levels;
     const FhFork& fork = head.fork;
     const bool forked_here = F.coarse && R.zrep;
+    auto leave = [&](Role to, hipEvent_t ev) { if (to != fs.cur) slot.record(); return hop(fs, to, ev); };
     if (F.coarse) {
         launch_tiles(ctx, R, F.level[0], dS, 0, true, fs);
         if (pre > 1) {
-            HIP_TRY(ctx, hop(fs, F.l1_flags, ctx->ev_l0));
+            HIP_TRY(ctx, leave(F.l1_flags, ctx->ev_l0));
             if (R.zrep) launch(ctx, fs.on(), FHIP_K_OTHER, [&] { FH_KLAUNCH(k_tape_flags, dim3(ctx->n_cu * 4), dim3(WAVE), 0, fs.on(), dS, 1, R.col_depmask, 0, FhFork{}); });
-            HIP_TRY(ctx, hop(fs, F.l1, ctx->ev_l0));
+            HIP_TRY(ctx, leave(F.l1, ctx->ev_l0));
             launch_tiles(ctx, R, F.level[1], dS, 1, true, fs);
         }
-        HIP_TRY(ctx, hop(fs, F.fork_on, pre > 1 ? ctx->ev_l1 : ctx->ev_l0));
+        HIP_TRY(ctx, leave(F.fork_on, pre > 1 ? ctx->ev_l1 : ctx->ev_l0));
         if (R.zrep && !head.on) launch(ctx, fs.on(), FHIP_K_OTHER, [&] { FH_KLAUNCH(k_tape_flags, dim3(ctx->n_cu * 8 + 1), dim3(WAVE), 0, fs.on(), dS, (int)pre, R.col_depmask, 1, fork); });
         if (!F.pipe && !forked_here) launch(ctx, fs.on(), FHIP_K_OTHER, [&] { FH_KLAUNCH(k_mark_frame, dim3(1), dim3(1), 0, fs.on(), dS); });
     }
     if (F.pipe) {
         if (!forked_here) FH_KLAUNCH(k_fork_state, dim3(1), dim3(1), 0, fs.on(), dS, fork);
-        HIP_TRY(ctx, hipEventRecord(ctx->ev_fork, fs.on()));
+        if (F.rec_fork) HIP_TRY(ctx, hipEventRecord(ctx->ev_fork, fs.on()));
         if (F.fork_to_side) HIP_TRY(ctx, hipStreamWaitEvent(fs.s[SIDE], ctx->ev_fork, 0));
     }
-    if (F.ev_pre) HIP_TRY(ctx, hop(fs, CALLER, ctx->ev_pre));
+    if (F.ev_pre) HIP_TRY(ctx, leave(CALLER, ctx->ev_pre));
     fs.cur = CALLER;
     if (F.fork_to_tail) HIP_TRY(ctx, hipStreamWaitEvent(fs.s[TAIL], ctx->ev_fork, 0));
     return FHIP_OK;
@@ -624,12 +635,21 @@
         leaf_work(ctx, R, F, dS, (uint32_t)(dS - dS0), fs.s[F.leaf]);
         if (F.aux_edge) { HIP_TRY(ctx, hipEventRecord(ctx->ev_aux[idx], fs.s[F.leaf])); HIP_TRY(ctx, hipStreamWaitEvent(fs.s[F.normals], ctx->ev_aux[idx], 0)); }
         if (F.normals_on) normals_work(ctx, R, F, dS, k, fs.s[F.normals]);
-        if (F.pipe) HIP_TRY(ctx, hipEventRecord(ctx->ev_leaves[idx], fs.s[F.normals]));
+        if (records_leaves(F, idx)) HIP_TRY(ctx, hipEventRecord(ctx->ev_leaves[idx], fs.s[F.normals]));
     }
     if (F.aux_edge && F.n_rendered > 0) HIP_TRY(ctx, hipStreamWaitEvent(fs.s[CALLER], ctx->ev_leaves[F.n_rendered - 1], 0));
     return FHIP_OK;
 }
 
+static void new_frame(fhip_ctx* ctx) { ctx->before_asked = false; }
+static bool frame_before_under_way(fhip_ctx* ctx) {
+    if (!ctx->before_asked) {
+        ctx->before_asked = true;
+        ctx->before_busy = ctx->last_end && hipEventQuery(ctx->last_end) == hipErrorNotReady;
+        (void)hipGetLastError();
+    }
+    return ctx->before_busy;
+}
 static fhip_status render3d_frame(fhip_ctx* ctx, const fhip_tape* tape, const fhip_render3d_config* cfg, void* out,
                                   int out_is_device, const PartSpec& part) {
     if (ctx->is_cancelled()) return fail(ctx, FHIP_ERR_CANCELLED, "cancelled");
@@ -658,8 +678,7 @@
     in.whole = part.n_shards == 1 && part.nx * part.ny * part.nz == 1;
     if (frame_pipelined(in)) {
         for (uint32_t i = 0; i < ctx->extra_sets; i++) std::swap(static_cast<FrameBufs&>(*ctx), ctx->others[i]);
-        in.frames_queued = ctx->extra_sets > 0 && ctx->others[0].ev_done_valid && hipEventQuery(ctx->others[0].ev_done) == hipErrorNotReady;
-        (void)hipGetLastError();
+        in.frames_queued = ctx->extra_sets > 0 && frame_before_under_way(ctx);
     }
     const CleanSig left_clean = ctx->clean;
     ctx->clean = CleanSig();
@@ -684,11 +703,12 @@
     want_clean.valid = true; want_clean.pixels = npix; want_clean.mind_words = R.mind_words;
     const bool is_clean = set_is_clean(left_clean, want_clean);
     const FrameClear clear3[3] = {{ctx->zbuf.p, npix * 8, 0u}, {ctx->normals.p, npix * 12, 0u}, {ctx->mind.p, R.mind_words * 4, 0u}}, no_clear[3] = {};
-    st = upload_frame(ctx, fs.on(), tape, R, is_clean ? no_clear : clear3);
+    StagingGuard slot(RecordSlot{});
+    st = upload_frame(ctx, fs.on(), tape, R, is_clean ? no_clear : clear3, &slot);
     if (st) return st;
     FH_SPAN(2);
     const FhHead head = tile_head(ctx, R, F);
-    st = coarse_levels(ctx, R, F, fs, dS0, head);
+    st = coarse_levels(ctx, R, F, fs, dS0, head, slot);
     if (st) return st;
     FH_SPAN(3);
     st = render_slabs(ctx, R, F, fs, dS0, head);
@@ -700,7 +720,8 @@
     if (ctx->launch_failed) { ctx->launch_failed = false; return FHIP_ERR_HIP; }
     ctx->async_pending = out_is_device != 0;
     HIP_TRY(ctx, hipEventRecord(ctx->ev_done, ctx->stream));
-    ctx->ev_done_valid = true;
+    ctx->ev_done_valid = true; ctx->last_end = ctx->ev_done;
+    slot.record();
     ctx->clean = set_left_by(kind, want_clean, true);
     if (ctx->opt.stats & 2) { g_spans.mark(5); g_spans.frame(); }
     if (!out_is_device) {
@@ -711,14 +732,12 @@
 }
 static bool lanes_possible(fhip_ctx* ctx, int out_is_device) {
     if (ctx->opt.frame_lanes < 2 || ctx->is_lane || !out_is_device || ctx->profiling || ctx->probe || (ctx->opt.stats & 1)) return false;
-    if (!ctx->ev_last_valid) return false;
-    const hipError_t q = hipEventQuery(ctx->ev_last);
-    (void)hipGetLastError();
-    return q == hipErrorNotReady;
+    return frame_before_under_way(ctx);
 }
 static void lane_tune_release(fhip_ctx* ctx);
 static void lanes_release(fhip_ctx* ctx, bool keep_measurements) {
     if (!keep_measurements) lane_tune_release(ctx);
+    for (fhip_ctx* L : ctx->lanes) if (ctx->last_end == L->lane_copied) ctx->last_end = nullptr;
     for (fhip_ctx* L : ctx->lanes) {
         hipStream_t const s = L->lane_stream_owned ? L->stream : nullptr;
         if (L->lane_done) (void)hipEventDestroy(L->lane_done);
@@ -762,7 +781,7 @@
     HIP_TRY(ctx, hipStreamWaitEvent(ctx->stream, L->lane_done, 0));
     HIP_TRY(ctx, hipMemcpyAsync(out, L->lane_img.p, bytes, hipMemcpyDeviceToDevice, ctx->stream));
     HIP_TRY(ctx, hipEventRecord(L->lane_copied, ctx->stream));
-    L->lane_copied_valid = true;
+    L->lane_copied_valid = true; ctx->last_end = L->lane_copied;
     ctx->lane_frames++;
     if (ctx->tune_cur < 0) ctx->lane_frames_wanted++;
     return FHIP_OK;
@@ -851,9 +870,6 @@
 }
 static fhip_status frame_queued(fhip_ctx* ctx, int out_is_device) {
     if (!out_is_device || ctx->is_lane || ctx->opt.frame_lanes < 2) return FHIP_OK;
-    if (!ctx->ev_last) HIP_TRY(ctx, hipEventCreateWithFlags(&ctx->ev_last, hipEventDisableTiming));
-    HIP_TRY(ctx, hipEventRecord(ctx->ev_last, ctx->stream));
-    ctx->ev_last_valid = true;
     if (ctx->tune_cur >= 0) {
         fhip_ctx::LaneTune& T = ctx->lane_tune[(size_t)ctx->tune_cur];
         ctx->tune_cur = -1;
@@ -881,6 +897,7 @@
         bcfg = *cfg; bcfg.axis_slots = BOUND_AXES; bcfg.var_keys = nullptr; bcfg.var_values = nullptr; bcfg.n_vars = 0;
         cfg = &bcfg;
     }
+    new_frame(ctx);
     fhip_status st = lane_mode(ctx, tape, cfg, out_is_device, part)
         ? run_on_lane(ctx, 8, (size_t)cfg->width * cfg->height * sizeof(FhGeometryPixel), out,
                       [&](fhip_ctx* L, void* img) { return render3d_frame(L, tape, cfg, img, 1, part); })
@@ -900,6 +917,7 @@
         bcfg = *cfg; bcfg.axis_slots = BOUND_AXES; bcfg.var_keys = nullptr; bcfg.var_values = nullptr; bcfg.n_vars = 0;
         cfg = &bcfg;
     }
+    new_frame(ctx);
     ctx->tune_cur = -1;
     ctx->tune_last_key = 0;
     fhip_status st = lanes_possible(ctx, out_is_device)
diff --git a/fidget_amd/csrc/frame_schedule.hpp b/fidget_amd/csrc/frame_schedule.hpp
--- a/fidget_amd/csrc/frame_schedule.hpp
+++ b/fidget_amd/csrc/frame_schedule.hpp
@@ -38,11 +38,13 @@
     bool fpipe = false, lone = false, alt_pre = false, takes_turn = false;
     Role root = CALLER, l1_flags = CALLER, l1 = CALLER, fork_on = CALLER, tiles = CALLER, lists = CALLER, leaf = CALLER, normals = CALLER;
     bool fork_to_side = false, fork_to_tail = false, ev_pre = false, pre_implied = false, aux_edge = false;
+    bool rec_fork = false;
     bool coarse = false, pipe = false, tiles_first = false; uint32_t NC = 1;
     int slab_first = 0, slab_stop = 0, n_rendered = 0;
     bool rare = false; uint32_t rare_stride = 0;
     enum LeafWalk : uint8_t { HIP_LEAVES, BY_LIST, BY_COLUMNS, BY_BLOCKS } leaf_walk = HIP_LEAVES;
     bool by_list = false, by_columns = false; uint32_t g = 0;
+    bool rare_leaves = false;
     uint32_t list_waves = 0, table_words = 0; int reset_blocks = 1;
     bool normals_on = true;
     LevelPlan level[FH_MAX_LEVELS];
@@ -103,6 +105,7 @@
     F.tiles = !F.pipe ? CALLER : F.tiles_first ? TAIL : SIDE;
     F.fork_to_side = F.pipe && F.fork_on != SIDE;
     F.fork_to_tail = F.tiles_first;
+    F.rec_fork = F.fork_to_side || F.fork_to_tail;
     F.pre_implied = F.fpipe && F.pipe && pre == 1 && in.has_side && F.fork_on == SIDE;
     F.ev_pre = F.fpipe && F.fork_on != CALLER && !F.pre_implied;
     const bool on_main = F.tiles_first && in.frames_queued;
@@ -115,6 +118,10 @@
     const uint32_t layers = P.slab / 8;
     F.by_list = in.column_walk == 1 && R.column_inv && R.split && R.zrep && R.asm_points && R.asm_normals && layers <= 64 && in.has_flags;
     F.table_words = F.by_list ? 0u : R.table_words;
+    F.rare_leaves = F.by_list && F.rare && P.max_regs > R.S.leaf_asm_regs && R.S.leaf_asm_regs == R.S.norm_asm_regs;
+#ifdef FH_EXP_TWO_RARE_LAUNCHES
+    F.rare_leaves = false;
+#endif
     F.list_waves = (R.n_footprints + 63) / 64 * 64;
     if (F.by_list && in.last_leaves) F.list_waves = std::min(F.list_waves, (in.last_leaves + in.last_leaves / 8 + 63) / 64 * 64);
     F.reset_blocks = (int)std::max<uint32_t>(1, std::min<uint32_t>(1024, (std::max(F.table_words, n_groups) + 255) / 256));
@@ -132,3 +139,26 @@
     }
     return F;
 }
+
+static bool waits_leaves(const FrameSchedule& F, int idx) { return F.pipe && idx >= (int)F.NC && idx < F.n_rendered; }
+static bool records_leaves(const FrameSchedule& F, int idx) {
+    if (!F.pipe || idx < 0 || idx >= F.n_rendered) return false;
+    return idx + (int)F.NC < F.n_rendered || (F.aux_edge && idx == F.n_rendered - 1);
+}
+
+static const uint32_t FH_STAGING_SLOTS = 8;
+struct StagingRing {
+    uint32_t next = 0;
+    bool used[FH_STAGING_SLOTS] = {};
+    uint32_t take() { return next++ % FH_STAGING_SLOTS; }
+};
+template <class Record> struct SlotGuard {
+    Record record_now;
+    bool armed = false;
+    explicit SlotGuard(Record r) : record_now(r) {}
+    SlotGuard(const SlotGuard&) = delete;
+    SlotGuard& operator=(const SlotGuard&) = delete;
+    void arm() { armed = true; }
+    void record() { if (armed) { armed = false; record_now(); } }
+    ~SlotGuard() { record(); }
+};
diff --git a/fidget_amd/csrc/kernels.hip b/fidget_amd/csrc/kernels.hip
--- a/fidget_amd/csrc/kernels.hip
+++ b/fidget_amd/csrc/kernels.hip
@@ -1209,6 +1209,26 @@
     }
 }
 
+template <int NR, int ZB, bool FULL>
+FH_DEV bool leaf_points(const AS4 FhRender& P, const Mat4& mat, ctape_t tape, uint32_t len, char* file, int lane, uint32_t px, uint32_t py, uint32_t lz, uint32_t T, bool pending,
+                        uint32_t& depth) {
+    bool hit = false;
+    for (int k = (int)T - 1; k >= 0; k -= ZB) {
+        float x[ZB], y[ZB], z[ZB], res[ZB];
+        FOR_Z { xf_point(mat, (float)px, (float)py, (float)(lz + k - j), x[j], y[j], z[j]); res[j] = 0.0f; }
+        if (NR) run_points<(NR ? NR : 1), ZB, FULL>(tape, len, P, x, y, z, res);
+        else res[0] = run_points_lds<FULL>(tape, len, P, (float*)file, lane, x[0], y[0], z[0]);
+        FOR_Z {
+            if (pending && res[j] < 0.0f) {
+                depth = lz + (uint32_t)(k - j) + 1;
+                hit = true;
+                pending = false;
+            }
+        }
+        if (ballot(pending) == 0) break;
+    }
+    return hit;
+}
 template <int CLS, int NR, int ZB, bool FULL>
 FH_DEV void leaves3d_body(FhRenderState* S, char* file, uint32_t first, uint32_t stride) {
     const AS4 FhRender& P = *(const AS4 FhRender*)&S->P;
@@ -1231,21 +1251,7 @@
         if (ballot(pending) == 0) continue;
         const ctape_t tape = (ctape_t)(S->arena + lf.tape.off);
         const uint32_t len = lf.tape.len;
-        bool hit = false;
-        for (int k = (int)T - 1; k >= 0; k -= ZB) {
-            float x[ZB], y[ZB], z[ZB], res[ZB];
-            FOR_Z { xf_point(mat, (float)px, (float)py, (float)(lz + k - j), x[j], y[j], z[j]); res[j] = 0.0f; }
-            if (NR) run_points<(NR ? NR : 1), ZB, FULL>(tape, len, P, x, y, z, res);
-            else res[0] = run_points_lds<FULL>(tape, len, P, (float*)file, lane, x[0], y[0], z[0]);
-            FOR_Z {
-                if (pending && res[j] < 0.0f) {
-                    depth = lz + (uint32_t)(k - j) + 1;
-                    hit = true;
-                    pending = false;
-                }
-            }
-            if (ballot(pending) == 0) break;
-        }
+        const bool hit = leaf_points<NR, ZB, FULL>(P, mat, tape, len, file, lane, px, py, lz, T, pending, depth);
         if (hit) atomicMax((unsigned long long*)&S->zbuf[pix], ((unsigned long long)depth << 32) | (li + 1));
     }
 }
@@ -1255,6 +1261,22 @@
     leaves3d_body<CLS, NR, ZB, FULL>(S, CLS == 2 ? big_file(S, smem) : smem, blockIdx.x, gridDim.x);
 }
 
+template <bool FULL>
+FH_DEV GR leaf_gradient(const AS4 FhRender& P, const Mat4& mat, ctape_t tape, uint32_t len, Regs<GR, WAVE> R, uint32_t px, uint32_t py, uint32_t depth) {
+    GR gx, gy, gz, res = gr1(0.0f);
+    xf_grad(mat, gr((float)px, 1, 0, 0), gr((float)py, 0, 1, 0), gr((float)(depth - 1), 0, 0, 1), gx, gy, gz);
+    for (uint32_t q = 0; q < len; q++) {
+        const uint64_t w = tape[q];
+        step<GRAD, WAVE, FULL>(
+            w, R,
+            [&](uint32_t slot) {
+                const uint32_t kd = P.in_kind[slot];
+                return kd == 0 ? gx : (kd == 1 ? gy : (kd == 2 ? gz : gr1(P.in_value[slot])));
+            },
+            [&](uint32_t, GR v) { res = v; }, [&](int) {});
+    }
+    return res;
+}
 template <bool FULL, bool BIG>
 FH_DEV void normals3d_body(FhRenderState* S, uint32_t z_lo, uint32_t z_hi, char* file, uint32_t first, uint32_t stride) {
     const AS4 FhRender& P = *(const AS4 FhRender*)&S->P;
@@ -1286,18 +1308,7 @@
             const AS4 FhLeaf& lf = *(const AS4 FhLeaf*)&S->leaves[cur - 1];
             const ctape_t tape = (ctape_t)(S->arena + lf.tape.off);
             const uint32_t len = lf.tape.len;
-            GR gx, gy, gz, res = gr1(0.0f);
-            xf_grad(mat, gr((float)px, 1, 0, 0), gr((float)py, 0, 1, 0), gr((float)(depth - 1), 0, 0, 1), gx, gy, gz);
-            for (uint32_t q = 0; q < len; q++) {
-                const uint64_t w = tape[q];
-                step<GRAD, WAVE, FULL>(
-                    w, R,
-                    [&](uint32_t slot) {
-                        const uint32_t kd = P.in_kind[slot];
-                        return kd == 0 ? gx : (kd == 1 ? gy : (kd == 2 ? gz : gr1(P.in_value[slot])));
-                    },
-                    [&](uint32_t, GR v) { res = v; }, [&](int) {});
-            }
+            const GR res = leaf_gradient<FULL>(P, mat, tape, len, R, px, py, depth);
             if (mine) {
                 S->normals[pix * 3 + 0] = res.dx; S->normals[pix * 3 + 1] = res.dy; S->normals[pix * 3 + 2] = res.dz;
                 S->zbuf[pix] = zb & 0xFFFFFFFF00000000ull;
@@ -1311,6 +1322,42 @@
 __global__ void __launch_bounds__(WAVE) k_normals3d(FhRenderState* S, uint32_t z_lo, uint32_t z_hi) {
     extern __shared__ __attribute__((aligned(16))) char smem[];
     normals3d_body<FULL, BIG>(S, z_lo, z_hi, BIG ? big_file(S, smem) : smem, blockIdx.x, gridDim.x);
+}
+
+__global__ void __launch_bounds__(WAVE) k_rare_leaves3d(FhRenderState* S, uint32_t z_lo, uint32_t z_hi, char* rare_file, uint32_t rare_stride) {
+    if (S->n_leaves_lds == 0) return;
+    const AS4 FhRender& P = *(const AS4 FhRender*)&S->P;
+    const int lane = threadIdx.x & (WAVE - 1);
+    const uint32_t T = P.tiles[P.n_levels - 1];
+    char* const file = rare_file + (size_t)blockIdx.x * rare_stride;
+    Mat4 mat;
+#pragma unroll
+    for (int i = 0; i < 16; i++) mat.m[i] = P.mat[i];
+    const uint32_t n_leaves = min(S->n_leaves, S->leaf_cap);
+    for (uint32_t li = blockIdx.x; li < n_leaves; li += gridDim.x) {
+        const AS4 FhLeaf& lf = *(const AS4 FhLeaf*)&S->leaves[li];
+        if (lf.tape.n_regs <= S->leaf_asm_regs) continue;
+        const uint32_t px = lf.x + (lane % T), py = lf.y + (lane / T), lz = lf.z;
+        const bool inimg = px < P.width && py < P.height;
+        const size_t pix = (size_t)py * P.width + px;
+        uint32_t depth = inimg ? (uint32_t)(S->zbuf[pix] >> 32) : 0xFFFFFFFFu;
+        const bool pending = depth < lz + T;
+        if (ballot(pending) == 0) continue;
+        const ctape_t tape = (ctape_t)(S->arena + lf.tape.off);
+        const uint32_t len = lf.tape.len;
+        const bool hit = leaf_points<0, 1, true>(P, mat, tape, len, file, lane, px, py, lz, T, pending, depth);
+        bool mine = false;
+        if (hit) {
+            const unsigned long long w = ((unsigned long long)depth << 32) | (li + 1);
+            mine = atomicMax((unsigned long long*)&S->zbuf[pix], w) < w && depth > z_lo && depth <= z_hi;
+        }
+        if (ballot(mine) == 0) continue;
+        const GR res = leaf_gradient<true>(P, mat, tape, len, Regs<GR, WAVE>{(GR*)file, lane}, px, py, depth);
+        if (mine) {
+            S->normals[pix * 3 + 0] = res.dx; S->normals[pix * 3 + 1] = res.dy; S->normals[pix * 3 + 2] = res.dz;
+            S->zbuf[pix] = (uint64_t)depth << 32;
+        }
+    }
 }
 
 __global__ void __launch_bounds__(WAVE) k_hits3d(FhRenderState* S, uint32_t z_lo, uint32_t z_hi, uint32_t bucket_cap, uint32_t hit_blocks, char* rare_file, uint32_t rare_stride) {
diff --git a/include/fidget_hip_debug.h b/include/fidget_hip_debug.h
--- a/include/fidget_hip_debug.h
+++ b/include/fidget_hip_debug.h
@@ -13,6 +13,7 @@
 fhip_status fhip_debug_probe(fhip_ctx* ctx, float* out);
 uint64_t fhip_debug_lane_frames(const fhip_ctx* ctx);
 uint64_t fhip_debug_rare_frames(const fhip_ctx* ctx);
+uint64_t fhip_debug_rare_launches(const fhip_ctx* ctx);
 int fhip_debug_lane_tune(const fhip_ctx* ctx, float ms[3], int* lanes);
 fhip_status fhip_debug_trans_probe(fhip_ctx* ctx, uint32_t copy, uint32_t fn, uint32_t first, uint64_t n, uint64_t out[2]);
 uint32_t fhip_debug_arena(fhip_ctx* ctx, uint32_t off, uint32_t n, uint64_t* out);
```
